# 0xC000005/PyChebyshev

Measured on AMD Instinct MI355X. Metric: point-evals/sec, 5D Black-Scholes n=11^5 barycentric + TT, 1/2/4/8 GPU, higher is better.
Workload: dtype f64; 1 GPU; 5D Black-Scholes n=11^5 full-tensor barycentric, 1,000,000 fp64 queries per GPU; evals_per_point=1, parallelism=batch-sharded x1, model replicated, one process per GPU, gather=none

## Files before the change

### pychebyshev_amd/_build.py

```python
from __future__ import annotations

import hashlib
import os
import shutil
import subprocess
import sys

HERE = os.path.dirname(os.path.abspath(__file__))
CSRC = os.path.join(HERE, "csrc")
LIB = os.path.join(HERE, "libpcx_hip.so")
PCX_H = os.path.join("..", "..", "include", "pcx.h")
HOST_H = ["pcx_common.h", "pcx_internal.h", PCX_H]
SOURCES = {
    "pcx_core.hip": HOST_H,
    "pcx_bary.hip": HOST_H + ["pcx_bary_internal.h", "bary_kernels.h", "gather_kernels.h", "sobol_kernels.h"],
    "pcx_bary_grid.hip": HOST_H + ["pcx_bary_internal.h", "bary_grid_kernels.h", "bary_weights.h"],
    "pcx_bary_kfold.hip": HOST_H + ["pcx_bary_internal.h", "bary_kfold_kernels.h"],
    "pcx_spline.hip": HOST_H + ["pcx_bary_internal.h", "gather_kernels.h", "route_kernels.h"],
    "pcx_tt.hip": HOST_H + ["tt_kernels.h", "tt_lpp_kernels.h", "tt_fd_kernels.h"],
    "pcx_tt_box.hip": HOST_H + ["tt_lpp_kernels.h", "tt_box_kernels.h"],
    "pcx_ttbuild.hip": HOST_H + ["ttcross_kernels.h", "ttsvd_kernels.h", "tt_round_kernels.h"],
    "pcx_calculus.hip": HOST_H + ["pcx_bary_internal.h", "calculus_kernels.h"],
    "pcx_comm.hip": [PCX_H],
}
OBJ_DIR = os.path.join(HERE, "_obj")
ARCH = "gfx950"
FLAGS = ["-O3", "-std=c++17", "-fPIC", "-fno-fast-math", "-ffp-contract=on", "-Wall", "-Wno-unused-function"]


def hipcc_path() -> str:
    for cand in (os.environ.get("HIPCC"), shutil.which("hipcc"), "/opt/rocm/bin/hipcc"):
        if cand and os.path.exists(cand):
            return cand
    raise RuntimeError("hipcc not found (set HIPCC or install ROCm)")


def _newer(target: str, deps) -> bool:
    if not os.path.exists(target):
        return True
    t = os.path.getmtime(target)
    return any(os.path.exists(f) and os.path.getmtime(f) > t for f in deps)


def _deps(src: str):
    return [os.path.join(CSRC, src)] + [os.path.join(CSRC, h) for h in SOURCES[src]] + [os.path.abspath(__file__)]


STAMP = LIB + ".stamp"


def _tu_digest(src: str) -> str:
    h = hashlib.sha256()
    h.update((" ".join(FLAGS) + ARCH).encode())
    for f in _deps(src)[:-1]:
        if os.path.exists(f):
            h.update(os.path.basename(f).encode())
            with open(f, "rb") as fh:
                h.update(fh.read())
    return h.hexdigest()


def _source_digest() -> str:
    return hashlib.sha256("".join(_tu_digest(src) for src in sorted(SOURCES)).encode()).hexdigest()


def _read(path: str) -> str:
    try:
        with open(path) as fh:
            return fh.read().strip()
    except OSError:
        return ""


def needs_build() -> bool:
    if not os.path.exists(LIB):
        return True
    try:
        with open(STAMP) as fh:
            return fh.read().strip() != _source_digest()
    except OSError:
        return any(_newer(LIB, _deps(src)) for src in SOURCES)


def _run(cmd, verbose):
    if verbose:
        print(" ".join(cmd), flush=True)
    res = subprocess.run(cmd, stdout=subprocess.PIPE, stderr=subprocess.STDOUT, text=True)
    if res.returncode != 0:
        raise RuntimeError("hipcc failed:\n" + res.stdout)
    if verbose and res.stdout.strip():
        print(res.stdout)


def build(force: bool = False, verbose: bool = False) -> str:
    if not force and not needs_build():
        return LIB
    hipcc = hipcc_path()
    os.makedirs(OBJ_DIR, exist_ok=True)
    digest_at_start = _source_digest()
    objs, stale = [], []
    for src in SOURCES:
        obj = os.path.join(OBJ_DIR, os.path.splitext(src)[0] + ".o")
        objs.append(obj)
        if force or not os.path.exists(obj) or _read(obj + ".stamp") != _tu_digest(src):
            stale.append((src, obj))

    def compile_one(item):
        src, obj = item
        digest = _tu_digest(src)
        _run([hipcc, f"--offload-arch={ARCH}", "-c"] + FLAGS + ["-o", obj, os.path.join(CSRC, src)], verbose)
        with open(obj + ".stamp", "w") as fh:
            fh.write(digest + "\n")

    jobs = max(1, min(len(stale), int(os.environ.get("PCX_BUILD_JOBS", "4"))))
    if jobs > 1:
        from concurrent.futures import ThreadPoolExecutor
        with ThreadPoolExecutor(jobs) as pool:
            list(pool.map(compile_one, stale))
    else:
        for item in stale:
            compile_one(item)
    for stale_obj in os.listdir(OBJ_DIR):
        if stale_obj.endswith(".o") and os.path.join(OBJ_DIR, stale_obj) not in objs:
            os.remove(os.path.join(OBJ_DIR, stale_obj))
    _run([hipcc, f"--offload-arch={ARCH}", "-shared", "-fPIC", "-o", LIB] + objs + ["-ldl"], verbose)
    with open(STAMP, "w") as fh:
        fh.write(digest_at_start + "\n")
    return LIB


if __name__ == "__main__":
    print(build(force="--force" in sys.argv, verbose=True))
```

### pychebyshev_amd/csrc/bary_kernels.h

```cpp
#pragma once

#include "pcx_common.h"

__global__ void k_mode_product(const double *__restrict__ in, double *__restrict__ out,
                               const double *__restrict__ D, long outer, int na, long inner) {
    long idx = (long)blockIdx.x * blockDim.x + threadIdx.x;
    long total = outer * na * inner;
    if (idx >= total) return;
    long q = idx % inner;
    long t = idx / inner;
    int i = (int)(t % na);
    long o = t / na;
    const double *src = in + (o * na) * inner + q;
    const double *drow = D + (long)i * na;
    double s = 0.0;
    for (int j = 0; j < na; ++j) s = __builtin_fma(src[(long)j * inner], drow[j], s);
    out[idx] = s;
}

__global__ void k_contract_axis(const double *__restrict__ in, double *__restrict__ out,
                                const double *__restrict__ vec, long outer, int na, long inner) {
    long idx = (long)blockIdx.x * blockDim.x + threadIdx.x;
    if (idx >= outer * inner) return;
    long q = idx % inner;
    long o = idx / inner;
    const double *src = in + (o * na) * inner + q;
    double s = 0.0;
    for (int j = 0; j < na; ++j) s = __builtin_fma(src[(long)j * inner], vec[j], s);
    out[idx] = s;
}

__global__ void k_pack_fragments(const double *__restrict__ T2, double *__restrict__ frag, int M,
                                 int K, int MT, int KS) {
    long idx = (long)blockIdx.x * blockDim.x + threadIdx.x;
    long total = (long)MT * KS * 64;
    if (idx >= total) return;
    int l = (int)(idx & 63);
    long ts = idx >> 6;
    int s = (int)(ts % KS);
    int t = (int)(ts / KS);
    int m = 16 * t + (l & 15);
    int k = 4 * s + (l >> 4);
    frag[idx] = (m < M && k < K) ? T2[(long)m * K + k] : 0.0;
}

__global__ void k_pack_fragments_slabs(const double *__restrict__ T3, double *__restrict__ frag, int n0, int M1,
                                       int K, int tps, int KS) {
    long idx = (long)blockIdx.x * blockDim.x + threadIdx.x;
    const long per_slab = (long)tps * KS * 64;
    if (idx >= per_slab * n0) return;
    const int i0 = (int)(idx / per_slab);
    const long r = idx - (long)i0 * per_slab;
    int l = (int)(r & 63);
    long ts = r >> 6;
    int s = (int)(ts % KS);
    int t = (int)(ts / KS);
    int m = 16 * t + (l & 15);
    int k = 4 * s + (l >> 4);
    frag[idx] = (m < M1 && k < K) ? T3[((long)i0 * M1 + m) * K + k] : 0.0;
}

__device__ __forceinline__ void bary_g0_finish(const BaryG0 &gs, const double *__restrict__ diff0, double *vecA,
                                               double *vecB, const double *b0, int stride, double *out_row) {
    typedef const double __attribute__((address_space(4))) *cptr_t;
    const cptr_t D0 = (cptr_t)(unsigned long long)diff0;
    const int n0 = gs.n0;
    for (int o = 0; o <= gs.maxorder; ++o) {
        if (o > 0) {
            for (int i = 0; i < n0; ++i) {
                double s = 0.0;
                for (int j = 0; j < n0; ++j) s = __builtin_fma(vecA[j * stride], D0[i * n0 + j], s);
                vecB[i * stride] = s;
            }
            double *t = vecA; vecA = vecB; vecB = t;
        }
        double y = 0.0;
        for (int i = 0; i < n0; ++i) y = __builtin_fma(b0[i * stride], vecA[i * stride], y);
        if (out_row)
            for (int s = 0; s < gs.nmem; ++s)
                if (gs.order[s] == o) out_row[gs.col[s]] = y;
    }
}

__device__ __forceinline__ void bary_weights_1d(double x, const double *__restrict__ nodes,
                                                const double *__restrict__ wts, int n, double *dst,
                                                int stride) {
    int exact = -1;
    for (int j = 0; j < n; ++j) {
        double diff = x - nodes[j];
        if (exact < 0 && __builtin_fabs(diff) < 1e-14) exact = j;
    }
    if (exact >= 0) {
        for (int j = 0; j < n; ++j) dst[j * stride] = (j == exact) ? 1.0 : 0.0;
    } else {
        double su = 0.0;
        for (int j = 0; j < n; ++j) {
            double u = wts[j] / (x - nodes[j]);
            dst[j * stride] = u;
            su += u;
        }
        double r = 1.0 / su;
        for (int j = 0; j < n; ++j) dst[j * stride] *= r;
    }
}

__device__ __forceinline__ double code_weight(unsigned code, const double *bw_col, int PW) {
    double w0 = bw_col[(code & 255u) * PW];
    double w1 = bw_col[((code >> 8) & 255u) * PW];
    double w2 = bw_col[((code >> 16) & 255u) * PW];
    double w3 = bw_col[(code >> 24) * PW];
    return (w0 * w1) * (w2 * w3);
}

struct pcx_u4 { unsigned v[4]; };
__device__ __forceinline__ pcx_u4 load_row_codes(const unsigned *__restrict__ codes, long t, int g) {
    const uint4 q = reinterpret_cast<const uint4 *>(codes)[4 * t + g];
    return pcx_u4{{q.x, q.y, q.z, q.w}};
}

template <int NF>
__device__ __forceinline__ double code_weight_t(unsigned code, const double *bw_col, int PW) {
    if constexpr (NF >= 4) return code_weight(code, bw_col, PW);
    else {
        double w0 = bw_col[(code & 255u) * PW];
        double w1 = bw_col[((code >> 8) & 255u) * PW];
        if constexpr (NF == 3) return (w0 * w1) * bw_col[((code >> 16) & 255u) * PW];
        else return w0 * w1;
    }
}

#define PCX_CHUNK_TILES 4

template <int KS, int NT, bool WIDE, int NF = 4, bool G0 = false>
__global__ void __launch_bounds__(256, 2)
k_bary_mfma(BaryDims dims, BaryMfmaPlan plan, const double *__restrict__ nodes,
            const double *__restrict__ wts, const double *const *__restrict__ frag_tab,
            const unsigned *__restrict__ rowcode, const unsigned *__restrict__ kcode,
            const unsigned *__restrict__ rowcode_hi, const unsigned *__restrict__ kcode_hi,
            const double *__restrict__ pts, double *__restrict__ out, long N, long ostride,
            long ooff, int chunks_per_split, double *__restrict__ partial,
            const int *__restrict__ perm, BaryG0 gs, const double *__restrict__ diff0) {
    static_assert(NT == 1 || NT == 2 || NT == 4, "PW must divide the wave");
    constexpr int PW = 16 * NT;
    constexpr int PH = 64 / PW;
    extern __shared__ double lds[];
    const int lane = threadIdx.x & 63;
    const int wave = threadIdx.x >> 6;
    const int g = lane >> 4;
    const int c = lane & 15;
    double *bw = lds + (size_t)wave * plan.rows * PW;
    const double *bwt = bw + (size_t)plan.tail_base * PW;
    const long base = ((long)blockIdx.x * 4 + wave) * PW;
    typedef const double __attribute__((address_space(1))) *gptr_t;
    const gptr_t frag = (gptr_t)frag_tab[blockIdx.z];
    const int nchunks = (plan.MT + PCX_CHUNK_TILES - 1) / PCX_CHUNK_TILES;
    const int ch0 = blockIdx.y * chunks_per_split;
    const int ch1 = (ch0 + chunks_per_split < nchunks) ? ch0 + chunks_per_split : nchunks;

    {
        const int pp = lane % PW;
        const int ph = lane / PW;
        const long pidx = base + pp;
        const bool valid = pidx < N;
        const long row = valid ? (perm ? (long)perm[pidx] : pidx) : 0;
        for (int k = ph; k < dims.d; k += PH) {
            const double *nd = nodes + dims.off[k];
            double x = valid ? pts[row * dims.d + k] : nd[0];
            const int trow = dims.off[k] + (k >= plan.split ? 1 : 0);
            bary_weights_1d(x, nd, wts + dims.off[k], dims.n[k], bw + (size_t)trow * PW + pp, PW);
        }
        if (ph == 0) {
            bw[(size_t)(plan.tail_base - 1) * PW + pp] = 1.0;
            bw[(size_t)(plan.rows - 1) * PW + pp] = 1.0;
        }
    }
    __syncthreads();

    double B[NT][KS];
#pragma unroll
    for (int s = 0; s < KS; ++s) {
        unsigned code = kcode[4 * s + g];
#pragma unroll
        for (int nt = 0; nt < NT; ++nt) B[nt][s] = code_weight(code, bwt + 16 * nt + c, PW);
        if (WIDE) {
            unsigned hi = kcode_hi[4 * s + g];
#pragma unroll
            for (int nt = 0; nt < NT; ++nt) B[nt][s] *= code_weight(hi, bwt + 16 * nt + c, PW);
        }
    }

    double total[NT], cs[NT];
#pragma unroll
    for (int nt = 0; nt < NT; ++nt) { total[nt] = 0.0; cs[nt] = 0.0; }
    const gptr_t tf = frag + lane;
    const int t_begin = ch0 * PCX_CHUNK_TILES;
    const int t_end = (ch1 * PCX_CHUNK_TILES < plan.MT) ? ch1 * PCX_CHUNK_TILES : plan.MT;
    const bool split = gridDim.y > 1;
    constexpr bool PIPELINED = (KS >= 12);
    constexpr int DEPTH = 6;
    unsigned cn[4] = {0u, 0u, 0u, 0u}, cnh[4] = {0u, 0u, 0u, 0u};
    double head[DEPTH];
#pragma unroll
    for (int i = 0; i < DEPTH; ++i) head[i] = 0.0;
    if (PIPELINED && t_begin < t_end) {
        {
            const pcx_u4 q = load_row_codes(rowcode, t_begin, g);
            pcx_u4 qh = q;
            if (WIDE) qh = load_row_codes(rowcode_hi, t_begin, g);
#pragma unroll
            for (int j = 0; j < 4; ++j) {
                cn[j] = q.v[j];
                if (WIDE) cnh[j] = qh.v[j];
            }
        }
#pragma unroll
        for (int i = 0; i < DEPTH; ++i) head[i] = tf[((size_t)t_begin * KS + i) * 64];
    }
    for (int t = t_begin; t < t_end; ++t) {
        double w[NT][4];
        pcx_d4 acc[NT];
#pragma unroll
        for (int nt = 0; nt < NT; ++nt) acc[nt] = (pcx_d4){0.0, 0.0, 0.0, 0.0};
        const gptr_t tt = tf + (size_t)t * KS * 64;
        if constexpr (PIPELINED) {
            const int t_next = (t + 1 < t_end) ? t + 1 : t;
            const gptr_t tn = tf + (size_t)t_next * KS * 64;
            double ring[DEPTH];
            unsigned cc[4], cch[4];
#pragma unroll
            for (int i = 0; i < DEPTH; ++i) ring[i] = head[i];
            {
                const pcx_u4 q = load_row_codes(rowcode, t_next, g);
                pcx_u4 qh = q;
                if (WIDE) qh = load_row_codes(rowcode_hi, t_next, g);
#pragma unroll
                for (int j = 0; j < 4; ++j) {
                    cc[j] = cn[j];
                    cn[j] = q.v[j];
                    if (WIDE) { cch[j] = cnh[j]; cnh[j] = qh.v[j]; }
                }
            }
            double wr[4][NT][4];
            double wh[4][NT][4];
#pragma unroll
            for (int s = 0; s < KS; ++s) {
                const double a = ring[s % DEPTH];
                if (s + DEPTH < KS) ring[s % DEPTH] = tt[(s + DEPTH) * 64];
                else head[s + DEPTH - KS] = tn[(s + DEPTH - KS) * 64];
#pragma unroll
                for (int j = 0; j < 4; ++j) {
                    if (s == 2 * j) {
#pragma unroll
                        for (int nt = 0; nt < NT; ++nt)
#pragma unroll
                            for (int f = 0; f < (NF < 4 ? NF : 4); ++f)
                                wr[j][nt][f] = bw[(size_t)((cc[j] >> (8 * f)) & 255u) * PW + 16 * nt + c];
                    }
                    if (s == 2 * j + 2) {
#pragma unroll
                        for (int nt = 0; nt < NT; ++nt)
                            w[nt][j] = NF >= 4 ? (wr[j][nt][0] * wr[j][nt][1]) * (wr[j][nt][2] * wr[j][nt][3])
                                     : (NF == 3 ? (wr[j][nt][0] * wr[j][nt][1]) * wr[j][nt][2]
                                                : wr[j][nt][0] * wr[j][nt][1]);
                    }
                    if (WIDE && s == 2 * j + 1) {
#pragma unroll
                        for (int nt = 0; nt < NT; ++nt)
#pragma unroll
                            for (int f = 0; f < 4; ++f)
                                wh[j][nt][f] = bw[(size_t)((cch[j] >> (8 * f)) & 255u) * PW + 16 * nt + c];
                    }
                    if (WIDE && s == 2 * j + 3) {
#pragma unroll
                        for (int nt = 0; nt < NT; ++nt)
                            w[nt][j] *= (wh[j][nt][0] * wh[j][nt][1]) * (wh[j][nt][2] * wh[j][nt][3]);
                    }
                }
                __builtin_amdgcn_sched_barrier(0);
#pragma unroll
                for (int nt = 0; nt < NT; ++nt)
                    acc[nt] = __builtin_amdgcn_mfma_f64_16x16x4f64(a, B[nt][s], acc[nt], 0, 0, 0);
                __builtin_amdgcn_sched_barrier(0);
            }
        } else {
            const pcx_u4 q = load_row_codes(rowcode, t, g);
            pcx_u4 qh = q;
            if (WIDE) qh = load_row_codes(rowcode_hi, t, g);
#pragma unroll
            for (int j = 0; j < 4; ++j) {
                unsigned code = q.v[j];
#pragma unroll
                for (int nt = 0; nt < NT; ++nt) w[nt][j] = code_weight_t<NF>(code, bw + 16 * nt + c, PW);
                if (WIDE) {
                    unsigned hi = qh.v[j];
#pragma unroll
                    for (int nt = 0; nt < NT; ++nt) w[nt][j] *= code_weight(hi, bw + 16 * nt + c, PW);
                }
            }
#pragma unroll
            for (int s = 0; s < KS; ++s) {
                double a = tt[s * 64];
#pragma unroll
                for (int nt = 0; nt < NT; ++nt)
                    acc[nt] = __builtin_amdgcn_mfma_f64_16x16x4f64(a, B[nt][s], acc[nt], 0, 0, 0);
            }
        }
#pragma unroll
        for (int nt = 0; nt < NT; ++nt)
#pragma unroll
            for (int j = 0; j < 4; ++j) cs[nt] = __builtin_fma(acc[nt][j], w[nt][j], cs[nt]);
        if constexpr (G0) {
            if ((t + 1) % gs.tps == 0) {
                const int i0 = t / gs.tps;
                double *Pl = const_cast<double *>(bwt);
#pragma unroll
                for (int nt = 0; nt < NT; ++nt) {
                    double v = cs[nt];
                    v += __shfl_xor(v, 16, 64);
                    v += __shfl_xor(v, 32, 64);
                    if (g == 0) Pl[(size_t)i0 * PW + 16 * nt + c] = v;
                    cs[nt] = 0.0;
                }
            }
            continue;
        }
        const bool chunk_end = ((t + 1) % PCX_CHUNK_TILES == 0) || (t + 1 == plan.MT);
        if (chunk_end) {
            if (split) {
                const int ch = t / PCX_CHUNK_TILES;
#pragma unroll
                for (int nt = 0; nt < NT; ++nt) {
                    long pidx = base + 16 * nt + c;
                    if (pidx < N)
                        partial[(((size_t)blockIdx.z * nchunks + ch) * 4 + g) * (size_t)N + pidx] = cs[nt];
                }
            }
#pragma unroll
            for (int nt = 0; nt < NT; ++nt) { total[nt] += cs[nt]; cs[nt] = 0.0; }
        }
    }

    if constexpr (G0) {
        if (lane < PW) {
            double *Pl = const_cast<double *>(bwt) + lane;
            const long pidx = base + lane;
            const long row = (pidx < N) ? (perm ? (long)perm[pidx] : pidx) : 0;
            bary_g0_finish(gs, diff0, Pl, Pl + (size_t)gs.n0 * PW, bw + (size_t)dims.off[0] * PW + lane, PW,
                           pidx < N ? out + row * ostride + ooff : nullptr);
        }
        return;
    }
    if (!split) {
#pragma unroll
        for (int nt = 0; nt < NT; ++nt) {
            double v = total[nt];
            v += __shfl_xor(v, 16, 64);
            v += __shfl_xor(v, 32, 64);
            long pidx = base + 16 * nt + c;
            if (g == 0 && pidx < N) {
                long row = perm ? (long)perm[pidx] : pidx;
                out[row * ostride + ooff + blockIdx.z] = v;
            }
        }
    }
}

template <int KS>
__global__ void __launch_bounds__(512, 2)
k_bary_mfma4(BaryDims dims, BaryMfmaPlan plan, const double *__restrict__ nodes,
             const double *__restrict__ wts, const double *const *__restrict__ frag_tab,
             const unsigned *__restrict__ rowcode, const unsigned *__restrict__ kcode,
             const double *__restrict__ pts, double *__restrict__ out, long N, long ostride,
             long ooff, const int *__restrict__ perm) {
    constexpr int NT = 2;
    constexpr int PW = 32;
    constexpr int SLAB = KS * 64;
    constexpr int CPT = (SLAB + 511) / 512;
    extern __shared__ double lds[];
    const int lane = threadIdx.x & 63;
    const int wave = threadIdx.x >> 6;
    const int g = lane >> 4;
    const int c = lane & 15;
    double *bw = lds + (size_t)wave * plan.rows * PW;
    const double *bwt = bw + (size_t)plan.tail_base * PW;
    double *slab = lds + (size_t)8 * plan.rows * PW;
    const long base = ((long)blockIdx.x * 8 + wave) * PW;
    typedef const double __attribute__((address_space(1))) *gptr_t;
    const gptr_t frag = (gptr_t)frag_tab[blockIdx.z];

    {
        const int pp = lane & 31;
        const int ph = lane >> 5;
        const long pidx = base + pp;
        const bool valid = pidx < N;
        const long row = valid ? (perm ? (long)perm[pidx] : pidx) : 0;
        for (int k = ph; k < dims.d; k += 2) {
            const double *nd = nodes + dims.off[k];
            double x = valid ? pts[row * dims.d + k] : nd[0];
            const int trow = dims.off[k] + (k >= plan.split ? 1 : 0);
            bary_weights_1d(x, nd, wts + dims.off[k], dims.n[k], bw + (size_t)trow * PW + pp, PW);
        }
        if (ph == 0) {
            bw[(size_t)(plan.tail_base - 1) * PW + pp] = 1.0;
            bw[(size_t)(plan.rows - 1) * PW + pp] = 1.0;
        }
    }
    double stage[CPT];
    auto img_index = [](int i) {
        const int s_ = i >> 6, l_ = i & 63;
        const int k_ = l_ >> 4, rg_ = (l_ >> 2) & 3, ii_ = l_ & 3;
        return s_ * 64 + (rg_ >> 1) * 32 + (k_ * 4 + ii_) * 2 + (rg_ & 1);
    };
#pragma unroll
    for (int r = 0; r < CPT; ++r) {
        const int i = threadIdx.x + 512 * r;
        if (i < SLAB) slab[img_index(i)] = frag[i];
    }
    if (plan.MT > 1) {
#pragma unroll
        for (int r = 0; r < CPT; ++r) {
            const int i = threadIdx.x + 512 * r;
            stage[r] = (i < SLAB) ? frag[(size_t)SLAB + i] : 0.0;
        }
    }
    __syncthreads();

    double B[NT][KS];
#pragma unroll
    for (int s = 0; s < KS; ++s) {
        unsigned code = kcode[4 * s + g];
#pragma unroll
        for (int nt = 0; nt < NT; ++nt) B[nt][s] = code_weight(code, bwt + 16 * nt + c, PW);
    }

    double total[NT], cs[NT];
#pragma unroll
    for (int nt = 0; nt < NT; ++nt) { total[nt] = 0.0; cs[nt] = 0.0; }
    const int aoff = ((lane >> 4) * 4 + (lane & 3)) * 2;
    for (int t = 0; t < plan.MT; ++t) {
        const double *cur = slab + (size_t)(t & 1) * SLAB;
        double *nxt = slab + (size_t)((t + 1) & 1) * SLAB;
        if (t + 1 < plan.MT) {
#pragma unroll
            for (int r = 0; r < CPT; ++r) {
                const int i = threadIdx.x + 512 * r;
                if (i < SLAB) nxt[img_index(i)] = stage[r];
            }
        }
        if (t + 2 < plan.MT) {
            const gptr_t src = frag + (size_t)(t + 2) * SLAB;
#pragma unroll
            for (int r = 0; r < CPT; ++r) {
                const int i = threadIdx.x + 512 * r;
                stage[r] = (i < SLAB) ? src[i] : 0.0;
            }
        }
        const pcx_u4 q4 = load_row_codes(rowcode, t, g);
        const unsigned code0 = q4.v[0], code1 = q4.v[1], code2 = q4.v[2], code3 = q4.v[3];
#pragma unroll
        for (int half = 0; half < 2; ++half) {
            constexpr int DEPTH = (KS < 6) ? KS : 6;
            double acc[2][NT];
#pragma unroll
            for (int r = 0; r < 2; ++r)
#pragma unroll
                for (int nt = 0; nt < NT; ++nt) acc[r][nt] = 0.0;
            typedef double d2_t __attribute__((ext_vector_type(2)));
            const d2_t *ar = reinterpret_cast<const d2_t *>(cur + aoff + 32 * half);
            d2_t ring[DEPTH];
#pragma unroll
            for (int s = 0; s < DEPTH; ++s) ring[s] = ar[s * 32];
#pragma unroll
            for (int s = 0; s < KS; ++s) {
                const double a0 = ring[s % DEPTH][0], a1 = ring[s % DEPTH][1];
                if (s + DEPTH < KS) ring[s % DEPTH] = ar[(s + DEPTH) * 32];
                __builtin_amdgcn_sched_barrier(0);
#pragma unroll
                for (int nt = 0; nt < NT; ++nt) {
                    acc[0][nt] = __builtin_amdgcn_mfma_f64_4x4x4f64(a0, B[nt][s], acc[0][nt], 0, 0, 0);
                    acc[1][nt] = __builtin_amdgcn_mfma_f64_4x4x4f64(a1, B[nt][s], acc[1][nt], 0, 0, 0);
                }
                __builtin_amdgcn_sched_barrier(0);
            }
            const unsigned codeA = half ? code2 : code0, codeB = half ? code3 : code1;
#pragma unroll
            for (int nt = 0; nt < NT; ++nt) {
                cs[nt] = __builtin_fma(acc[0][nt], code_weight(codeA, bw + 16 * nt + c, PW), cs[nt]);
                cs[nt] = __builtin_fma(acc[1][nt], code_weight(codeB, bw + 16 * nt + c, PW), cs[nt]);
            }
        }
        const bool chunk_end = ((t + 1) % PCX_CHUNK_TILES == 0) || (t + 1 == plan.MT);
        if (chunk_end) {
#pragma unroll
            for (int nt = 0; nt < NT; ++nt) { total[nt] += cs[nt]; cs[nt] = 0.0; }
        }
        __syncthreads();
    }

#pragma unroll
    for (int nt = 0; nt < NT; ++nt) {
        double v = total[nt];
        v += __shfl_xor(v, 16, 64);
        v += __shfl_xor(v, 32, 64);
        long pidx = base + 16 * nt + c;
        if (g == 0 && pidx < N) {
            long row = perm ? (long)perm[pidx] : pidx;
            out[row * ostride + ooff + blockIdx.z] = v;
        }
    }
}

__global__ void k_bary_reduce(const double *__restrict__ partial, double *__restrict__ out, long N,
                              int nchunks, int nspec, long ostride, long ooff,
                              const int *__restrict__ perm) {
    long idx = (long)blockIdx.x * blockDim.x + threadIdx.x;
    if (idx >= N * nspec) return;
    long p = idx % N;
    int z = (int)(idx / N);
    const double *src = partial + (size_t)z * nchunks * 4 * (size_t)N + p;
    double sg[4];
    for (int g = 0; g < 4; ++g) {
        double t = 0.0;
        for (int ch = 0; ch < nchunks; ++ch) t += src[((size_t)ch * 4 + g) * (size_t)N];
        sg[g] = t;
    }
    long row = perm ? (long)perm[p] : p;
    out[row * ostride + ooff + z] = (sg[0] + sg[1]) + (sg[2] + sg[3]);
}

__global__ void __launch_bounds__(256)
k_bary_rows(BaryDims dims, int LPP, const double *__restrict__ nodes,
            const double *__restrict__ wts, const double *__restrict__ T,
            const double *__restrict__ pts, double *__restrict__ out, long N, long ostride,
            long ooff, const int *__restrict__ perm) {
    extern __shared__ double lds[];
    const int ppw = 256 / LPP;
    const int pl = threadIdx.x / LPP;
    const int sub = threadIdx.x % LPP;
    const long pidx = (long)blockIdx.x * ppw + pl;
    const bool valid = pidx < N;
    const long row = valid ? (perm ? (long)perm[pidx] : pidx) : 0;
    double *bw = lds + (size_t)pl * dims.sum_n;
    for (int k = sub; k < dims.d; k += LPP) {
        const double *nd = nodes + dims.off[k];
        double x = valid ? pts[row * dims.d + k] : nd[0];
        bary_weights_1d(x, nd, wts + dims.off[k], dims.n[k], bw + dims.off[k], 1);
    }
    __syncthreads();
    const int d = dims.d;
    const int K = dims.n[d - 1];
    long M = 1;
    for (int k = 0; k < d - 1; ++k) M *= dims.n[k];
    const double *bl = bw + dims.off[d - 1];
    double acc = 0.0;
    for (long m = sub; m < M; m += LPP) {
        double w = 1.0;
        long rem = m;
        for (int k = d - 2; k >= 0; --k) {
            int nk = dims.n[k];
            int i = (int)(rem % nk);
            rem /= nk;
            w *= bw[dims.off[k] + i];
        }
        const double *row = T + m * K;
        double s = 0.0;
        for (int j = 0; j < K; ++j) s = __builtin_fma(row[j], bl[j], s);
        acc = __builtin_fma(s, w, acc);
    }
    for (int o = LPP >> 1; o > 0; o >>= 1) acc += __shfl_xor(acc, o, 64);
    if (sub == 0 && valid) out[row * ostride + ooff] = acc;
}


typedef const double __attribute__((address_space(4))) *pcx_cptr;
__device__ __forceinline__ pcx_cptr pcx_as_constant(const double *p) { return (pcx_cptr)(unsigned long long)p; }

template <int NLP, bool EXACT>
__device__ __forceinline__ void bary_weights_reg(double x, double scale, pcx_cptr snodes, pcx_cptr wts, int n,
                                                 double (&b)[NLP]) {
    double t[NLP];
    double run = 1.0, amin = 1.0e300;
#pragma unroll
    for (int j = 0; j < NLP; ++j) {
        b[j] = 0.0;
        t[j] = 1.0;
        if (EXACT || j < n) {
            t[j] = __builtin_fma(x, scale, -snodes[j]);
            amin = __builtin_fmin(amin, __builtin_fabs(t[j]));
            b[j] = wts[j] * run;
            run *= t[j];
        }
    }
    run = 1.0;
    double su = 0.0;
#pragma unroll
    for (int j = NLP - 1; j >= 0; --j) {
        if (EXACT || j < n) {
            b[j] *= run;
            su += b[j];
            run *= t[j];
        }
    }
    const double r = 1.0 / su;
#pragma unroll
    for (int j = 0; j < NLP; ++j) b[j] *= r;
    if (amin < 1e-14 * scale) {
        bool found = false;
#pragma unroll
        for (int j = 0; j < NLP; ++j) {
            const bool hit = !found && (EXACT || j < n) && __builtin_fabs(t[j]) < 1e-14 * scale;
            b[j] = hit ? 1.0 : 0.0;
            found = found || hit;
        }
    }
}

__device__ __forceinline__ void bary_weights_prod(double x, double scale, pcx_cptr snodes, pcx_cptr wts, int n,
                                                  double *dst, int stride) {
    double run = 1.0, amin = 1.0e300;
    for (int j = 0; j < n; ++j) {
        dst[j * stride] = wts[j] * run;
        const double t = __builtin_fma(x, scale, -snodes[j]);
        amin = __builtin_fmin(amin, __builtin_fabs(t));
        run *= t;
    }
    run = 1.0;
    double su = 0.0;
    for (int j = n - 1; j >= 0; --j) {
        const double c = dst[j * stride] * run;
        dst[j * stride] = c;
        su += c;
        run *= __builtin_fma(x, scale, -snodes[j]);
    }
    const double r = 1.0 / su;
    for (int j = 0; j < n; ++j) dst[j * stride] *= r;
    if (amin < 1e-14 * scale) {
        bool found = false;
        for (int j = 0; j < n; ++j) {
            const bool hit = !found && __builtin_fabs(__builtin_fma(x, scale, -snodes[j])) < 1e-14 * scale;
            dst[j * stride] = hit ? 1.0 : 0.0;
            found = found || hit;
        }
    }
}

template <int LEVEL, int DOUT, int NLP>
__device__ __forceinline__ double bary_small_nest(const BaryDims &dims, pcx_cptr Tb,
                                                  const double *bw_lane, const double (&bl)[NLP]) {
    if constexpr (LEVEL == DOUT) {
        double s = 0.0;
#pragma unroll
        for (int i = 0; i < NLP; ++i) s = __builtin_fma(Tb[i], bl[i], s);
        return s;
    } else {
        long stride = 1;
        for (int q = LEVEL + 1; q <= DOUT; ++q) stride *= dims.n[q];
        const double *wk = bw_lane + (size_t)dims.off[LEVEL] * 64;
        double s = 0.0;
        for (int i = 0; i < dims.n[LEVEL]; ++i)
            s = __builtin_fma(wk[(size_t)i * 64], bary_small_nest<LEVEL + 1, DOUT, NLP>(dims, Tb + i * stride, bw_lane, bl), s);
        return s;
    }
}


template <int DOUT, int NLP>
__device__ __forceinline__ void bary_small_body(const BaryDims &dims, const BarySmallScale &sc, pcx_cptr csn, pcx_cptr cnd,
                                                pcx_cptr cw, const double *T, const double *const *T_tab, int m,
                                                const double *__restrict__ pts, double *__restrict__ out, bool valid,
                                                long row, long ostride, long ooff, double *bw_lane) {
    const int d = DOUT + 1;
#pragma unroll
    for (int k = 0; k < DOUT; ++k) {
        const double x = valid ? pts[row * d + k] : cnd[dims.off[k]];
        bary_weights_prod(x, sc.s[k], csn + dims.off[k], cw + dims.off[k], dims.n[k],
                          bw_lane + (size_t)dims.off[k] * 64, 64);
    }
    double bl[NLP];
    {
        const double x = valid ? pts[row * d + DOUT] : cnd[dims.off[DOUT]];
        if (dims.n[DOUT] == NLP)
            bary_weights_reg<NLP, true>(x, sc.s[DOUT], csn + dims.off[DOUT], cw + dims.off[DOUT], NLP, bl);
        else
            bary_weights_reg<NLP, false>(x, sc.s[DOUT], csn + dims.off[DOUT], cw + dims.off[DOUT], dims.n[DOUT], bl);
    }
    if (T_tab == nullptr) {
        const double y = bary_small_nest<0, DOUT, NLP>(dims, pcx_as_constant(T), bw_lane, bl);
        if (valid) out[row * ostride + ooff] = y;
    } else {
        for (int z = 0; z < m; ++z) {
            const double y = bary_small_nest<0, DOUT, NLP>(dims, pcx_as_constant(T_tab[z]), bw_lane, bl);
            if (valid) out[row * ostride + ooff + z] = y;
        }
    }
}

template <int DOUT, int NLP>
__global__ void __launch_bounds__(64)
k_bary_small(BaryDims dims, BarySmallScale sc, const double *__restrict__ snodes, const double *__restrict__ nodes,
             const double *__restrict__ wts, const double *__restrict__ T, const double *const *__restrict__ T_tab,
             int m, const double *__restrict__ pts, double *__restrict__ out, long N, long ostride, long ooff,
             const int *__restrict__ perm) {
    extern __shared__ double lds[];
    const int lane = threadIdx.x;
    const long pidx = (long)blockIdx.x * 64 + lane;
    const bool valid = pidx < N;
    const long row = valid ? (perm ? (long)perm[pidx] : pidx) : 0;
    bary_small_body<DOUT, NLP>(dims, sc, pcx_as_constant(snodes), pcx_as_constant(nodes), pcx_as_constant(wts), T, T_tab, m,
                               pts, out, valid, row, ostride, ooff, lds + lane);
}

template <int NL>
__device__ __forceinline__ double bary_sq_block(pcx_cptr Tb, const double (&b1)[NL], const double (&b2)[NL]) {
    constexpr int R4 = (NL % 4 == 0) ? 4 : (NL % 3 == 0) ? 3 : (NL % 5 == 0) ? 5 : (NL % 4 == 1 && NL > 5) ? 3 : 4;
    double t0 = 0.0, t1 = 0.0;
#pragma unroll
    for (int i = 0; i < NL; i += R4) {
        double s[R4];
#pragma unroll
        for (int r = 0; r < R4; ++r)
            if (i + r < NL) s[r] = Tb[(i + r) * NL] * b2[0];
#pragma unroll
        for (int k = 1; k < NL; ++k)
#pragma unroll
            for (int r = 0; r < R4; ++r)
                if (i + r < NL) s[r] = __builtin_fma(Tb[(i + r) * NL + k], b2[k], s[r]);
#pragma unroll
        for (int r = 0; r < R4; ++r)
            if (i + r < NL) {
                if (r & 1) t1 = __builtin_fma(b1[i + r], s[r], t1);
                else t0 = __builtin_fma(b1[i + r], s[r], t0);
            }
    }
    return t0 + t1;
}

template <int NL, int LEAD>
__device__ __forceinline__ double bary_sq_tensor(const BaryDims &dims, pcx_cptr T, const double *bw_lane,
                                                 const double (&b1)[NL], const double (&b2)[NL]) {
    if constexpr (LEAD == 0) return bary_sq_block<NL>(T, b1, b2);
    else if constexpr (LEAD == 1) {
        double y = 0.0;
        for (int i0 = 0; i0 < dims.n[0]; ++i0, T += NL * NL)
            y = __builtin_fma(bw_lane[(size_t)i0 * 64], bary_sq_block<NL>(T, b1, b2), y);
        return y;
    } else {
        double y = 0.0;
        const double *w1 = bw_lane + (size_t)dims.off[1] * 64;
        for (int i0 = 0; i0 < dims.n[0]; ++i0) {
            double a = 0.0;
            for (int i1 = 0; i1 < dims.n[1]; ++i1, T += NL * NL)
                a = __builtin_fma(w1[(size_t)i1 * 64], bary_sq_block<NL>(T, b1, b2), a);
            y = __builtin_fma(bw_lane[(size_t)i0 * 64], a, y);
        }
        return y;
    }
}

template <int NL, int LEAD>
__device__ __forceinline__ void bary_sq_body(const BaryDims &dims, const BarySmallScale &sc, pcx_cptr csn, pcx_cptr cnd, pcx_cptr cw,
                                             const double *T, const double *const *T_tab, int m, const double *__restrict__ pts,
                                             double *__restrict__ out, bool valid, long row, long ostride, long ooff,
                                             double *bw_lane) {
    constexpr int D = LEAD + 2;
#pragma unroll
    for (int k = 0; k < LEAD; ++k) {
        const double x = valid ? pts[row * D + k] : cnd[dims.off[k]];
        bary_weights_prod(x, sc.s[k], csn + dims.off[k], cw + dims.off[k], dims.n[k], bw_lane + (size_t)dims.off[k] * 64, 64);
    }
    double b1[NL], b2[NL];
    {
        const double x1 = valid ? pts[row * D + LEAD] : cnd[dims.off[LEAD]];
        const double x2 = valid ? pts[row * D + LEAD + 1] : cnd[dims.off[LEAD + 1]];
        bary_weights_reg<NL, true>(x1, sc.s[LEAD], csn + dims.off[LEAD], cw + dims.off[LEAD], NL, b1);
        bary_weights_reg<NL, true>(x2, sc.s[LEAD + 1], csn + dims.off[LEAD + 1], cw + dims.off[LEAD + 1], NL, b2);
    }
    for (int z = 0; z < m; ++z) {
        const double y = bary_sq_tensor<NL, LEAD>(dims, pcx_as_constant(T_tab ? T_tab[z] : T), bw_lane, b1, b2);
        if (valid) out[row * ostride + ooff + z] = y;
    }
}

template <int NL, int LEAD>
__global__ void __launch_bounds__(64)
k_bary_sq(BaryDims dims, BarySmallScale sc, const double *__restrict__ snodes, const double *__restrict__ nodes,
          const double *__restrict__ wts, const double *__restrict__ T, const double *const *__restrict__ T_tab, int m,
          const double *__restrict__ pts, double *__restrict__ out, long N, long ostride, long ooff,
          const int *__restrict__ perm) {
    extern __shared__ double lds[];
    const int lane = threadIdx.x;
    const long pidx = (long)blockIdx.x * 64 + lane;
    const bool valid = pidx < N;
    const long row = valid ? (perm ? (long)perm[pidx] : pidx) : 0;
    bary_sq_body<NL, LEAD>(dims, sc, pcx_as_constant(snodes), pcx_as_constant(nodes), pcx_as_constant(wts), T, T_tab, m, pts, out,
                           valid, row, ostride, ooff, lds + lane);
}


template <int DOUT, int NLP>
__global__ void __launch_bounds__(64)
k_bary_small_pieces(BaryDims dims, const SplinePieceModel *__restrict__ models, const int *__restrict__ blk_piece,
                    const int *__restrict__ blk_first, const int *__restrict__ piece_end, int m,
                    const double *__restrict__ pts, double *__restrict__ out, long ostride, long ooff,
                    const int *__restrict__ perm) {
    extern __shared__ double lds[];
    const int lane = threadIdx.x;
    const int piece = blk_piece[blockIdx.x];
    const long pidx = (long)blk_first[blockIdx.x] + lane;
    const bool valid = pidx < (long)piece_end[piece];
    const long row = valid ? (long)perm[pidx] : 0;
    typedef const SplinePieceModel __attribute__((address_space(4))) *model_cptr;
    const model_cptr mp = (model_cptr)(unsigned long long)(models + piece);
    BarySmallScale sc;
#pragma unroll
    for (int k = 0; k < 4; ++k) sc.s[k] = mp->sc.s[k];
    bary_small_body<DOUT, NLP>(dims, sc, pcx_as_constant(mp->snodes), pcx_as_constant(mp->nodes), pcx_as_constant(mp->wts),
                               mp->T, mp->T_tab, m, pts, out, valid, row, ostride, ooff, lds + lane);
}

template <int NL, int LEAD>
__global__ void __launch_bounds__(64)
k_bary_sq_pieces(BaryDims dims, const SplinePieceModel *__restrict__ models, const int *__restrict__ blk_piece,
                 const int *__restrict__ blk_first, const int *__restrict__ piece_end, int m,
                 const double *__restrict__ pts, double *__restrict__ out, long ostride, long ooff,
                 const int *__restrict__ perm) {
    extern __shared__ double lds[];
    const int lane = threadIdx.x;
    const int piece = blk_piece[blockIdx.x];
    const long pidx = (long)blk_first[blockIdx.x] + lane;
    const bool valid = pidx < (long)piece_end[piece];
    const long row = valid ? (long)perm[pidx] : 0;
    typedef const SplinePieceModel __attribute__((address_space(4))) *model_cptr;
    const model_cptr mp = (model_cptr)(unsigned long long)(models + piece);
    BarySmallScale sc;
#pragma unroll
    for (int k = 0; k < 4; ++k) sc.s[k] = mp->sc.s[k];
    bary_sq_body<NL, LEAD>(dims, sc, pcx_as_constant(mp->snodes), pcx_as_constant(mp->nodes), pcx_as_constant(mp->wts), mp->T,
                           mp->T_tab, m, pts, out, valid, row, ostride, ooff, lds + lane);
}
```

### pychebyshev_amd/csrc/pcx_bary.hip

```cpp

#include "pcx_bary_internal.h"
#include "bary_kernels.h"
#include "gather_kernels.h"
#include "sobol_kernels.h"

static const int g_g0_span_default = [] { const char *e = getenv("PCX_BARY_G0_SPAN"); return e ? std::min(8, std::max(0, atoi(e))) : 1; }();

static const double g_group_tol_default = [] { const char *e = getenv("PCX_BARY_GROUP_TOL"); double v = e ? atof(e) : 0.0; return v > 0.0 ? v : 3e-13; }();

static const long kSmallTensorElems = 4096;
static const int kCacheSpecs = 96;

static const int kKsList[] = {1, 2, 3, 4, 5, 6, 7, 8, 9, 10, 11, 12, 13, 14, 15, 16, 17, 18, 19, 20, 21, 22,
                              23, 24, 25, 26, 27, 28, 29, 30, 31, 32, 36, 40, 44, 48, 52, 56, 60, 64};

static int pick_ks(int K) {
    int need = (K + 3) / 4;
    for (int ks : kKsList)
        if (ks >= need) return ks;
    return -1;
}

static bool plan_mfma(const BaryDims &dm, BaryMfmaPlan &best) {
    bool found = false;
    long best_cost = 0;
    for (int split = std::max(0, dm.d - 2 * PCX_CODE_FIELDS); split < dm.d; ++split) {
        if (split > 2 * PCX_CODE_FIELDS) continue;
        long M = 1, K = 1, head_rows = 0, tail_rows = 0;
        for (int k = 0; k < split; ++k) { M *= dm.n[k]; head_rows += dm.n[k]; }
        for (int k = split; k < dm.d; ++k) { K *= dm.n[k]; tail_rows += dm.n[k]; }
        if (K > 256 || M > (1 << 24)) continue;
        if (head_rows > PCX_MAX_PART_ROWS || tail_rows > PCX_MAX_PART_ROWS) continue;
        int ks = pick_ks((int)K);
        if (ks < 0) continue;
        long mt = (M + 15) / 16;
        long cost = mt * (ks + 5) * (ks > 32 ? 23 : 20);
        if (!found || cost < best_cost || (cost == best_cost && K > best.K)) {
            found = true;
            best_cost = cost;
            best.split = split; best.M = (int)M; best.K = (int)K; best.MT = (int)mt; best.KS = ks;
            best.tail_base = (int)head_rows + 1;
            best.rows = dm.sum_n + 2;
        }
    }
    return found;
}

static size_t mfma4_lds_bytes(const BaryDims &dm, int ks) {
    return ((size_t)8 * (dm.sum_n + 2) * 32 + (size_t)2 * ks * 64) * sizeof(double);
}

static size_t mfma_lds_bytes(const BaryDims &dm, int nt) {
    return (size_t)4 * (dm.sum_n + 2) * 16 * nt * sizeof(double);
}

extern "C" int pcx_bary_destroy(pcx_bary *h) {
    PCX_API_BEGIN
    if (!h) return PCX_OK;
    (void)hipSetDevice(h->device);
    if (h->stream) (void)hipStreamSynchronize(h->stream);
    for (auto &kv : h->cache) kv.second.free_all();
    (void)hipFree(h->d_tab);
    h->s_partial.release();
    (void)hipFree(h->d_nodes); (void)hipFree(h->d_wts); (void)hipFree(h->d_diff);
    (void)hipFree(h->d_cheb);
    h->s_cheb[0].release(); h->s_cheb[1].release(); h->s_sobol.release();
    (void)hipFree(h->d_snodes);
    (void)hipFree(h->d_gsnodes);
    (void)hipFree(h->d_rowcode); (void)hipFree(h->d_kcode);
    (void)hipFree(h->d_rowcode_hi); (void)hipFree(h->d_kcode_hi);
    (void)hipFree(h->d_rowcode_g0);
    for (pcx_bary *&r : h->rot) { if (r) pcx_bary_destroy(r); r = nullptr; }
    h->stage.release();
    h->s_rot.release(); h->s_rot2.release();
    if (h->stream) (void)hipStreamDestroy(h->stream);
    delete h;
    return PCX_OK;
    PCX_API_END
}

static int bary_pack(pcx_bary *h, DerivedTensor &dt) {
    if (!h->mfma_ok) return PCX_OK;
    const BaryMfmaPlan &p = h->plan;
    size_t cnt = h->kfold_ok ? bary_kfold_frag_count(h->kf) : (size_t)(h->grid_ok ? h->gp.MT : p.MT) * p.KS * 64;
    DevBuf frag, slot;
    int rc = frag.alloc(cnt * sizeof(double));
    if (rc) return rc;
    if (h->kfold_ok) {
        if ((rc = bary_pack_kfold(h, dt.plain, frag.as<double>()))) return rc;
    } else if (h->grid_ok) {
        if ((rc = bary_pack_grid(h, dt.plain, frag.as<double>()))) return rc;
    } else {
        int blocks = (int)((cnt + 255) / 256);
        hipLaunchKernelGGL(k_pack_fragments, dim3(blocks), dim3(256), 0, h->stream, dt.plain, frag.as<double>(),
                           p.M, p.K, p.MT, p.KS);
        HIP_TRY(hipGetLastError());
    }
    if ((rc = slot.alloc(sizeof(double *)))) return rc;
    double *fp = frag.as<double>();
    HIP_TRY(hipMemcpy(slot.p, &fp, sizeof(double *), hipMemcpyHostToDevice));
    dt.frag = frag.release<double>();
    dt.slot = slot.release<double *>();
    return PCX_OK;
}

extern "C" int pcx_bary_create(int device, int d, const int32_t *n_nodes, const double *nodes_cat,
                               const double *weights_cat, const double *diffmat_cat,
                               const double *tensor, pcx_bary **out) {
    PCX_API_BEGIN
    if (!out) return fail(PCX_ERR_INVALID, "out is NULL");
    *out = nullptr;
    if (d < 1 || d > PCX_MAX_DIMS) return fail(PCX_ERR_INVALID, "d=%d outside [1, %d]", d, PCX_MAX_DIMS);
    if (!n_nodes || !nodes_cat || !weights_cat || !diffmat_cat || !tensor)
        return fail(PCX_ERR_INVALID, "NULL model array");
    int rc = use_device(device);
    if (rc) return rc;
    pcx_bary *h = new (std::nothrow) pcx_bary();
    if (!h) return fail(PCX_ERR_NOMEM, "out of host memory");
    h->device = device;
    h->dims.d = d;
    h->g0_span = g_g0_span_default;
    h->group_tol = g_group_tol_default;
    long total = 1, sum_n = 0, sum_n2 = 0;
    for (int k = 0; k < d; ++k) {
        if (n_nodes[k] < 1 || n_nodes[k] > 4096) { delete h; return fail(PCX_ERR_INVALID, "n_nodes[%d]=%d outside [1, 4096]", k, n_nodes[k]); }
        h->dims.n[k] = n_nodes[k];
        h->dims.off[k] = (int)sum_n;
        h->doff.push_back((int)sum_n2);
        sum_n += n_nodes[k];
        sum_n2 += (long)n_nodes[k] * n_nodes[k];
        total *= n_nodes[k];
        if (total > (1L << 33)) { delete h; return fail(PCX_ERR_UNSUPPORTED, "tensor larger than 2^33 elements"); }
    }
    for (int k = d; k < PCX_MAX_DIMS; ++k) { h->dims.n[k] = 1; h->dims.off[k] = 0; }
    h->dims.sum_n = (int)sum_n;
    h->total = total;

#define CREATE_TRY(expr)                                                                   \
    do {                                                                                   \
        hipError_t e_ = (expr);                                                            \
        if (e_ != hipSuccess) {                                                            \
            int c_ = fail(PCX_ERR_HIP, "%s failed: %s", #expr, hipGetErrorString(e_));     \
            pcx_bary_destroy(h);                                                           \
            return c_;                                                                     \
        }                                                                                  \
    } while (0)

    CREATE_TRY(hipStreamCreateWithFlags(&h->stream, hipStreamNonBlocking));
    CREATE_TRY(hipMalloc((void **)&h->d_nodes, sum_n * sizeof(double)));
    CREATE_TRY(hipMalloc((void **)&h->d_wts, sum_n * sizeof(double)));
    CREATE_TRY(hipMalloc((void **)&h->d_diff, sum_n2 * sizeof(double)));
    CREATE_TRY(hipMemcpy(h->d_nodes, nodes_cat, sum_n * sizeof(double), hipMemcpyHostToDevice));
    CREATE_TRY(hipMemcpy(h->d_wts, weights_cat, sum_n * sizeof(double), hipMemcpyHostToDevice));
    CREATE_TRY(hipMemcpy(h->d_diff, diffmat_cat, sum_n2 * sizeof(double), hipMemcpyHostToDevice));

    long Mrows = total / h->dims.n[d - 1];
    int lpp = 1;
    while (lpp < 64 && lpp < Mrows) lpp <<= 1;
    while (lpp < 64 && (size_t)(256 / lpp) * sum_n * sizeof(double) > 48 * 1024) lpp <<= 1;
    h->lpp = lpp;

    h->mfma_ok = plan_mfma(h->dims, h->plan);
    if (h->mfma_ok) {
        const bool narrow = h->plan.split <= PCX_CODE_FIELDS && d - h->plan.split <= PCX_CODE_FIELDS;
        h->nt = (h->plan.KS <= 32 || (narrow && h->plan.KS <= 40)) ? 2 : 1;
        if (mfma_lds_bytes(h->dims, h->nt) > 150 * 1024) h->nt = 1;
        if (mfma_lds_bytes(h->dims, h->nt) > 150 * 1024) h->mfma_ok = false;
    }
    if (!h->mfma_ok && (size_t)(256 / h->lpp) * sum_n * sizeof(double) > 160 * 1024) {
        int c_ = fail(PCX_ERR_UNSUPPORTED, "sum of node counts %ld too large for any kernel (MFMA plan: each of the "
                      "head / tail parts <= %d rows and a tail product <= 256; row kernel: sum <= 5120)", sum_n, PCX_MAX_PART_ROWS);
        pcx_bary_destroy(h);
        return c_;
    }
    h->mfma4_ok = h->mfma_ok && mfma4_lds_bytes(h->dims, h->plan.KS) <= 160 * 1024 &&
                  h->plan.KS <= 32 && h->plan.split <= PCX_CODE_FIELDS && d - h->plan.split <= PCX_CODE_FIELDS;
    {
        static const int kNlp[] = {2, 3, 4, 5, 6, 7, 8, 9, 10, 11, 12, 13, 14, 15, 16, 24, 32, 48, 64};
        const int nl = h->dims.n[d - 1];
        const long outer_rows = sum_n - nl;
        if (d <= 4 && nl <= 64 && outer_rows * 64 * (long)sizeof(double) <= 64 * 1024 && total <= (1L << 22)) {
            for (int v : kNlp)
                if (v >= nl) { h->small_nlp = v; break; }
            h->small_preferred = total <= kSmallTensorElems && (nl <= 48 || (d == 2 && n_nodes[0] <= 48));
            if (d >= 2 && n_nodes[d - 2] == nl && ((nl >= 4 && nl <= 24) || nl == 26 || nl == 28 || nl == 30 || nl == 32) &&
                (outer_rows - nl) * 64 * (long)sizeof(double) <= 48 * 1024) {
                h->sq_nl = nl;
                static const bool sq_auto = [] { const char *e = getenv("PCX_BARY_SQ"); return !(e && e[0] == '0'); }();
                h->sq_preferred = sq_auto && (d <= 3 || total <= kSmallTensorElems) && nl != 23 &&
                                  !(d >= 3 && nl >= 24) && !(d == 3 && nl == 20 && n_nodes[0] == 20);
            }
            std::vector<double> sn((size_t)sum_n);
            for (int k = 0; k < d; ++k) {
                const double *nd = nodes_cat + h->dims.off[k];
                const double span = nd[n_nodes[k] - 1] - nd[0];
                int e = 0;
                if (span > 0.0 && std::isfinite(span)) (void)std::frexp(2.0 / span, &e);
                const double sck = std::ldexp(1.0, e - 1);
                h->small_scale.s[k] = sck;
                for (int j = 0; j < n_nodes[k]; ++j) sn[h->dims.off[k] + j] = nd[j] * sck;
            }
            CREATE_TRY(hipMalloc((void **)&h->d_snodes, sum_n * sizeof(double)));
            CREATE_TRY(hipMemcpy(h->d_snodes, sn.data(), sum_n * sizeof(double), hipMemcpyHostToDevice));
        }
    }
    if (h->mfma_ok) {
        const BaryMfmaPlan &p = h->plan;
        const unsigned ones_h = (unsigned)(p.tail_base - 1), ones_t = (unsigned)(p.rows - 1 - p.tail_base);
        std::vector<unsigned> rowcode((size_t)p.MT * 16), kcode((size_t)p.KS * 4);
        std::vector<unsigned> rowcode_hi(rowcode.size()), kcode_hi(kcode.size());
        h->wide = p.split > PCX_CODE_FIELDS || d - p.split > PCX_CODE_FIELDS;
        for (long m = 0; m < (long)p.MT * 16; ++m) {
            unsigned f[2 * PCX_CODE_FIELDS] = {ones_h, ones_h, ones_h, ones_h, ones_h, ones_h, ones_h, ones_h};
            if (m < p.M) {
                long rem = m;
                for (int k = p.split - 1; k >= 0; --k) {
                    int i = (int)(rem % h->dims.n[k]);
                    rem /= h->dims.n[k];
                    f[k] = (unsigned)(h->dims.off[k] + i);
                }
            }
            rowcode[m] = f[0] | (f[1] << 8) | (f[2] << 16) | (f[3] << 24);
            rowcode_hi[m] = f[4] | (f[5] << 8) | (f[6] << 16) | (f[7] << 24);
        }
        for (long kk = 0; kk < (long)p.KS * 4; ++kk) {
            unsigned f[2 * PCX_CODE_FIELDS] = {ones_t, ones_t, ones_t, ones_t, ones_t, ones_t, ones_t, ones_t};
            if (kk < p.K) {
                long rem = kk;
                for (int k = d - 1; k >= p.split; --k) {
                    int i = (int)(rem % h->dims.n[k]);
                    rem /= h->dims.n[k];
                    f[k - p.split] = (unsigned)(h->dims.off[k] - h->dims.off[p.split] + i);
                }
            }
            kcode[kk] = f[0] | (f[1] << 8) | (f[2] << 16) | (f[3] << 24);
            kcode_hi[kk] = f[4] | (f[5] << 8) | (f[6] << 16) | (f[7] << 24);
        }
        auto lane_order = [&](std::vector<unsigned> &v) {
            std::vector<unsigned> o(v.size());
            for (long t = 0; t < (long)p.MT; ++t)
                for (int g = 0; g < 4; ++g)
                    for (int j = 0; j < 4; ++j) o[(size_t)(4 * t + g) * 4 + j] = v[(size_t)16 * t + g + 4 * j];
            v.swap(o);
        };
        lane_order(rowcode);
        lane_order(rowcode_hi);
        if (h->wide) {
            CREATE_TRY(hipMalloc((void **)&h->d_rowcode_hi, rowcode_hi.size() * sizeof(unsigned)));
            CREATE_TRY(hipMalloc((void **)&h->d_kcode_hi, kcode_hi.size() * sizeof(unsigned)));
            CREATE_TRY(hipMemcpy(h->d_rowcode_hi, rowcode_hi.data(), rowcode_hi.size() * sizeof(unsigned), hipMemcpyHostToDevice));
            CREATE_TRY(hipMemcpy(h->d_kcode_hi, kcode_hi.data(), kcode_hi.size() * sizeof(unsigned), hipMemcpyHostToDevice));
        }
        CREATE_TRY(hipMalloc((void **)&h->d_rowcode, rowcode.size() * sizeof(unsigned)));
        CREATE_TRY(hipMalloc((void **)&h->d_kcode, kcode.size() * sizeof(unsigned)));
        CREATE_TRY(hipMemcpy(h->d_rowcode, rowcode.data(), rowcode.size() * sizeof(unsigned), hipMemcpyHostToDevice));
        CREATE_TRY(hipMemcpy(h->d_kcode, kcode.data(), kcode.size() * sizeof(unsigned), hipMemcpyHostToDevice));
        long M1 = 1;
        for (int k = 1; k < p.split; ++k) M1 *= h->dims.n[k];
        if (!h->wide && p.split >= 2 && p.split <= PCX_CODE_FIELDS && h->nt == 2 && p.KS <= 32 && M1 >= 16 &&
            2 * h->dims.n[0] <= p.rows - p.tail_base && h->dims.n[0] >= 2 && h->dims.n[0] <= 16) {
            const int tps = (int)((M1 + 15) / 16);
            const long mtg = (long)tps * h->dims.n[0];
            if (mtg * 100 <= (long)p.MT * 115) {
                std::vector<unsigned> rc((size_t)mtg * 16);
                for (long t = 0; t < mtg; ++t)
                    for (int r = 0; r < 16; ++r) {
                        const long m1 = (t % tps) * 16 + r;
                        unsigned f[PCX_CODE_FIELDS] = {ones_h, ones_h, ones_h, ones_h};
                        if (m1 < M1) {
                            long rem = m1;
                            for (int k = p.split - 1; k >= 1; --k) {
                                int i = (int)(rem % h->dims.n[k]);
                                rem /= h->dims.n[k];
                                f[k - 1] = (unsigned)(h->dims.off[k] + i);
                            }
                        }
                        rc[(size_t)16 * t + r] = f[0] | (f[1] << 8) | (f[2] << 16) | (f[3] << 24);
                    }
                std::vector<unsigned> o(rc.size());
                for (long t = 0; t < mtg; ++t)
                    for (int g = 0; g < 4; ++g)
                        for (int j = 0; j < 4; ++j) o[(size_t)(4 * t + g) * 4 + j] = rc[(size_t)16 * t + g + 4 * j];
                CREATE_TRY(hipMalloc((void **)&h->d_rowcode_g0, o.size() * sizeof(unsigned)));
                CREATE_TRY(hipMemcpy(h->d_rowcode_g0, o.data(), o.size() * sizeof(unsigned), hipMemcpyHostToDevice));
                h->g0_ok = true;
                h->g0_tps = tps;
                h->g0_nf = std::max(2, p.split - 1);
            }
        }
    }

    if (h->mfma_ok && !(h->plan.split > PCX_CODE_FIELDS || d - h->plan.split > PCX_CODE_FIELDS)) {
        long kfold_est = 0;
        {
            const long keff = bary_plan_kfold(h->dims, h->kf);
            kfold_est = bary_kfold_estimate(h->kf, keff);
            long geff = 0;
            BaryGridPlan gtry;
            gtry.MT = 0;
            if (keff > 0 && !h->g0_ok) {
                (void)bary_plan_grid(h->dims, h->plan, gtry);
                if (gtry.MT > 0)
                    geff = (long)((double)h->plan.M * h->plan.K * 10000.0 / ((double)gtry.MT * 16.0 * h->plan.KS * 4.0));
            }
            h->kfold_ok = bary_kfold_take(h->kf, keff, geff, h->plan.KS);
        }
        if (h->kfold_ok) {
            const int nt_rc = h->nt;
            h->nt = 2;
            if (bary_kfold_lds_bytes(h->kf, 2) > (size_t)72 * 1024) h->nt = 1;
            if (bary_kfold_lds_bytes(h->kf, h->nt) > (size_t)150 * 1024) { h->kfold_ok = false; h->nt = nt_rc; }
        }
        if (h->kfold_ok && total >= kSmallTensorElems && kfold_est >= 500) h->sq_preferred = h->small_preferred = false;
        if (h->kfold_ok && h->g0_ok) {
            h->g0_ok = false;
            (void)hipFree(h->d_rowcode_g0);
            h->d_rowcode_g0 = nullptr;
        }
        if (!h->kfold_ok && !h->g0_ok) h->grid_ok = bary_plan_grid(h->dims, h->plan, h->gp);
        if (h->grid_ok) {
            h->nt = h->plan.KS > 32 ? 1 : 2;
            const size_t cap = (size_t)(h->gp.wpb == 4 ? 150 : 64) * 1024;
            if (bary_grid_lds_bytes(h, h->nt) > cap) h->nt = 1;
            if (bary_grid_lds_bytes(h, h->nt) > cap) h->grid_ok = false;
        }
    }
    if (h->grid_ok || h->kfold_ok) {
        std::vector<double> sn((size_t)sum_n + PCX_MAX_DIMS, 0.0);
        h->grid_prod = true;
        for (int k = 0; k < d; ++k) {
            const double *nd = nodes_cat + h->dims.off[k];
            const double span = nd[n_nodes[k] - 1] - nd[0];
            int e = 0;
            if (span > 0.0 && std::isfinite(span)) (void)std::frexp(2.0 / span, &e);
            const double sck = std::ldexp(1.0, e - 1);
            sn[(size_t)sum_n + k] = sck;
            for (int j = 0; j < n_nodes[k]; ++j) sn[h->dims.off[k] + j] = nd[j] * sck;
            if (n_nodes[k] > 64) h->grid_prod = false;
        }
        { const char *e = getenv("PCX_BARY_GRID_PROD"); if (e && e[0] == '0') h->grid_prod = false; }
        CREATE_TRY(hipMalloc((void **)&h->d_gsnodes, sn.size() * sizeof(double)));
        CREATE_TRY(hipMemcpy(h->d_gsnodes, sn.data(), sn.size() * sizeof(double), hipMemcpyHostToDevice));
    }
    if (h->grid_ok || h->kfold_ok) h->mfma4_ok = false;

    DerivedTensor dt;
    {
        DevBuf plain;
        rc = alloc_plain(plain, total);
        if (rc) { pcx_bary_destroy(h); return rc; }
        dt.plain = plain.release<double>();
    }
    { hipError_t e_ = hipMemcpy(dt.plain, tensor, total * sizeof(double), hipMemcpyHostToDevice);
      if (e_ != hipSuccess) { (void)hipFree(dt.plain); int c_ = fail(PCX_ERR_HIP, "tensor upload: %s", hipGetErrorString(e_)); pcx_bary_destroy(h); return c_; } }
    rc = bary_pack(h, dt);
    if (rc) { (void)hipFree(dt.plain); pcx_bary_destroy(h); return rc; }
    h->cache[std::vector<int>(d, 0)] = dt;
    CREATE_TRY(hipMalloc((void **)&h->d_tab, kMaxSpecs * sizeof(double *)));
    CREATE_TRY(hipStreamSynchronize(h->stream));
#undef CREATE_TRY
    *out = h;
    return PCX_OK;
    PCX_API_END
}

static void host_grid_metadata(double lo, double hi, int n, double *x, double *w, double *D) {
    const double pi = 3.14159265358979323846;
    for (int k = 0; k < n; ++k)
        x[k] = 0.5 * (lo + hi) + 0.5 * (hi - lo) * std::sin(0.5 * pi / n * (double)(-n + 1 + 2 * k));
    std::sort(x, x + n);
    for (int i = 0; i < n; ++i) {
        double wi = 1.0;
        for (int j = 0; j < n; ++j)
            if (j != i) wi /= (x[i] - x[j]);
        w[i] = wi;
    }
    for (int i = 0; i < n; ++i) {
        double rowsum = 0.0;
        for (int j = 0; j < n; ++j) {
            double v = (i == j) ? 0.0 : w[j] / ((x[i] - x[j]) * w[i]);
            D[(size_t)i * n + j] = v;
            rowsum += v;
        }
        D[(size_t)i * n + i] = -rowsum;
    }
}

extern "C" int pcx_bary_create_from_pcb(int device, const char *path, pcx_bary **out) {
    PCX_API_BEGIN
    if (!out) return fail(PCX_ERR_INVALID, "out is NULL");
    *out = nullptr;
    if (!path) return fail(PCX_ERR_INVALID, "path is NULL");
    FILE *f = fopen(path, "rb");
    if (!f) return fail(PCX_ERR_INVALID, "cannot open %s", path);
    auto bail = [&](const char *why) { fclose(f); return fail(PCX_ERR_INVALID, "%s: %s", path, why); };
    unsigned char head[12];
    if (fread(head, 1, 12, f) != 12) return bail("shorter than the 12-byte .pcb header");
    if (memcmp(head, "PCB\0", 4) != 0) return bail("not a PyChebyshev binary file (bad magic)");
    if (head[4] != 1) return bail("unsupported .pcb major version");
    if ((head[6] | (head[7] << 8)) != 1) return bail("class tag is not ChebyshevApproximation");
    if (head[8] | head[9] | head[10] | head[11]) return bail("reserved header bytes nonzero");
    uint32_t d = 0;
    if (fread(&d, 4, 1, f) != 1) return bail("unexpected EOF reading num_dimensions");
    if (d < 1 || d > PCX_MAX_DIMS) return bail("num_dimensions outside [1, 16]");
    std::vector<double> lo(d), hi(d);
    std::vector<uint32_t> nn(d);
    if (fread(lo.data(), 8, d, f) != d || fread(hi.data(), 8, d, f) != d || fread(nn.data(), 4, d, f) != d)
        return bail("unexpected EOF reading domain / n_nodes");
    size_t total = 1, sum_n = 0, sum_n2 = 0;
    std::vector<int32_t> n(d);
    for (uint32_t k = 0; k < d; ++k) {
        if (!(lo[k] < hi[k])) return bail("domain lo must be < hi");
        if (nn[k] < 1 || nn[k] > 4096) return bail("n_nodes outside [1, 4096]");
        n[k] = (int32_t)nn[k];
        total *= nn[k];
        sum_n += nn[k];
        sum_n2 += (size_t)nn[k] * nn[k];
        if (total > ((size_t)1 << 33)) return bail("tensor larger than 2^33 elements");
    }
    std::vector<double> tensor(total);
    if (fread(tensor.data(), 8, total, f) != total) return bail("unexpected EOF reading tensor_values");
    fclose(f);
    for (size_t i = 0; i < total; ++i)
        if (!std::isfinite(tensor[i])) return fail(PCX_ERR_INVALID, "%s: tensor_values contains NaN or Inf", path);
    std::vector<double> nodes(sum_n), wts(sum_n), diff(sum_n2);
    size_t o1 = 0, o2 = 0;
    for (uint32_t k = 0; k < d; ++k) {
        host_grid_metadata(lo[k], hi[k], n[k], nodes.data() + o1, wts.data() + o1, diff.data() + o2);
        o1 += n[k];
        o2 += (size_t)n[k] * n[k];
    }
    int rc = pcx_bary_create(device, (int)d, n.data(), nodes.data(), wts.data(), diff.data(), tensor.data(), out);
    if (rc == PCX_OK) { (*out)->dom_lo = lo; (*out)->dom_hi = hi; }
    return rc;
    PCX_API_END
}

extern "C" int pcx_bary_save_pcb(pcx_bary *h, const char *path, const double *lo, const double *hi) {
    PCX_API_BEGIN
    if (!h || !path) return fail(PCX_ERR_INVALID, "NULL argument");
    const int d = h->dims.d;
    if ((lo == nullptr) != (hi == nullptr)) return fail(PCX_ERR_INVALID, "pass both domain bounds or neither");
    if (!lo) {
        if ((int)h->dom_lo.size() != d)
            return fail(PCX_ERR_INVALID, "the handle does not know its domain (not loaded from a .pcb file): pass lo / hi");
        lo = h->dom_lo.data();
        hi = h->dom_hi.data();
    }
    for (int k = 0; k < d; ++k)
        if (!(lo[k] < hi[k])) return fail(PCX_ERR_INVALID, "domain[%d]: lo must be < hi", k);
    std::vector<double> tensor((size_t)h->total);
    {
        HIP_TRY(hipSetDevice(h->device));
        std::lock_guard<std::mutex> lk(h->mu);
        const DerivedTensor &base = h->cache[std::vector<int>(d, 0)];
        HIP_TRY(hipMemcpy(tensor.data(), base.plain, (size_t)h->total * sizeof(double), hipMemcpyDeviceToHost));
    }
    FILE *f = fopen(path, "wb");
    if (!f) return fail(PCX_ERR_INVALID, "cannot open %s for writing", path);
    const unsigned char head[12] = {'P', 'C', 'B', 0, 1, 0, 1, 0, 0, 0, 0, 0};
    const uint32_t du = (uint32_t)d;
    std::vector<uint32_t> nn(d);
    for (int k = 0; k < d; ++k) nn[k] = (uint32_t)h->dims.n[k];
    bool ok = fwrite(head, 1, 12, f) == 12 && fwrite(&du, 4, 1, f) == 1 && fwrite(lo, 8, d, f) == (size_t)d &&
              fwrite(hi, 8, d, f) == (size_t)d && fwrite(nn.data(), 4, d, f) == (size_t)d &&
              fwrite(tensor.data(), 8, tensor.size(), f) == tensor.size();
    ok = (fclose(f) == 0) && ok;
    if (!ok) return fail(PCX_ERR_INVALID, "short write to %s", path);
    return PCX_OK;
    PCX_API_END
}

extern "C" int pcx_bary_shape(pcx_bary *h, int32_t *d_out, int32_t *n_nodes_out) {
    PCX_API_BEGIN
    if (!h) return fail(PCX_ERR_INVALID, "handle is NULL");
    if (d_out) *d_out = h->dims.d;
    if (n_nodes_out)
        for (int k = 0; k < PCX_MAX_DIMS; ++k) n_nodes_out[k] = k < h->dims.d ? h->dims.n[k] : 0;
    return PCX_OK;
    PCX_API_END
}

PCX_HIDDEN int bary_get_tensor(pcx_bary *h, const int32_t *deriv, DerivedTensor **out) {
    const int d = h->dims.d;
    std::vector<int> key(d, 0);
    if (deriv)
        for (int k = 0; k < d; ++k) {
            if (deriv[k] < 0 || deriv[k] > 8) return fail(PCX_ERR_INVALID, "derivative order %d at dim %d outside [0, 8]", deriv[k], k);
            key[k] = deriv[k];
        }
    auto it = h->cache.find(key);
    if (it != h->cache.end()) {
        it->second.last_use = ++h->clock;
        *out = &it->second;
        return PCX_OK;
    }
    if (h->cache.size() > (size_t)kCacheSpecs) {
        auto victim = h->cache.end();
        for (auto c = h->cache.begin(); c != h->cache.end(); ++c) {
            bool is_base = true;
            for (int v : c->first) is_base = is_base && v == 0;
            if (is_base || c->second.last_use > h->call_mark) continue;
            if (victim == h->cache.end() || c->second.last_use < victim->second.last_use) victim = c;
        }
        if (victim == h->cache.end())
            return fail(PCX_ERR_UNSUPPORTED, "more than %d distinct derivative specs in one call", kCacheSpecs);
        HIP_TRY(hipDeviceSynchronize());
        if (!h->tab_host.empty()) h->tab_host.clear();
        victim->second.free_all();
        h->cache.erase(victim);
    }

    DerivedTensor &base = h->cache[std::vector<int>(d, 0)];
    DevBuf cur, tmp;
    int rc = alloc_plain(cur, h->total);
    if (rc) return rc;
    if ((rc = alloc_plain(tmp, h->total))) return rc;
    HIP_TRY(hipMemcpyAsync(cur.p, base.plain, h->total * sizeof(double), hipMemcpyDeviceToDevice, h->stream));
    for (int k = d - 1; k >= 0; --k) {
        long outer = 1, inner = 1;
        for (int q = 0; q < k; ++q) outer *= h->dims.n[q];
        for (int q = k + 1; q < d; ++q) inner *= h->dims.n[q];
        for (int r = 0; r < key[k]; ++r) {
            int blocks = (int)((h->total + 255) / 256);
            hipLaunchKernelGGL(k_mode_product, dim3(blocks), dim3(256), 0, h->stream, cur.as<double>(), tmp.as<double>(),
                               h->d_diff + h->doff[k], outer, h->dims.n[k], inner);
            std::swap(cur.p, tmp.p);
        }
    }
    HIP_TRY(hipGetLastError());
    HIP_TRY(hipStreamSynchronize(h->stream));
    DerivedTensor dt;
    dt.plain = cur.as<double>();
    if ((rc = bary_pack(h, dt))) return rc;
    (void)cur.release<double>();
    dt.last_use = ++h->clock;
    auto ins = h->cache.emplace(key, dt);
    *out = &ins.first->second;
    return PCX_OK;
}

template <int KS, int NT, bool WIDE, int NF = 4>
static int launch_mfma_t(pcx_bary *h, const double *const *frag_tab, int m, const double *d_pts, long N,
                         double *d_out, long ostride, long ooff, hipStream_t st, Scratch *split_scratch,
                         const int *perm) {
    const bool allow_split = split_scratch != nullptr;
    size_t lds = mfma_lds_bytes(h->dims, NT);
    auto kern = k_bary_mfma<KS, NT, WIDE, NF>;
    if (lds > 64 * 1024)
        HIP_TRY(hipFuncSetAttribute((const void *)kern, hipFuncAttributeMaxDynamicSharedMemorySize, (int)lds));
    long per_wg = 4L * 16 * NT;
    long blocks = (N + per_wg - 1) / per_wg;
    if (blocks > 0x7fffffffL) return fail(PCX_ERR_UNSUPPORTED, "batch too large for one launch");
    int nchunks = (h->plan.MT + PCX_CHUNK_TILES - 1) / PCX_CHUNK_TILES;
    int nsplit = 1, cps = nchunks;
    const long want = 512;
    if (allow_split && blocks * m < want && nchunks > 1) {
        nsplit = (int)std::min<long>(nchunks, (want + blocks * m - 1) / (blocks * m));
        cps = (nchunks + nsplit - 1) / nsplit;
        nsplit = (nchunks + cps - 1) / cps;
    }
    double *partial = nullptr;
    if (nsplit > 1) {
        int rc = split_scratch->reserve((size_t)m * nchunks * 4 * (size_t)N * sizeof(double));
        if (rc) return rc;
        partial = (double *)split_scratch->ptr;
    }
    hipLaunchKernelGGL(kern, dim3((unsigned)blocks, (unsigned)nsplit, (unsigned)m), dim3(256), lds, st,
                       h->dims, h->plan, h->d_nodes, h->d_wts, frag_tab, h->d_rowcode, h->d_kcode,
                       h->d_rowcode_hi, h->d_kcode_hi, d_pts, d_out, N, ostride, ooff, cps, partial, perm, BaryG0{}, nullptr);
    HIP_TRY(hipGetLastError());
    if (nsplit > 1) {
        long cnt = N * m;
        hipLaunchKernelGGL(k_bary_reduce, dim3((unsigned)((cnt + 255) / 256)), dim3(256), 0, st, partial, d_out,
                           N, nchunks, m, ostride, ooff, perm);
        HIP_TRY(hipGetLastError());
    }
    return PCX_OK;
}

template <int KS>
static int launch_mfma4_t(pcx_bary *h, const double *const *frag_tab, int m, const double *d_pts, long N,
                          double *d_out, long ostride, long ooff, hipStream_t st, const int *perm) {
    size_t lds = mfma4_lds_bytes(h->dims, KS);
    auto kern = k_bary_mfma4<KS>;
    if (lds > 64 * 1024)
        HIP_TRY(hipFuncSetAttribute((const void *)kern, hipFuncAttributeMaxDynamicSharedMemorySize, (int)lds));
    long blocks = (N + 255) / 256;
    if (blocks > 0x7fffffffL) return fail(PCX_ERR_UNSUPPORTED, "batch too large for one launch");
    hipLaunchKernelGGL(kern, dim3((unsigned)blocks, 1, (unsigned)m), dim3(512), lds, st, h->dims, h->plan,
                       h->d_nodes, h->d_wts, frag_tab, h->d_rowcode, h->d_kcode, d_pts, d_out, N, ostride, ooff, perm);
    HIP_TRY(hipGetLastError());
    return PCX_OK;
}

static int launch_mfma4(pcx_bary *h, const double *const *frag_tab, int m, const double *d_pts, long N,
                        double *d_out, long ostride, long ooff, hipStream_t st, const int *perm) {
    switch (h->plan.KS) {
#define CASE_KS(v) case v: return launch_mfma4_t<v>(h, frag_tab, m, d_pts, N, d_out, ostride, ooff, st, perm);
        CASE_KS(1) CASE_KS(2) CASE_KS(3) CASE_KS(4) CASE_KS(5) CASE_KS(6) CASE_KS(7) CASE_KS(8)
        CASE_KS(9) CASE_KS(10) CASE_KS(11) CASE_KS(12) CASE_KS(13) CASE_KS(14) CASE_KS(15) CASE_KS(16)
        CASE_KS(17) CASE_KS(18) CASE_KS(19) CASE_KS(20) CASE_KS(21) CASE_KS(22) CASE_KS(23) CASE_KS(24)
        CASE_KS(25) CASE_KS(26) CASE_KS(27) CASE_KS(28) CASE_KS(29) CASE_KS(30) CASE_KS(31) CASE_KS(32)
#undef CASE_KS
    }
    return fail(PCX_ERR_UNSUPPORTED, "no MFMA instantiation for KS=%d", h->plan.KS);
}

template <int NT, bool WIDE, int NF>
static int launch_mfma_nf(pcx_bary *h, const double *const *frag_tab, int m, const double *d_pts, long N,
                          double *d_out, long ostride, long ooff, hipStream_t st, Scratch *split_scratch,
                          const int *perm) {
    switch (h->plan.KS) {
#define CASE_KS(v) case v: return launch_mfma_t<v, NT, WIDE, NF>(h, frag_tab, m, d_pts, N, d_out, ostride, ooff, st, split_scratch, perm);
        CASE_KS(1) CASE_KS(2) CASE_KS(3) CASE_KS(4) CASE_KS(5) CASE_KS(6) CASE_KS(7) CASE_KS(8)
        CASE_KS(9) CASE_KS(10) CASE_KS(11) CASE_KS(12) CASE_KS(13) CASE_KS(14) CASE_KS(15) CASE_KS(16)
        CASE_KS(17) CASE_KS(18) CASE_KS(19) CASE_KS(20) CASE_KS(21) CASE_KS(22) CASE_KS(23) CASE_KS(24)
        CASE_KS(25) CASE_KS(26) CASE_KS(27) CASE_KS(28) CASE_KS(29) CASE_KS(30) CASE_KS(31) CASE_KS(32)
#undef CASE_KS
    }
    if constexpr (NT == 1) {
        switch (h->plan.KS) {
#define CASE_KS(v) case v: return launch_mfma_t<v, 1, WIDE, NF>(h, frag_tab, m, d_pts, N, d_out, ostride, ooff, st, split_scratch, perm);
            CASE_KS(36) CASE_KS(40) CASE_KS(44) CASE_KS(48) CASE_KS(52) CASE_KS(56) CASE_KS(60) CASE_KS(64)
#undef CASE_KS
        }
    }
    if constexpr (NT == 2 && !WIDE) {
        switch (h->plan.KS) {
#define CASE_KS(v) case v: return launch_mfma_t<v, 2, WIDE, NF>(h, frag_tab, m, d_pts, N, d_out, ostride, ooff, st, split_scratch, perm);
            CASE_KS(36) CASE_KS(40)
#undef CASE_KS
        }
    }
    return fail(PCX_ERR_UNSUPPORTED, "no MFMA instantiation for KS=%d, NT=%d", h->plan.KS, NT);
}

template <int NT, bool WIDE>
static int launch_mfma_nt(pcx_bary *h, const double *const *frag_tab, int m, const double *d_pts, long N,
                          double *d_out, long ostride, long ooff, hipStream_t st, Scratch *split_scratch,
                          const int *perm) {
    if constexpr (!WIDE) {
        if (h->plan.split <= 2)
            return launch_mfma_nf<NT, false, 2>(h, frag_tab, m, d_pts, N, d_out, ostride, ooff, st, split_scratch, perm);
        if (h->plan.split == 3)
            return launch_mfma_nf<NT, false, 3>(h, frag_tab, m, d_pts, N, d_out, ostride, ooff, st, split_scratch, perm);
    }
    return launch_mfma_nf<NT, WIDE, 4>(h, frag_tab, m, d_pts, N, d_out, ostride, ooff, st, split_scratch, perm);
}

static int launch_rows(pcx_bary *h, const DerivedTensor &dt, const double *d_pts, long N,
                       double *d_out, long ostride, long ooff, hipStream_t st, const int *perm) {
    int ppw = 256 / h->lpp;
    size_t lds = (size_t)ppw * h->dims.sum_n * sizeof(double);
    if (lds > 160 * 1024) return fail(PCX_ERR_UNSUPPORTED, "sum of node counts %d too large for the rows kernel", h->dims.sum_n);
    if (lds > 64 * 1024)
        HIP_TRY(hipFuncSetAttribute((const void *)k_bary_rows, hipFuncAttributeMaxDynamicSharedMemorySize, (int)lds));
    long blocks = (N + ppw - 1) / ppw;
    if (blocks > 0x7fffffffL) return fail(PCX_ERR_UNSUPPORTED, "batch too large for one launch");
    hipLaunchKernelGGL(k_bary_rows, dim3((unsigned)blocks), dim3(256), lds, st, h->dims, h->lpp,
                       h->d_nodes, h->d_wts, dt.plain, d_pts, d_out, N, ostride, ooff, perm);
    HIP_TRY(hipGetLastError());
    return PCX_OK;
}

template <int DOUT, int NLP>
static int launch_small_t(pcx_bary *h, const DerivedTensor &dt, const double *const *T_tab, int m, const double *d_pts,
                          long N, double *d_out, long ostride, long ooff, hipStream_t st, const int *perm) {
    auto kern = k_bary_small<DOUT, NLP>;
    size_t lds = (size_t)(h->dims.sum_n - h->dims.n[DOUT]) * 64 * sizeof(double);
    if (lds > 64 * 1024)
        HIP_TRY(hipFuncSetAttribute((const void *)kern, hipFuncAttributeMaxDynamicSharedMemorySize, (int)lds));
    long blocks = (N + 63) / 64;
    if (blocks > 0x7fffffffL) return fail(PCX_ERR_UNSUPPORTED, "batch too large for one launch");
    hipLaunchKernelGGL(kern, dim3((unsigned)blocks), dim3(64), lds, st, h->dims, h->small_scale, h->d_snodes, h->d_nodes,
                       h->d_wts, dt.plain, T_tab, m, d_pts, d_out, N, ostride, ooff, perm);
    HIP_TRY(hipGetLastError());
    return PCX_OK;
}

template <int DOUT>
static int launch_small_d(pcx_bary *h, const DerivedTensor &dt, const double *const *T_tab, int m, const double *d_pts,
                          long N, double *d_out, long ostride, long ooff, hipStream_t st, const int *perm) {
    switch (h->small_nlp) {
#define CASE_NLP(v) case v: return launch_small_t<DOUT, v>(h, dt, T_tab, m, d_pts, N, d_out, ostride, ooff, st, perm);
    CASE_NLP(2) CASE_NLP(3) CASE_NLP(4) CASE_NLP(5) CASE_NLP(6) CASE_NLP(7) CASE_NLP(8) CASE_NLP(9) CASE_NLP(10) CASE_NLP(11)
    CASE_NLP(12) CASE_NLP(13) CASE_NLP(14) CASE_NLP(15) CASE_NLP(16) CASE_NLP(24) CASE_NLP(32) CASE_NLP(48) CASE_NLP(64)
#undef CASE_NLP
    }
    return fail(PCX_ERR_UNSUPPORTED, "lane-per-point kernel does not cover this shape");
}

static int launch_small(pcx_bary *h, const DerivedTensor &dt, const double *const *T_tab, int m, const double *d_pts,
                        long N, double *d_out, long ostride, long ooff, hipStream_t st, const int *perm) {
    switch (h->dims.d) {
    case 1: return launch_small_d<0>(h, dt, T_tab, m, d_pts, N, d_out, ostride, ooff, st, perm);
    case 2: return launch_small_d<1>(h, dt, T_tab, m, d_pts, N, d_out, ostride, ooff, st, perm);
    case 3: return launch_small_d<2>(h, dt, T_tab, m, d_pts, N, d_out, ostride, ooff, st, perm);
    case 4: return launch_small_d<3>(h, dt, T_tab, m, d_pts, N, d_out, ostride, ooff, st, perm);
    }
    return fail(PCX_ERR_UNSUPPORTED, "lane-per-point kernel does not cover this shape");
}


template <int NL>
static int launch_sq_t(pcx_bary *h, const DerivedTensor &dt, const double *const *T_tab, int m, const double *d_pts,
                       long N, double *d_out, long ostride, long ooff, hipStream_t st, const int *perm) {
    const int d = h->dims.d;
    size_t lds = 0;
    for (int k = 0; k < d - 2; ++k) lds += (size_t)h->dims.n[k] * 64 * sizeof(double);
    long blocks = (N + 63) / 64;
    if (blocks > 0x7fffffffL) return fail(PCX_ERR_UNSUPPORTED, "batch too large for one launch");
#define PCX_SQ_GO(LEAD)                                                                                               \
    hipLaunchKernelGGL((k_bary_sq<NL, LEAD>), dim3((unsigned)blocks), dim3(64), lds, st, h->dims, h->small_scale,    \
                       h->d_snodes, h->d_nodes, h->d_wts, dt.plain, T_tab, m, d_pts, d_out, N, ostride, ooff, perm)
    if (d == 2) PCX_SQ_GO(0);
    else if (d == 3) PCX_SQ_GO(1);
    else PCX_SQ_GO(2);
#undef PCX_SQ_GO
    HIP_TRY(hipGetLastError());
    return PCX_OK;
}

static int launch_sq(pcx_bary *h, const DerivedTensor &dt, const double *const *T_tab, int m, const double *d_pts,
                     long N, double *d_out, long ostride, long ooff, hipStream_t st, const int *perm) {
    switch (h->sq_nl) {
#define CASE_NL(v) case v: return launch_sq_t<v>(h, dt, T_tab, m, d_pts, N, d_out, ostride, ooff, st, perm);
    CASE_NL(4) CASE_NL(5) CASE_NL(6) CASE_NL(7) CASE_NL(8) CASE_NL(9) CASE_NL(10) CASE_NL(11) CASE_NL(12) CASE_NL(13)
    CASE_NL(14) CASE_NL(15) CASE_NL(16) CASE_NL(17) CASE_NL(18) CASE_NL(19) CASE_NL(20) CASE_NL(21) CASE_NL(22)
    CASE_NL(23) CASE_NL(24) CASE_NL(26) CASE_NL(28) CASE_NL(30) CASE_NL(32)
#undef CASE_NL
    }
    return fail(PCX_ERR_UNSUPPORTED, "square-trailing lane-per-point kernel does not cover this shape");
}

static int bary_pack_g0(pcx_bary *h, DerivedTensor &dt) {
    if (dt.frag_g0) return PCX_OK;
    const BaryMfmaPlan &p = h->plan;
    const int n0 = h->dims.n[0];
    const size_t cnt = (size_t)n0 * h->g0_tps * p.KS * 64;
    DevBuf frag, slot;
    int rc = frag.alloc(cnt * sizeof(double));
    if (rc) return rc;
    hipLaunchKernelGGL(k_pack_fragments_slabs, dim3((unsigned)((cnt + 255) / 256)), dim3(256), 0, h->stream, dt.plain,
                       frag.as<double>(), n0, p.M / n0, p.K, h->g0_tps, p.KS);
    HIP_TRY(hipGetLastError());
    if ((rc = slot.alloc(sizeof(double *)))) return rc;
    double *fp = frag.as<double>();
    HIP_TRY(hipMemcpy(slot.p, &fp, sizeof(double *), hipMemcpyHostToDevice));
    HIP_TRY(hipStreamSynchronize(h->stream));
    dt.frag_g0 = frag.release<double>();
    dt.slot_g0 = slot.release<double *>();
    return PCX_OK;
}

template <int KS, int NF>
static int launch_g0_t(pcx_bary *h, const DerivedTensor &base, const BaryG0 &gs, const double *d_pts, long N, double *d_out,
                       long ostride, long ooff, hipStream_t st) {
    auto kern = k_bary_mfma<KS, 2, false, NF, true>;
    const size_t lds = mfma_lds_bytes(h->dims, 2);
    if (lds > 64 * 1024)
        HIP_TRY(hipFuncSetAttribute((const void *)kern, hipFuncAttributeMaxDynamicSharedMemorySize, (int)lds));
    const long blocks = (N + 127) / 128;
    if (blocks > 0x7fffffffL) return fail(PCX_ERR_UNSUPPORTED, "batch too large for one launch");
    BaryMfmaPlan plan = h->plan;
    plan.MT = gs.tps * gs.n0;
    const int nchunks = (plan.MT + PCX_CHUNK_TILES - 1) / PCX_CHUNK_TILES;
    hipLaunchKernelGGL(kern, dim3((unsigned)blocks, 1, 1), dim3(256), lds, st, h->dims, plan, h->d_nodes, h->d_wts,
                       (const double *const *)base.slot_g0, h->d_rowcode_g0, h->d_kcode, nullptr, nullptr, d_pts, d_out, N,
                       ostride, ooff, nchunks, nullptr, nullptr, gs, h->d_diff + h->doff[0]);
    HIP_TRY(hipGetLastError());
    return PCX_OK;
}

template <int NF>
static int launch_g0_nf(pcx_bary *h, const DerivedTensor &base, const BaryG0 &gs, const double *d_pts, long N, double *d_out,
                        long ostride, long ooff, hipStream_t st) {
    switch (h->plan.KS) {
#define CASE_KS(v) case v: return launch_g0_t<v, NF>(h, base, gs, d_pts, N, d_out, ostride, ooff, st);
        CASE_KS(1) CASE_KS(2) CASE_KS(3) CASE_KS(4) CASE_KS(5) CASE_KS(6) CASE_KS(7) CASE_KS(8)
        CASE_KS(9) CASE_KS(10) CASE_KS(11) CASE_KS(12) CASE_KS(13) CASE_KS(14) CASE_KS(15) CASE_KS(16)
        CASE_KS(17) CASE_KS(18) CASE_KS(19) CASE_KS(20) CASE_KS(21) CASE_KS(22) CASE_KS(23) CASE_KS(24)
        CASE_KS(25) CASE_KS(26) CASE_KS(27) CASE_KS(28) CASE_KS(29) CASE_KS(30) CASE_KS(31) CASE_KS(32)
#undef CASE_KS
    }
    return fail(PCX_ERR_UNSUPPORTED, "no dim-0 group instantiation for KS=%d", h->plan.KS);
}

static const long kG0MinPoints = 65536;

PCX_HIDDEN int bary_effective_variant(const pcx_bary *h) {
    if (h->variant != 0) return h->variant;
    if (h->sq_nl && h->sq_preferred) return 5;
    return (h->small_nlp && (h->small_preferred || !h->mfma_ok)) ? 4 : (h->mfma_ok ? 2 : 1);
}

PCX_HIDDEN int bary_launch(pcx_bary *h, DerivedTensor *const *dts, int m, const double *const *frag_tab,
                       const double *d_pts, long N, double *d_out, long ostride, long ooff,
                       hipStream_t st, Scratch *split_scratch, const int *perm) {
    if (N == 0) return PCX_OK;
    const int variant = bary_effective_variant(h);
    if (variant == 4) {
        if (!h->small_nlp) return fail(PCX_ERR_UNSUPPORTED, "lane-per-point kernel does not cover this shape");
        return launch_small(h, *dts[0], m > 1 ? frag_tab : nullptr, m, d_pts, N, d_out, ostride, ooff, st, perm);
    }
    if (variant == 5) {
        if (!h->sq_nl) return fail(PCX_ERR_UNSUPPORTED, "square-trailing lane-per-point kernel does not cover this shape");
        return launch_sq(h, *dts[0], m > 1 ? frag_tab : nullptr, m, d_pts, N, d_out, ostride, ooff, st, perm);
    }
    if (variant == 3) {
        if (!h->mfma4_ok) return fail(PCX_ERR_UNSUPPORTED, "4x4x4 MFMA kernel does not cover this shape");
        return launch_mfma4(h, frag_tab, m, d_pts, N, d_out, ostride, ooff, st, perm);
    }
    if (variant == 2) {
        if (!h->mfma_ok) return fail(PCX_ERR_UNSUPPORTED, "MFMA kernel does not cover this shape");
        if (h->kfold_ok) return bary_launch_kfold(h, frag_tab, m, d_pts, N, d_out, ostride, ooff, st, perm);
        if (h->grid_ok) return bary_launch_grid(h, frag_tab, m, d_pts, N, d_out, ostride, ooff, st, split_scratch, perm);
        int nt = (N >= 65536) ? h->nt : 1;
        if (h->wide)
            return nt == 2 ? launch_mfma_nt<2, true>(h, frag_tab, m, d_pts, N, d_out, ostride, ooff, st, split_scratch, perm)
                           : launch_mfma_nt<1, true>(h, frag_tab, m, d_pts, N, d_out, ostride, ooff, st, split_scratch, perm);
        return nt == 2 ? launch_mfma_nt<2, false>(h, frag_tab, m, d_pts, N, d_out, ostride, ooff, st, split_scratch, perm)
                       : launch_mfma_nt<1, false>(h, frag_tab, m, d_pts, N, d_out, ostride, ooff, st, split_scratch, perm);
    }
    for (int s = 0; s < m; ++s) {
        int rc = launch_rows(h, *dts[s], d_pts, N, d_out, ostride, ooff + s, st, perm);
        if (rc) return rc;
    }
    return PCX_OK;
}

static const long kRotMaxElems = 1L << 24;
static pcx_bary *bary_rot(pcx_bary *h, int q) {
    if (h->rot_state[q]) return h->rot[q];
    h->rot_state[q] = 2;
    const int d = h->dims.d;
    if (q < 1 || q >= d || h->total > kRotMaxElems || h->dims.n[q] < 2 || h->dims.n[q] > 16) return nullptr;
    const long sum_n = h->dims.sum_n;
    long sum_n2 = 0;
    for (int k = 0; k < d; ++k) sum_n2 += (long)h->dims.n[k] * h->dims.n[k];
    std::vector<double> nodes((size_t)sum_n), wts((size_t)sum_n), diff((size_t)sum_n2), T((size_t)h->total), TR((size_t)h->total);
    const DerivedTensor &val = h->cache[std::vector<int>(d, 0)];
    if (hipMemcpy(nodes.data(), h->d_nodes, sum_n * sizeof(double), hipMemcpyDeviceToHost) != hipSuccess ||
        hipMemcpy(wts.data(), h->d_wts, sum_n * sizeof(double), hipMemcpyDeviceToHost) != hipSuccess ||
        hipMemcpy(diff.data(), h->d_diff, sum_n2 * sizeof(double), hipMemcpyDeviceToHost) != hipSuccess ||
        hipMemcpy(T.data(), val.plain, h->total * sizeof(double), hipMemcpyDeviceToHost) != hipSuccess) {
        (void)hipGetLastError();
        return nullptr;
    }
    int pd[PCX_MAX_DIMS];
    pd[0] = q;
    for (int k = 0, c = 1; k < d; ++k)
        if (k != q) pd[c++] = k;
    std::vector<int32_t> nn(d);
    std::vector<double> rn, rw, rd;
    long stride[PCX_MAX_DIMS];
    { long acc = 1; for (int k = d - 1; k >= 0; --k) { stride[k] = acc; acc *= h->dims.n[k]; } }
    for (int c = 0; c < d; ++c) {
        const int k = pd[c], n = h->dims.n[k];
        nn[c] = n;
        rn.insert(rn.end(), nodes.begin() + h->dims.off[k], nodes.begin() + h->dims.off[k] + n);
        rw.insert(rw.end(), wts.begin() + h->dims.off[k], wts.begin() + h->dims.off[k] + n);
        rd.insert(rd.end(), diff.begin() + h->doff[k], diff.begin() + h->doff[k] + (long)n * n);
    }
    {
        int idx[PCX_MAX_DIMS] = {};
        long src = 0;
        for (long e = 0; e < h->total; ++e) {
            TR[(size_t)e] = T[(size_t)src];
            for (int c = d - 1; c >= 0; --c) {
                src += stride[pd[c]];
                if (++idx[c] < nn[c]) break;
                src -= stride[pd[c]] * nn[c];
                idx[c] = 0;
            }
        }
    }
    pcx_bary *r = nullptr;
    if (pcx_bary_create(h->device, d, nn.data(), rn.data(), rw.data(), rd.data(), TR.data(), &r) != PCX_OK || !r) return nullptr;
    if (!r->g0_ok) { pcx_bary_destroy(r); return nullptr; }
    h->rot[q] = r;
    h->rot_state[q] = 1;
    return r;
}

static int bary_launch_group(pcx_bary *h, int q, const int32_t *lower, const int *rel, const int *col, int nmem,
                             const double *pp, long N, double *d_out, long ostride, long ooff, hipStream_t st) {
    const int d = h->dims.d;
    pcx_bary *g = q == 0 ? h : h->rot[q];
    std::vector<int32_t> bspec(d);
    if (q == 0) bspec.assign(lower, lower + d);
    else { bspec[0] = lower[q]; for (int k = 0, c = 1; k < d; ++k) if (k != q) bspec[c++] = lower[k]; }
    if (g != h) g->call_mark = g->clock;
    DerivedTensor *base = nullptr;
    int rc = bary_get_tensor(g, bspec.data(), &base);
    if (rc) return rc;
    if ((rc = bary_pack_g0(g, *base))) return rc;
    BaryG0 gs{};
    gs.nmem = nmem;
    gs.tps = g->g0_tps;
    gs.n0 = g->dims.n[0];
    for (int i = 0; i < nmem; ++i) {
        gs.order[i] = rel[i];
        gs.col[i] = col[i];
        gs.maxorder = std::max(gs.maxorder, rel[i]);
    }
    return (g->g0_nf == 2) ? launch_g0_nf<2>(g, *base, gs, pp, N, d_out, ostride, ooff, st)
                           : launch_g0_nf<3>(g, *base, gs, pp, N, d_out, ostride, ooff, st);
}

static const int kProbePoints = 2048;
static double bary_pair_deviation(pcx_bary *h, const std::vector<int> &lower, int q) {
    std::vector<int> key = lower;
    key.push_back(q);
    auto it = h->pair_dev.find(key);
    if (it != h->pair_dev.end()) return it->second;
    struct Forget {
        pcx_bary *h; const std::vector<int> &key; bool keep = false;
        ~Forget() {
            if (keep) return;
            h->pair_dev.erase(key);
            (void)hipGetLastError();
            if (getenv("PCX_BARY_PROBE_LOG")) fprintf(stderr, "[pcx] pair probe could not run: not cached, retried by the next call\n");
        }
    } forget{h, key};
    double &dev = h->pair_dev[key];
    dev = INFINITY;
    const int d = h->dims.d;
    std::vector<double> nodes((size_t)h->dims.sum_n);
    if (hipMemcpy(nodes.data(), h->d_nodes, nodes.size() * sizeof(double), hipMemcpyDeviceToHost) != hipSuccess) return dev;
    std::vector<double> lo(d), hi(d);
    for (int k = 0; k < d; ++k) {
        const int n = h->dims.n[k];
        const double a = nodes[h->dims.off[k]], b = nodes[h->dims.off[k] + n - 1];
        const double half = n > 1 ? 0.5 * (b - a) / std::cos(3.14159265358979323846 / (2.0 * n)) : 0.0;
        lo[k] = 0.5 * (a + b) - half;
        hi[k] = 0.5 * (a + b) + half;
    }
    const long N = kProbePoints;
    std::vector<double> P((size_t)N * d);
    uint64_t state = 0x9E3779B97F4A7C15ull;
    auto rnd = [&]() { state = state * 6364136223846793005ull + 1442695040888963407ull; return (uint32_t)(state >> 33); };
    for (long p = 0; p < N; ++p) {
        const int mode = (int)(p % 4);
        for (int k = 0; k < d; ++k) {
            const uint32_t r = rnd();
            const double uni = lo[k] + (hi[k] - lo[k]) * ((double)(r >> 8) / 8388608.0);
            const int pick = mode == 0 ? 2 : (mode == 1 ? (int)(r & 1) : (int)(r % 3));
            P[(size_t)p * d + k] = pick == 0 ? lo[k] : (pick == 1 ? hi[k] : uni);
        }
    }
    DevBuf dp, dr, dout;
    if (dp.alloc(P.size() * sizeof(double)) || dr.alloc(P.size() * sizeof(double)) || dout.alloc((size_t)N * 2 * sizeof(double))) return dev;
    if (hipMemcpy(dp.p, P.data(), P.size() * sizeof(double), hipMemcpyHostToDevice) != hipSuccess) return dev;
    const double *gp = dp.as<double>();
    if (q > 0) {
        SliderCols cols{};
        cols.nc = d;
        cols.col[0] = q;
        for (int k = 0, c = 1; k < d; ++k)
            if (k != q) cols.col[c++] = k;
        hipLaunchKernelGGL(k_gather_columns, dim3((unsigned)((N * d + 255) / 256)), dim3(256), 0, h->stream, dp.as<double>(), N, d,
                           cols, dr.as<double>());
        gp = dr.as<double>();
    }
    std::vector<int32_t> lspec(lower.begin(), lower.end()), uspec(lower.begin(), lower.end());
    ++uspec[q];
    const int rel = 1, col = 0;
    if (bary_launch_group(h, q, lspec.data(), &rel, &col, 1, gp, N, dout.as<double>(), 2, 0, h->stream)) return dev;
    DerivedTensor *own = nullptr;
    if (bary_get_tensor(h, uspec.data(), &own)) return dev;
    DerivedTensor *one[1] = {own};
    if (bary_launch(h, one, 1, own->slot, dp.as<double>(), N, dout.as<double>(), 2, 1, h->stream, &h->s_partial)) return dev;
    std::vector<double> R((size_t)N * 2);
    if (hipStreamSynchronize(h->stream) != hipSuccess ||
        hipMemcpy(R.data(), dout.p, R.size() * sizeof(double), hipMemcpyDeviceToHost) != hipSuccess) {
        (void)hipGetLastError();
        return dev;
    }
    double scale = 0.0, diff = 0.0;
    for (long p = 0; p < N; ++p) {
        scale = std::max(scale, std::fabs(R[2 * p + 1]));
        diff = std::max(diff, std::fabs(R[2 * p] - R[2 * p + 1]));
    }
    if (std::isfinite(diff) && std::isfinite(scale)) dev = scale > 0.0 ? diff / scale : (diff == 0.0 ? 0.0 : INFINITY);
    forget.keep = true;
    static const bool log = getenv("PCX_BARY_PROBE_LOG") != nullptr;
    if (log) {
        fprintf(stderr, "[pcx] pair probe (");
        for (int k = 0; k < d; ++k) fprintf(stderr, "%d%s", lower[k], k + 1 < d ? "," : "");
        fprintf(stderr, ") + e_%d out of one GEMM: %.3g of the scale from its own GEMM (tolerance %.3g)\n", q, dev, h->group_tol);
    }
    return dev;
}

struct BaryGroup { int q; int base; std::vector<int> members; };

static void bary_plan_groups(pcx_bary *h, const int32_t *derivs, int m, long N, bool own_stream, std::vector<BaryGroup> &subs,
                             std::vector<char> &grouped) {
    const int d = h->dims.d;
    grouped.assign(m, 0);
    const int span = h->g0_span;
    if (!(span > 0 && derivs && m > 1 && N >= kG0MinPoints && bary_effective_variant(h) == 2)) return;
    auto spec = [&](int s) { return std::vector<int>(derivs + (size_t)s * d, derivs + (size_t)(s + 1) * d); };
    if (span >= 2 && h->g0_ok) {
        std::map<std::vector<int>, std::vector<int>> by_key;
        for (int s = 0; s < m; ++s)
            by_key[std::vector<int>(derivs + (size_t)s * d + 1, derivs + (size_t)(s + 1) * d)].push_back(s);
        for (auto &kv : by_key) {
            std::vector<int> &mem = kv.second;
            if (mem.size() < 2) continue;
            std::sort(mem.begin(), mem.end(), [&](int a, int b) {
                const int oa = derivs[(size_t)a * d], ob = derivs[(size_t)b * d];
                return oa != ob ? oa < ob : a < b;
            });
            for (size_t i = 0; i < mem.size();) {
                const int base = derivs[(size_t)mem[i] * d];
                size_t e = i;
                while (e < mem.size() && derivs[(size_t)mem[e] * d] <= base + span && e - i < PCX_G0_MAX) ++e;
                if (e - i >= 2) {
                    subs.push_back(BaryGroup{0, base, std::vector<int>(mem.begin() + i, mem.begin() + e)});
                    for (size_t q = i; q < e; ++q) grouped[mem[q]] = 1;
                }
                i = e;
            }
        }
    }
    std::map<std::vector<int>, int> first;
    std::vector<int> by_order;
    for (int s = 0; s < m; ++s)
        if (!grouped[s] && first.emplace(spec(s), s).second) by_order.push_back(s);
    auto total_order = [&](int s) { int t = 0; for (int k = 0; k < d; ++k) t += derivs[(size_t)s * d + k]; return t; };
    std::stable_sort(by_order.begin(), by_order.end(), [&](int a, int b) { return total_order(a) > total_order(b); });
    for (int b : by_order) {
        if (grouped[b]) continue;
        std::vector<int> lower = spec(b);
        for (int q = 0; q < d; ++q) {
            if (lower[q] < 1) continue;
            --lower[q];
            auto it = first.find(lower);
            ++lower[q];
            if (it == first.end() || grouped[it->second]) continue;
            if (q == 0 ? !h->g0_ok : !(own_stream && bary_rot(h, q))) continue;
            --lower[q];
            const double dev = bary_pair_deviation(h, lower, q);
            ++lower[q];
            if (!(dev <= h->group_tol)) continue;
            subs.push_back(BaryGroup{q, lower[q] - 1, {it->second, b}});
            grouped[it->second] = grouped[b] = 1;
            break;
        }
    }
}

static int bary_launch_specs(pcx_bary *h, const int32_t *derivs, DerivedTensor *const *dts, int m,
                             const double *const *frag_tab, const double *d_pts, long N, double *d_out, long ostride,
                             long ooff, hipStream_t st, Scratch *split_scratch, long N_call = -1) {
    const int d = h->dims.d;
    std::vector<BaryGroup> subs;
    std::vector<char> grouped;
    const bool own_stream = st == h->stream || (h->stage.second && st == h->stage.second);
    bary_plan_groups(h, derivs, m, N_call > 0 ? N_call : N, own_stream, subs, grouped);
    for (int s = 0; s < m;) {
        if (grouped[s]) { ++s; continue; }
        int e = s;
        while (e < m && !grouped[e]) ++e;
        int rc = bary_launch(h, dts + s, e - s, (e - s == 1) ? (const double *const *)dts[s]->slot : frag_tab + s, d_pts, N,
                             d_out, ostride, ooff + s, st, split_scratch);
        if (rc) return rc;
        s = e;
    }
    const double *rpts[PCX_MAX_DIMS] = {};
    {
        int nq = 0;
        for (const BaryGroup &sub : subs)
            if (sub.q > 0 && !rpts[sub.q]) { rpts[sub.q] = d_pts; ++nq; }
        if (nq) {
            Scratch &sc = (h->stage.second && st == h->stage.second) ? h->s_rot2 : h->s_rot;
            int rc = sc.reserve((size_t)nq * N * d * sizeof(double));
            if (rc) return rc;
            double *dst = (double *)sc.ptr;
            for (int q = 1; q < d; ++q) {
                if (!rpts[q]) continue;
                SliderCols cols{};
                cols.nc = d;
                cols.col[0] = q;
                for (int k = 0, c = 1; k < d; ++k)
                    if (k != q) cols.col[c++] = k;
                const long elems = N * d;
                hipLaunchKernelGGL(k_gather_columns, dim3((unsigned)((elems + 255) / 256)), dim3(256), 0, st, d_pts, N, d, cols, dst);
                HIP_TRY(hipGetLastError());
                rpts[q] = dst;
                dst += (size_t)N * d;
            }
        }
    }
    for (const BaryGroup &sub : subs) {
        std::vector<int32_t> lower(derivs + (size_t)sub.members[0] * d, derivs + (size_t)(sub.members[0] + 1) * d);
        lower[sub.q] = sub.base;
        int rel[PCX_G0_MAX], col[PCX_G0_MAX];
        const int nmem = (int)sub.members.size();
        for (int i = 0; i < nmem; ++i) {
            rel[i] = derivs[(size_t)sub.members[i] * d + sub.q] - sub.base;
            col[i] = sub.members[i];
        }
        int rc = bary_launch_group(h, sub.q, lower.data(), rel, col, nmem, sub.q == 0 ? d_pts : rpts[sub.q], N, d_out, ostride,
                                   ooff, st);
        if (rc) return rc;
    }
    return PCX_OK;
}

extern "C" int pcx_bary_count_gemms(pcx_bary *h, const int32_t *derivs, int m, int64_t N, int32_t *gemms_out) {
    PCX_API_BEGIN
    if (!h || !derivs || !gemms_out || m < 1) return fail(PCX_ERR_INVALID, "bad argument");
    HIP_TRY(hipSetDevice(h->device));
    std::lock_guard<std::mutex> lk(h->mu);
    std::vector<BaryGroup> subs;
    std::vector<char> grouped;
    bary_plan_groups(h, derivs, m, (long)N, true, subs, grouped);
    int count = (int)subs.size();
    for (int s = 0; s < m; ++s) count += !grouped[s];
    *gemms_out = count;
    return PCX_OK;
    PCX_API_END
}

extern "C" int pcx_bary_eval_batch_dev(pcx_bary *h, const double *d_pts, int64_t N,
                                       const int32_t *deriv, double *d_out, void *stream) {
    PCX_API_BEGIN
    if (!h) return fail(PCX_ERR_INVALID, "handle is NULL");
    if (N < 0) return fail(PCX_ERR_INVALID, "N=%lld < 0", (long long)N);
    if (N > 0 && (!d_pts || !d_out)) return fail(PCX_ERR_INVALID, "NULL device buffer");
    HIP_TRY(hipSetDevice(h->device));
    std::lock_guard<std::mutex> lk(h->mu);
    h->call_mark = h->clock;
    DerivedTensor *dt = nullptr;
    int rc = bary_get_tensor(h, deriv, &dt);
    if (rc) return rc;
    hipStream_t st = stream ? (hipStream_t)stream : h->stream;
    return bary_launch(h, &dt, 1, dt->slot, d_pts, (long)N, d_out, 1, 0, st,
                       st == h->stream ? &h->s_partial : nullptr);
    PCX_API_END
}

PCX_HIDDEN int bary_spec_tensors(pcx_bary *h, const int32_t *derivs, int m, std::vector<DerivedTensor *> &dts,
                                 const double *const **frag_tab) {
    const int d = h->dims.d;
    dts.resize(m);
    for (int s = 0; s < m; ++s) {
        int rc = bary_get_tensor(h, derivs ? derivs + (size_t)s * d : nullptr, &dts[s]);
        if (rc) return rc;
    }
    *frag_tab = dts[0]->slot;
    const int eff = bary_effective_variant(h);
    if (m > 1 && (eff == 4 || eff == 5 || h->mfma_ok)) {
        std::vector<double *> tab(m);
        for (int s = 0; s < m; ++s) tab[s] = (eff == 4 || eff == 5) ? dts[s]->plain : dts[s]->frag;
        if (tab != h->tab_host) {
            HIP_TRY(hipDeviceSynchronize());
            HIP_TRY(hipMemcpy(h->d_tab, tab.data(), m * sizeof(double *), hipMemcpyHostToDevice));
            h->tab_host = tab;
        }
        *frag_tab = h->d_tab;
    }
    return PCX_OK;
}

extern "C" int pcx_bary_eval_multi_batch_dev(pcx_bary *h, const double *d_pts, int64_t N, const int32_t *derivs,
                                             int m, double *d_out, void *stream) {
    PCX_API_BEGIN
    if (!h) return fail(PCX_ERR_INVALID, "handle is NULL");
    if (N < 0 || m < 1) return fail(PCX_ERR_INVALID, "bad N or m");
    if (!derivs) return fail(PCX_ERR_INVALID, "derivs is NULL");
    if (N == 0) return PCX_OK;
    if (!d_pts || !d_out) return fail(PCX_ERR_INVALID, "NULL device buffer");
    HIP_TRY(hipSetDevice(h->device));
    std::lock_guard<std::mutex> lk(h->mu);
    h->call_mark = h->clock;
    const int d = h->dims.d;
    hipStream_t st = stream ? (hipStream_t)stream : h->stream;
    for (int s0 = 0; s0 < m; s0 += kMaxSpecs) {
        const int mc = std::min(kMaxSpecs, m - s0);
        std::vector<DerivedTensor *> dts;
        const double *const *frag_tab = nullptr;
        int rc = bary_spec_tensors(h, derivs + (size_t)s0 * d, mc, dts, &frag_tab);
        if (rc) return rc;
        rc = bary_launch_specs(h, derivs + (size_t)s0 * d, dts.data(), mc, frag_tab, d_pts, (long)N, d_out, m, s0, st,
                               st == h->stream ? &h->s_partial : nullptr);
        if (rc) return rc;
    }
    return PCX_OK;
    PCX_API_END
}

static int bary_eval_host(pcx_bary *h, const double *pts, int64_t N, const int32_t *derivs, int m,
                          double *out, int64_t N_call = -1) {
    if (N_call < N) N_call = N;
    if (!h) return fail(PCX_ERR_INVALID, "handle is NULL");
    if (N < 0 || m < 1) return fail(PCX_ERR_INVALID, "bad N or m");
    if (N > 0 && (!pts || !out)) return fail(PCX_ERR_INVALID, "NULL buffer");
    if (m > kMaxSpecs)
        return eval_spec_groups(N, derivs, h->dims.d, m, out, [&](const int32_t *group, int mc, double *part) {
            return bary_eval_host(h, pts, N, group, mc, part, N_call);
        });
    HIP_TRY(hipSetDevice(h->device));
    std::lock_guard<std::mutex> lk(h->mu);
    h->call_mark = h->clock;
    const int d = h->dims.d;
    std::vector<DerivedTensor *> dts;
    const double *const *frag_tab = nullptr;
    int rc = bary_spec_tensors(h, derivs, m, dts, &frag_tab);
    if (rc) return rc;
    const int64_t piece = std::min<int64_t>((int64_t)1 << 21, std::max<int64_t>(kPipeChunkPoints, (((int64_t)10 << 20) / (d * 8)) & ~(int64_t)65535));
    const StagePlan plan = N >= 2 * piece ? StagePlan{1 << 16, piece, true, true} : StagePlan{kChunkPoints, kChunkPoints, false, true};
    return stage_host_batch(h->stage, h->device, h->stream, pts, N, d, m, out, plan,
                            [&](int slot, hipStream_t st, const double *dp, long cnt, double *dout) {
                                return bary_launch_specs(h, derivs, dts.data(), m, frag_tab, dp, cnt, dout, m, 0, st,
                                                         slot ? nullptr : &h->s_partial, (long)N_call);
                            });
}

extern "C" int pcx_bary_eval_batch(pcx_bary *h, const double *pts, int64_t N, const int32_t *deriv,
                                   double *out) {
    PCX_API_BEGIN
    return bary_eval_host(h, pts, N, deriv, 1, out);
    PCX_API_END
}

extern "C" int pcx_bary_eval_multi_batch(pcx_bary *h, const double *pts, int64_t N,
                                         const int32_t *derivs, int m, double *out) {
    PCX_API_BEGIN
    if (!derivs) return fail(PCX_ERR_INVALID, "derivs is NULL");
    return bary_eval_host(h, pts, N, derivs, m, out);
    PCX_API_END
}

template <int DOUT, int NLP>
static void launch_small_pieces_t(const pcx_bary *p0, const SplinePieceModel *models, const int *blk_piece,
                                  const int *blk_first, const int *piece_end, int m, long blocks, const double *dp,
                                  double *dout, const int *perm, hipStream_t st) {
    auto kern = k_bary_small_pieces<DOUT, NLP>;
    const size_t lds = (size_t)(p0->dims.sum_n - p0->dims.n[DOUT]) * 64 * sizeof(double);
    if (lds > 64 * 1024)
        (void)hipFuncSetAttribute((const void *)kern, hipFuncAttributeMaxDynamicSharedMemorySize, (int)lds);
    hipLaunchKernelGGL(kern, dim3((unsigned)blocks), dim3(64), lds, st, p0->dims, models, blk_piece, blk_first, piece_end, m,
                       dp, dout, (long)m, 0L, perm);
}

template <int DOUT>
static int launch_small_pieces_d(const pcx_bary *p0, const SplinePieceModel *models, const int *blk_piece,
                                 const int *blk_first, const int *piece_end, int m, long blocks, const double *dp,
                                 double *dout, const int *perm, hipStream_t st) {
    switch (p0->small_nlp) {
#define CASE_NLP(v) case v: launch_small_pieces_t<DOUT, v>(p0, models, blk_piece, blk_first, piece_end, m, blocks, dp, dout, perm, st); return PCX_OK;
    CASE_NLP(2) CASE_NLP(3) CASE_NLP(4) CASE_NLP(5) CASE_NLP(6) CASE_NLP(7) CASE_NLP(8) CASE_NLP(9) CASE_NLP(10) CASE_NLP(11)
    CASE_NLP(12) CASE_NLP(13) CASE_NLP(14) CASE_NLP(15) CASE_NLP(16) CASE_NLP(24) CASE_NLP(32) CASE_NLP(48) CASE_NLP(64)
#undef CASE_NLP
    }
    return fail(PCX_ERR_UNSUPPORTED, "lane-per-point kernel does not cover this shape");
}

template <int NL>
static int launch_sq_pieces_t(const pcx_bary *p0, const SplinePieceModel *models, const int *blk_piece, const int *blk_first,
                              const int *piece_end, int m, long blocks, const double *dp, double *dout, const int *perm,
                              hipStream_t st) {
    const int d = p0->dims.d;
    size_t lds = 0;
    for (int k = 0; k < d - 2; ++k) lds += (size_t)p0->dims.n[k] * 64 * sizeof(double);
#define PCX_SQP_GO(LEAD)                                                                                              \
    hipLaunchKernelGGL((k_bary_sq_pieces<NL, LEAD>), dim3((unsigned)blocks), dim3(64), lds, st, p0->dims, models, blk_piece, \
                       blk_first, piece_end, m, dp, dout, (long)m, 0L, perm)
    if (d == 2) PCX_SQP_GO(0);
    else if (d == 3) PCX_SQP_GO(1);
    else PCX_SQP_GO(2);
#undef PCX_SQP_GO
    return PCX_OK;
}

PCX_HIDDEN int bary_launch_sq_pieces(const pcx_bary *p0, const SplinePieceModel *models, const int *blk_piece, const int *blk_first,
                            const int *piece_end, int m, long blocks, const double *dp, double *dout, const int *perm,
                            hipStream_t st) {
    switch (p0->sq_nl) {
#define CASE_NL(v) case v: return launch_sq_pieces_t<v>(p0, models, blk_piece, blk_first, piece_end, m, blocks, dp, dout, perm, st);
    CASE_NL(4) CASE_NL(5) CASE_NL(6) CASE_NL(7) CASE_NL(8) CASE_NL(9) CASE_NL(10) CASE_NL(11) CASE_NL(12) CASE_NL(13)
    CASE_NL(14) CASE_NL(15) CASE_NL(16) CASE_NL(17) CASE_NL(18) CASE_NL(19) CASE_NL(20) CASE_NL(21) CASE_NL(22)
    CASE_NL(23) CASE_NL(24) CASE_NL(26) CASE_NL(28) CASE_NL(30) CASE_NL(32)
#undef CASE_NL
    }
    return fail(PCX_ERR_UNSUPPORTED, "square-trailing lane-per-point kernel does not cover this piece shape");
}
PCX_HIDDEN int bary_launch_small_pieces(int dout, const pcx_bary *p0, const SplinePieceModel *models, const int *blk_piece,
                                        const int *blk_first, const int *piece_end, int m, long blocks, const double *dp,
                                        double *dout_buf, const int *perm, hipStream_t st) {
    switch (dout) {
    case 0: return launch_small_pieces_d<0>(p0, models, blk_piece, blk_first, piece_end, m, blocks, dp, dout_buf, perm, st);
    case 1: return launch_small_pieces_d<1>(p0, models, blk_piece, blk_first, piece_end, m, blocks, dp, dout_buf, perm, st);
    case 2: return launch_small_pieces_d<2>(p0, models, blk_piece, blk_first, piece_end, m, blocks, dp, dout_buf, perm, st);
    case 3: return launch_small_pieces_d<3>(p0, models, blk_piece, blk_first, piece_end, m, blocks, dp, dout_buf, perm, st);
    }
    return fail(PCX_ERR_UNSUPPORTED, "lane-per-point kernel covers d <= 4");
}

extern "C" int pcx_bary_group_eval_multi_batch(pcx_bary *const *handles, int n_handles, const double *pts, int64_t N,
                                               const int32_t *derivs, int m, double *out, int pin) {
    PCX_API_BEGIN
    if (!handles || n_handles < 1) return fail(PCX_ERR_INVALID, "no handles");
    for (int g = 0; g < n_handles; ++g) {
        if (!handles[g]) return fail(PCX_ERR_INVALID, "handle %d is NULL", g);
        if (handles[g]->dims.d != handles[0]->dims.d || handles[g]->total != handles[0]->total)
            return fail(PCX_ERR_INVALID, "handle %d holds a different model", g);
    }
    if (N < 0 || m < 1) return fail(PCX_ERR_INVALID, "bad N or m");
    if (N > 0 && (!pts || !out)) return fail(PCX_ERR_INVALID, "NULL buffer");
    const int d = handles[0]->dims.d;
    return fan_out_host(n_handles, handles[0]->device, pin, N, pts, (size_t)N * d * sizeof(double), out,
                        (size_t)N * m * sizeof(double), [&](int g, int64_t lo, int64_t cnt) {
                            return bary_eval_host(handles[g], pts + (size_t)lo * d, cnt, derivs, m, out + (size_t)lo * m, N);
                        });
    PCX_API_END
}

extern "C" int pcx_bary_derivative_tensor(pcx_bary *h, const int32_t *deriv, double *tensor_out) {
    PCX_API_BEGIN
    if (!h || !tensor_out) return fail(PCX_ERR_INVALID, "NULL argument");
    HIP_TRY(hipSetDevice(h->device));
    std::lock_guard<std::mutex> lk(h->mu);
    h->call_mark = h->clock;
    DerivedTensor *dt = nullptr;
    int rc = bary_get_tensor(h, deriv, &dt);
    if (rc) return rc;
    HIP_TRY(hipStreamSynchronize(h->stream));
    HIP_TRY(hipMemcpy(tensor_out, dt->plain, h->total * sizeof(double), hipMemcpyDeviceToHost));
    return PCX_OK;
    PCX_API_END
}

static int bary_cheb_matrices(pcx_bary *h) {
    if (h->d_cheb) return PCX_OK;
    const int d = h->dims.d;
    std::vector<double> M((size_t)h->doff[d - 1] + (size_t)h->dims.n[d - 1] * h->dims.n[d - 1]);
    for (int k = 0; k < d; ++k) {
        const long n = h->dims.n[k];
        double *Mk = M.data() + h->doff[k];
        for (long m = 0; m < n; ++m)
            for (long i = 0; i < n; ++i) {
                const long p = (m * (2 * (n - 1 - i) + 1)) % (4 * n);
                Mk[m * n + i] = (2.0 / (double)n) * std::cos(M_PI * (double)p / (2.0 * (double)n)) * (m == 0 ? 0.5 : 1.0);
            }
    }
    DevBuf b;
    int rc = b.alloc(M.size() * sizeof(double));
    if (rc) return rc;
    HIP_TRY(hipMemcpy(b.p, M.data(), M.size() * sizeof(double), hipMemcpyHostToDevice));
    h->d_cheb = b.release<double>();
    return PCX_OK;
}

static int bary_cheb_coeffs(pcx_bary *h, const double **coeffs) {
    int rc = bary_cheb_matrices(h);
    if (rc) return rc;
    DerivedTensor *base = nullptr;
    if ((rc = bary_get_tensor(h, nullptr, &base))) return rc;
    for (Scratch &sc : h->s_cheb)
        if ((rc = sc.reserve((size_t)h->total * sizeof(double)))) return rc;
    const int d = h->dims.d;
    const double *src = base->plain;
    double *dst = (double *)h->s_cheb[0].ptr, *other = (double *)h->s_cheb[1].ptr;
    const int blocks = (int)((h->total + 255) / 256);
    for (int k = 0; k < d; ++k) {
        long outer = 1, inner = 1;
        for (int q = 0; q < k; ++q) outer *= h->dims.n[q];
        for (int q = k + 1; q < d; ++q) inner *= h->dims.n[q];
        hipLaunchKernelGGL(k_mode_product, dim3(blocks), dim3(256), 0, h->stream, src, dst, h->d_cheb + h->doff[k], outer,
                           h->dims.n[k], inner);
        src = dst;
        std::swap(dst, other);
    }
    HIP_TRY(hipGetLastError());
    *coeffs = src;
    return PCX_OK;
}

extern "C" int pcx_bary_chebyshev_coefficients(pcx_bary *h, double *coeffs_out) {
    PCX_API_BEGIN
    if (!h || !coeffs_out) return fail(PCX_ERR_INVALID, "NULL argument");
    HIP_TRY(hipSetDevice(h->device));
    std::lock_guard<std::mutex> lk(h->mu);
    h->call_mark = h->clock;
    const double *coeffs = nullptr;
    int rc = bary_cheb_coeffs(h, &coeffs);
    if (rc) return rc;
    HIP_TRY(hipMemcpyAsync(coeffs_out, coeffs, (size_t)h->total * sizeof(double), hipMemcpyDeviceToHost, h->stream));
    HIP_TRY(hipStreamSynchronize(h->stream));
    return PCX_OK;
    PCX_API_END
}

extern "C" int pcx_bary_sobol(pcx_bary *h, double *variance_out, double *first_out, double *total_out) {
    PCX_API_BEGIN
    if (!h || !variance_out || !first_out || !total_out) return fail(PCX_ERR_INVALID, "NULL argument");
    HIP_TRY(hipSetDevice(h->device));
    std::lock_guard<std::mutex> lk(h->mu);
    h->call_mark = h->clock;
    const int d = h->dims.d;
    SobolDims sd{};
    sd.L = h->dims.n[d - 1];
    sd.rows = h->total / sd.L;
    int W = 1;
    while (W < 64 && W < sd.L) W <<= 1;
    for (sd.lw = 0; (1 << sd.lw) < W; ++sd.lw) {}
    for (int k = 0; k < PCX_MAX_DIMS; ++k) sd.n[k] = k < d ? (unsigned)h->dims.n[k] : 1u;
    sd.pid = 1.0;
    for (int k = 0; k < d; ++k) sd.pid *= M_PI;
    const long per_block = (long)(PCX_SOBOL_THREADS / 64) * (64 / W) * PCX_SOBOL_UNROLL;
    const int blocks = (int)std::min<long>(PCX_SOBOL_MAX_BLOCKS, (sd.rows + per_block - 1) / per_block);
    const int S = PCX_SOBOL_SLOTS(d);
    int rc = h->s_sobol.reserve(((size_t)blocks + 1) * S * sizeof(double));
    if (rc) return rc;
    double *slab = (double *)h->s_sobol.ptr, *res = slab + (size_t)blocks * S;
    const double *coeffs = nullptr;
    if ((rc = bary_cheb_coeffs(h, &coeffs))) return rc;
    const bool narrow = sd.rows <= 0xffffffffL;
    switch (d) {
#define CASE_D(v)                                                                                                        \
    case v:                                                                                                              \
        if (narrow) hipLaunchKernelGGL((k_sobol_energy<v, unsigned>), dim3(blocks), dim3(PCX_SOBOL_THREADS), 0, h->stream, \
                                       coeffs, slab, sd);                                                   \
        else hipLaunchKernelGGL((k_sobol_energy<v, unsigned long long>), dim3(blocks), dim3(PCX_SOBOL_THREADS), 0,       \
                                h->stream, coeffs, slab, sd);                                               \
        break;
        CASE_D(1) CASE_D(2) CASE_D(3) CASE_D(4) CASE_D(5) CASE_D(6) CASE_D(7) CASE_D(8)
        CASE_D(9) CASE_D(10) CASE_D(11) CASE_D(12) CASE_D(13) CASE_D(14) CASE_D(15) CASE_D(16)
#undef CASE_D
        default: return fail(PCX_ERR_INVALID, "d=%d outside [1, %d]", d, PCX_MAX_DIMS);
    }
    hipLaunchKernelGGL(k_sobol_finish, dim3(1), dim3(PCX_SOBOL_FINISH_THREADS), 0, h->stream,
                       (const double *)slab, blocks, S, res);
    HIP_TRY(hipGetLastError());
    double r[PCX_SOBOL_SLOTS(PCX_MAX_DIMS)];
    HIP_TRY(hipMemcpyAsync(r, res, (size_t)S * sizeof(double), hipMemcpyDeviceToHost, h->stream));
    HIP_TRY(hipStreamSynchronize(h->stream));
    if (r[S - 1] != 0.0)
        return fail(PCX_ERR_INVALID, "coefficients contain NaN or Inf; sobol_indices() requires finite spectral coefficients");
    const double var = r[0];
    for (int k = 0; k < d; ++k) {
        if (d == 1) {
            first_out[k] = total_out[k] = var > 0.0 ? 1.0 : 0.0;
        } else if (var == 0.0) {
            first_out[k] = total_out[k] = 0.0;
        } else {
            first_out[k] = r[1 + k] / var;
            total_out[k] = r[1 + d + k] / var;
        }
    }
    *variance_out = var;
    return PCX_OK;
    PCX_API_END
}

extern "C" int pcx_tensor_contract_axis(int device, int d, const int32_t *n_nodes, const double *tensor,
                                        int axis, const double *vec, double *out) {
    PCX_API_BEGIN
    if (d < 1 || d > PCX_MAX_DIMS || !n_nodes || !tensor || !vec || !out) return fail(PCX_ERR_INVALID, "bad argument");
    if (axis < 0 || axis >= d) return fail(PCX_ERR_INVALID, "axis %d outside [0, %d)", axis, d);
    long outer = 1, inner = 1;
    for (int k = 0; k < d; ++k) {
        if (n_nodes[k] < 1) return fail(PCX_ERR_INVALID, "n_nodes[%d] < 1", k);
        if (k < axis) outer *= n_nodes[k];
        if (k > axis) inner *= n_nodes[k];
    }
    const int na = n_nodes[axis];
    int rc = use_device(device);
    if (rc) return rc;
    DevBuf din, dvec, dout;
    HIP_TRY(hipMalloc(&din.p, (size_t)outer * na * inner * sizeof(double)));
    HIP_TRY(hipMalloc(&dvec.p, (size_t)na * sizeof(double)));
    HIP_TRY(hipMalloc(&dout.p, (size_t)outer * inner * sizeof(double)));
    HIP_TRY(hipMemcpy(din.p, tensor, (size_t)outer * na * inner * sizeof(double), hipMemcpyHostToDevice));
    HIP_TRY(hipMemcpy(dvec.p, vec, (size_t)na * sizeof(double), hipMemcpyHostToDevice));
    long cnt = outer * inner;
    hipLaunchKernelGGL(k_contract_axis, dim3((unsigned)((cnt + 255) / 256)), dim3(256), 0, 0, (const double *)din.p,
                       (double *)dout.p, (const double *)dvec.p, outer, na, inner);
    HIP_TRY(hipGetLastError());
    HIP_TRY(hipMemcpy(out, dout.p, (size_t)cnt * sizeof(double), hipMemcpyDeviceToHost));
    return PCX_OK;
    PCX_API_END
}

extern "C" int pcx_bary_set_kernel(pcx_bary *h, int variant) {
    PCX_API_BEGIN
    if (!h) return fail(PCX_ERR_INVALID, "handle is NULL");
    if (variant < 0 || variant > 5) return fail(PCX_ERR_INVALID, "variant %d outside [0, 5]", variant);
    if (variant == 4 && !h->small_nlp) return fail(PCX_ERR_UNSUPPORTED, "lane-per-point kernel does not cover this shape");
    if (variant == 5 && !h->sq_nl) return fail(PCX_ERR_UNSUPPORTED, "square-trailing lane-per-point kernel does not cover this shape");
    if (variant == 2 && !h->mfma_ok) return fail(PCX_ERR_UNSUPPORTED, "MFMA kernel does not cover this shape");
    if (variant == 3 && !h->mfma4_ok) return fail(PCX_ERR_UNSUPPORTED, "4x4x4 MFMA kernel does not cover this shape");
    std::lock_guard<std::mutex> lk(h->mu);
    h->variant = variant;
    return PCX_OK;
    PCX_API_END
}

extern "C" int pcx_bary_set_group_span(pcx_bary *h, int span) {
    PCX_API_BEGIN
    if (!h) return fail(PCX_ERR_INVALID, "handle is NULL");
    if (span < 0 || span > 8) return fail(PCX_ERR_INVALID, "span %d outside [0, 8]", span);
    std::lock_guard<std::mutex> lk(h->mu);
    h->g0_span = span;
    return PCX_OK;
    PCX_API_END
}

extern "C" int pcx_bary_set_group_tolerance(pcx_bary *h, double tol) {
    PCX_API_BEGIN
    if (!h) return fail(PCX_ERR_INVALID, "handle is NULL");
    if (!(tol >= 0.0)) return fail(PCX_ERR_INVALID, "tolerance must be >= 0");
    std::lock_guard<std::mutex> lk(h->mu);
    h->group_tol = tol;
    return PCX_OK;
    PCX_API_END
}

extern "C" int pcx_bary_kernel_info(pcx_bary *h, int32_t *info) {
    PCX_API_BEGIN
    if (!h || !info) return fail(PCX_ERR_INVALID, "NULL argument");
    { const int keep = h->variant; h->variant = 0; info[0] = bary_effective_variant(h); h->variant = keep; }
    info[1] = h->mfma_ok ? (h->kfold_ok ? h->kf.MT : (h->grid_ok ? h->gp.MT : h->plan.MT)) : 0;
    info[2] = h->mfma_ok ? (h->kfold_ok ? h->kf.nbody * h->kf.P : h->plan.KS) : 0;
    info[3] = h->mfma_ok ? (int32_t)(h->kfold_ok ? bary_kfold_lds_bytes(h->kf, h->nt)
                                                  : (h->grid_ok ? bary_grid_lds_bytes(h, h->nt) : mfma_lds_bytes(h->dims, h->nt)))
                         : (256 / h->lpp) * h->dims.sum_n * 8;
    info[4] = h->mfma_ok ? 64 * h->nt : 256 / h->lpp;
    info[5] = h->mfma_ok ? h->plan.split : h->dims.d - 1;
    return PCX_OK;
    PCX_API_END
}

extern "C" int pcx_bary_grid_info(pcx_bary *h, int32_t *info) {
    PCX_API_BEGIN
    if (!h || !info) return fail(PCX_ERR_INVALID, "NULL argument");
    info[0] = h->grid_ok ? 1 : (h->kfold_ok ? 2 : 0);
    info[1] = h->grid_ok ? h->gp.RA : 0;
    info[2] = h->grid_ok ? h->gp.MT : (h->kfold_ok ? h->kf.MT : 0);
    info[3] = h->grid_ok ? h->gp.nchunks : (h->kfold_ok ? h->kf.KS2 : 0);
    return PCX_OK;
    PCX_API_END
}

extern "C" int pcx_bary_stream(pcx_bary *h, void **stream) {
    PCX_API_BEGIN
    if (!h || !stream) return fail(PCX_ERR_INVALID, "NULL argument");
    *stream = (void *)h->stream;
    return PCX_OK;
    PCX_API_END
}
```

### pychebyshev_amd/csrc/pcx_bary_internal.h

```cpp
#pragma once

#include "pcx_internal.h"

static int alloc_plain(DevBuf &b, long total) {
    int rc = b.alloc(((size_t)total + PCX_PLAIN_PAD) * sizeof(double));
    if (rc) return rc;
    HIP_TRY(hipMemset((char *)b.p + (size_t)total * sizeof(double), 0, PCX_PLAIN_PAD * sizeof(double)));
    return PCX_OK;
}

struct DerivedTensor {
    double *plain = nullptr;
    double *frag = nullptr;
    double **slot = nullptr;
    double *frag_g0 = nullptr;
    double **slot_g0 = nullptr;
    uint64_t last_use = 0;
    void free_all() {
        if (plain) (void)hipFree(plain);
        if (frag) (void)hipFree(frag);
        if (slot) (void)hipFree(slot);
        if (frag_g0) (void)hipFree(frag_g0);
        if (slot_g0) (void)hipFree(slot_g0);
        plain = frag = frag_g0 = nullptr;
        slot = slot_g0 = nullptr;
    }
};

struct pcx_bary {
    int device = 0;
    hipStream_t stream = nullptr;
    BaryDims dims;
    long total = 0;
    std::vector<int> doff;
    double *d_nodes = nullptr, *d_wts = nullptr, *d_diff = nullptr;
    double *d_cheb = nullptr;
    Scratch s_cheb[2];
    Scratch s_sobol;
    bool mfma_ok = false;
    BaryMfmaPlan plan;
    int nt = 2;
    unsigned *d_rowcode = nullptr, *d_kcode = nullptr;
    unsigned *d_rowcode_hi = nullptr, *d_kcode_hi = nullptr;
    bool wide = false;
    bool grid_ok = false;
    BaryGridPlan gp;
    double *d_gsnodes = nullptr;
    bool kfold_ok = false;
    BaryKfoldPlan kf;
    bool grid_prod = false;
    bool g0_ok = false;
    int g0_tps = 0;
    int g0_nf = 2;
    unsigned *d_rowcode_g0 = nullptr;
    int g0_span = 1;
    pcx_bary *rot[PCX_MAX_DIMS] = {};
    char rot_state[PCX_MAX_DIMS] = {};
    Scratch s_rot, s_rot2;
    std::map<std::vector<int>, double> pair_dev;
    double group_tol = 3e-13;
    int lpp = 64;
    bool mfma4_ok = false;
    int small_nlp = 0;
    std::vector<double> dom_lo, dom_hi;
    BarySmallScale small_scale;
    double *d_snodes = nullptr;
    bool small_preferred = false;
    int sq_nl = 0;
    bool sq_preferred = false;
    int variant = 0;
    std::mutex mu;
    std::map<std::vector<int>, DerivedTensor> cache;
    uint64_t clock = 0;
    uint64_t call_mark = 0;
    HostStage stage;
    double **d_tab = nullptr;
    std::vector<double *> tab_host;
    Scratch s_partial;
};

static const int kMaxSpecs = 64;

template <typename Fn>
static int eval_spec_groups(int64_t N, const int32_t *derivs, int d, int m, double *out, Fn &&eval) {
    if (!derivs) return fail(PCX_ERR_INVALID, "derivs is NULL");
    std::vector<double> part;
    for (int s0 = 0; s0 < m; s0 += kMaxSpecs) {
        const int mc = std::min(kMaxSpecs, m - s0);
        part.resize((size_t)N * mc);
        int rc = eval(derivs + (size_t)s0 * d, mc, part.data());
        if (rc) return rc;
        for (int64_t i = 0; i < N; ++i)
            memcpy(out + (size_t)i * m + s0, part.data() + (size_t)i * mc, (size_t)mc * sizeof(double));
    }
    return PCX_OK;
}

PCX_HIDDEN bool bary_plan_grid(const BaryDims &dm, const BaryMfmaPlan &plan, BaryGridPlan &gp);
PCX_HIDDEN int bary_pack_grid(pcx_bary *h, const double *plain, double *frag);
PCX_HIDDEN size_t bary_grid_lds_bytes(const pcx_bary *h, int nt);
PCX_HIDDEN long bary_plan_kfold(const BaryDims &dm, BaryKfoldPlan &kp);
PCX_HIDDEN long bary_kfold_estimate(const BaryKfoldPlan &kp, long eff);
PCX_HIDDEN bool bary_kfold_take(const BaryKfoldPlan &kp, long eff, long grid_eff, int grid_ks);
PCX_HIDDEN size_t bary_kfold_frag_count(const BaryKfoldPlan &kp);
PCX_HIDDEN size_t bary_kfold_lds_bytes(const BaryKfoldPlan &kp, int nt);
PCX_HIDDEN int bary_pack_kfold(pcx_bary *h, const double *plain, double *frag);
PCX_HIDDEN int bary_launch_kfold(pcx_bary *h, const double *const *frag_tab, int m, const double *d_pts, long N, double *d_out,
                                 long ostride, long ooff, hipStream_t st, const int *perm);
PCX_HIDDEN int bary_launch_grid(pcx_bary *h, const double *const *frag_tab, int m, const double *d_pts, long N, double *d_out,
                                long ostride, long ooff, hipStream_t st, Scratch *split_scratch, const int *perm);

PCX_HIDDEN int bary_get_tensor(pcx_bary *h, const int32_t *deriv, DerivedTensor **out);
PCX_HIDDEN int bary_spec_tensors(pcx_bary *h, const int32_t *derivs, int m, std::vector<DerivedTensor *> &dts,
                                 const double *const **frag_tab);
PCX_HIDDEN int bary_effective_variant(const pcx_bary *h);
PCX_HIDDEN int bary_launch(pcx_bary *h, DerivedTensor *const *dts, int m, const double *const *frag_tab,
                           const double *d_pts, long N, double *d_out, long ostride, long ooff, hipStream_t st,
                           Scratch *split_scratch, const int *perm = nullptr);
PCX_HIDDEN int bary_launch_small_pieces(int dout, const pcx_bary *p0, const SplinePieceModel *models, const int *blk_piece,
                                        const int *blk_first, const int *piece_end, int m, long blocks, const double *dp,
                                        double *dout_buf, const int *perm, hipStream_t st);
PCX_HIDDEN int bary_launch_sq_pieces(const pcx_bary *p0, const SplinePieceModel *models, const int *blk_piece, const int *blk_first,
                                     const int *piece_end, int m, long blocks, const double *dp, double *dout, const int *perm,
                                     hipStream_t st);
```

### pychebyshev_amd/csrc/pcx_common.h

```cpp
#pragma once

#include <hip/hip_runtime.h>
#include <stdint.h>

#include "../../include/pcx.h"

#define PCX_WAVE 64

typedef double pcx_d4 __attribute__((ext_vector_type(4)));

#define PCX_MAX_PART_ROWS 255
#define PCX_CODE_FIELDS 4

struct BaryDims {
    int d;
    int sum_n;
    int n[PCX_MAX_DIMS];
    int off[PCX_MAX_DIMS];
};

struct BaryMfmaPlan {
    int split;
    int M;
    int K;
    int MT;
    int KS;
    int tail_base;
    int rows;
};

struct BaryGridPlan {
    int RA;
    int gbs;
    int nA, nB;
    int TA, TB;
    int rowA, rowB;
    int nouter;
    int no1;
    int rowo0, rowo1;
    int nchunks;
    int hrows;
    int trows;
    int af;
    int wpb;
    int MT;
};

#define PCX_KFOLD_PAD 16
struct BaryKfoldPlan {
    int dim[3];
    long stride[3];
    int n0, n1, n2;
    int MT;
    int KS2;
    int trows;
    int str;
    int P;
    int nbody;
};

#define PCX_G0_MAX 9
struct BaryG0 {
    int nmem;
    int maxorder;
    int tps;
    int n0;
    int order[PCX_G0_MAX];
    int col[PCX_G0_MAX];
};

#define PCX_PLAIN_PAD 64

struct BarySmallScale {
    double s[4];
};

struct SplinePieceModel {
    const double *snodes, *nodes, *wts;
    const double *T;
    const double *const *T_tab;
    BarySmallScale sc;
};

struct TTDims {
    int d;
    int n[PCX_MAX_DIMS];
    int col[PCX_MAX_DIMS];
    double lo[PCX_MAX_DIMS];
    double hi[PCX_MAX_DIMS];
    double scale[PCX_MAX_DIMS];
    long frag_off[PCX_MAX_DIMS];
};
```

Before: 202.1 million point-evals/s.

## Seed MFMA accumulators with leftover K columns instead of zero-padding the last k-step

When K is not a multiple of 4, the R leftover columns (K mod 4) are packed into a separate seed array and folded into the accumulators with scalar FMAs before each tile's MFMA chain. Previously they were zero-padded into an extra MFMA k-step. This removes the padded k-step and its fragment loads, and in the pipelined path the seed load is prefetched alongside the next tile. The cost is extra register state, new R-templated kernel instantiations split across separate translation units, and a more complex pack layout.

Measured after the change: 206.3 million point-evals/s, median of 6. +2.1%, better.

```diff
diff --git a/pychebyshev_amd/_build.py b/pychebyshev_amd/_build.py
--- a/pychebyshev_amd/_build.py
+++ b/pychebyshev_amd/_build.py
@@ -13,7 +13,9 @@
 HOST_H = ["pcx_common.h", "pcx_internal.h", PCX_H]
 SOURCES = {
     "pcx_core.hip": HOST_H,
-    "pcx_bary.hip": HOST_H + ["pcx_bary_internal.h", "bary_kernels.h", "gather_kernels.h", "sobol_kernels.h"],
+    "pcx_bary.hip": HOST_H + ["pcx_bary_internal.h", "bary_kernels.h", "bary_mfma_launch.h", "gather_kernels.h", "sobol_kernels.h"],
+    "pcx_bary_seed1.hip": HOST_H + ["pcx_bary_internal.h", "bary_kernels.h", "bary_mfma_launch.h"],
+    "pcx_bary_seed2.hip": HOST_H + ["pcx_bary_internal.h", "bary_kernels.h", "bary_mfma_launch.h"],
     "pcx_bary_grid.hip": HOST_H + ["pcx_bary_internal.h", "bary_grid_kernels.h", "bary_weights.h"],
     "pcx_bary_kfold.hip": HOST_H + ["pcx_bary_internal.h", "bary_kfold_kernels.h"],
     "pcx_spline.hip": HOST_H + ["pcx_bary_internal.h", "gather_kernels.h", "route_kernels.h"],
diff --git a/pychebyshev_amd/csrc/bary_kernels.h b/pychebyshev_amd/csrc/bary_kernels.h
--- a/pychebyshev_amd/csrc/bary_kernels.h
+++ b/pychebyshev_amd/csrc/bary_kernels.h
@@ -2,7 +2,7 @@
 
 #include "pcx_common.h"
 
-__global__ void k_mode_product(const double *__restrict__ in, double *__restrict__ out,
+static __global__ void k_mode_product(const double *__restrict__ in, double *__restrict__ out,
                                const double *__restrict__ D, long outer, int na, long inner) {
     long idx = (long)blockIdx.x * blockDim.x + threadIdx.x;
     long total = outer * na * inner;
@@ -18,7 +18,7 @@
     out[idx] = s;
 }
 
-__global__ void k_contract_axis(const double *__restrict__ in, double *__restrict__ out,
+static __global__ void k_contract_axis(const double *__restrict__ in, double *__restrict__ out,
                                 const double *__restrict__ vec, long outer, int na, long inner) {
     long idx = (long)blockIdx.x * blockDim.x + threadIdx.x;
     if (idx >= outer * inner) return;
@@ -30,8 +30,8 @@
     out[idx] = s;
 }
 
-__global__ void k_pack_fragments(const double *__restrict__ T2, double *__restrict__ frag, int M,
-                                 int K, int MT, int KS) {
+static __global__ void k_pack_fragments(const double *__restrict__ T2, double *__restrict__ frag, int M,
+                                 int K, int MT, int KS, int R) {
     long idx = (long)blockIdx.x * blockDim.x + threadIdx.x;
     long total = (long)MT * KS * 64;
     if (idx >= total) return;
@@ -40,12 +40,25 @@
     int s = (int)(ts % KS);
     int t = (int)(ts / KS);
     int m = 16 * t + (l & 15);
-    int k = 4 * s + (l >> 4);
+    int k = R + 4 * s + (l >> 4);
     frag[idx] = (m < M && k < K) ? T2[(long)m * K + k] : 0.0;
 }
 
-__global__ void k_pack_fragments_slabs(const double *__restrict__ T3, double *__restrict__ frag, int n0, int M1,
-                                       int K, int tps, int KS) {
+static __global__ void k_pack_seed(const double *__restrict__ T2, double *__restrict__ seed, int M, int K, int MT, int R, int tps) {
+    long idx = (long)blockIdx.x * blockDim.x + threadIdx.x;
+    if (idx >= (long)MT * 16 * R) return;
+    const int j = (int)(idx & 3);
+    const int r = (int)((idx >> 2) % R);
+    const long tg = (idx >> 2) / R;
+    const int g = (int)(tg & 3);
+    const long t = tg >> 2;
+    const long slab = tps > 0 ? t / tps : 0;
+    const int m = 16 * (int)(tps > 0 ? t % tps : t) + g + 4 * j;
+    seed[idx] = m < M ? T2[(slab * M + m) * K + r] : 0.0;
+}
+
+static __global__ void k_pack_fragments_slabs(const double *__restrict__ T3, double *__restrict__ frag, int n0, int M1,
+                                       int K, int tps, int KS, int R) {
     long idx = (long)blockIdx.x * blockDim.x + threadIdx.x;
     const long per_slab = (long)tps * KS * 64;
     if (idx >= per_slab * n0) return;
@@ -56,7 +69,7 @@
     int s = (int)(ts % KS);
     int t = (int)(ts / KS);
     int m = 16 * t + (l & 15);
-    int k = 4 * s + (l >> 4);
+    int k = R + 4 * s + (l >> 4);
     frag[idx] = (m < M1 && k < K) ? T3[((long)i0 * M1 + m) * K + k] : 0.0;
 }
 
@@ -118,6 +131,17 @@
     return pcx_u4{{q.x, q.y, q.z, q.w}};
 }
 
+typedef const pcx_d4 __attribute__((address_space(1))) *pcx_seed_ptr;
+template <int R>
+struct pcx_seed { pcx_d4 v[R > 0 ? R : 1]; };
+template <int R>
+__device__ __forceinline__ pcx_seed<R> load_seed(pcx_seed_ptr seed, long t, int g) {
+    pcx_seed<R> q;
+#pragma unroll
+    for (int r = 0; r < R; ++r) q.v[r] = seed[(4 * t + g) * R + r];
+    return q;
+}
+
 template <int NF>
 __device__ __forceinline__ double code_weight_t(unsigned code, const double *bw_col, int PW) {
     if constexpr (NF >= 4) return code_weight(code, bw_col, PW);
@@ -131,7 +155,7 @@
 
 #define PCX_CHUNK_TILES 4
 
-template <int KS, int NT, bool WIDE, int NF = 4, bool G0 = false>
+template <int KS, int NT, bool WIDE, int NF = 4, bool G0 = false, int R = 0>
 __global__ void __launch_bounds__(256, 2)
 k_bary_mfma(BaryDims dims, BaryMfmaPlan plan, const double *__restrict__ nodes,
             const double *__restrict__ wts, const double *const *__restrict__ frag_tab,
@@ -153,6 +177,7 @@
     const long base = ((long)blockIdx.x * 4 + wave) * PW;
     typedef const double __attribute__((address_space(1))) *gptr_t;
     const gptr_t frag = (gptr_t)frag_tab[blockIdx.z];
+    const pcx_seed_ptr seed = (pcx_seed_ptr)(frag + (size_t)plan.MT * KS * 64);
     const int nchunks = (plan.MT + PCX_CHUNK_TILES - 1) / PCX_CHUNK_TILES;
     const int ch0 = blockIdx.y * chunks_per_split;
     const int ch1 = (ch0 + chunks_per_split < nchunks) ? ch0 + chunks_per_split : nchunks;
@@ -188,6 +213,18 @@
             for (int nt = 0; nt < NT; ++nt) B[nt][s] *= code_weight(hi, bwt + 16 * nt + c, PW);
         }
     }
+    double ws[NT][R > 0 ? R : 1];
+#pragma unroll
+    for (int r = 0; r < R; ++r) {
+        unsigned code = kcode[4 * KS + r];
+#pragma unroll
+        for (int nt = 0; nt < NT; ++nt) ws[nt][r] = code_weight(code, bwt + 16 * nt + c, PW);
+        if (WIDE) {
+            unsigned hi = kcode_hi[4 * KS + r];
+#pragma unroll
+            for (int nt = 0; nt < NT; ++nt) ws[nt][r] *= code_weight(hi, bwt + 16 * nt + c, PW);
+        }
+    }
 
     double total[NT], cs[NT];
 #pragma unroll
@@ -200,9 +237,22 @@
     constexpr int DEPTH = 6;
     unsigned cn[4] = {0u, 0u, 0u, 0u}, cnh[4] = {0u, 0u, 0u, 0u};
     double head[DEPTH];
+    pcx_d4 acc[NT];
+    auto seed_acc = [&](const pcx_seed<R> &sd) {
+#pragma unroll
+        for (int nt = 0; nt < NT; ++nt) acc[nt] = (pcx_d4){0.0, 0.0, 0.0, 0.0};
+#pragma unroll
+        for (int r = 0; r < R; ++r)
+#pragma unroll
+            for (int nt = 0; nt < NT; ++nt)
+#pragma unroll
+                for (int j = 0; j < 4; ++j) acc[nt][j] = __builtin_fma(sd.v[r][j], ws[nt][r], acc[nt][j]);
+    };
+    constexpr bool CARRY = PIPELINED && R > 0;
 #pragma unroll
     for (int i = 0; i < DEPTH; ++i) head[i] = 0.0;
     if (PIPELINED && t_begin < t_end) {
+        if constexpr (R > 0) seed_acc(load_seed<R>(seed, t_begin, g));
         {
             const pcx_u4 q = load_row_codes(rowcode, t_begin, g);
             pcx_u4 qh = q;
@@ -218,9 +268,11 @@
     }
     for (int t = t_begin; t < t_end; ++t) {
         double w[NT][4];
-        pcx_d4 acc[NT];
-#pragma unroll
-        for (int nt = 0; nt < NT; ++nt) acc[nt] = (pcx_d4){0.0, 0.0, 0.0, 0.0};
+        pcx_seed<R> sdn;
+        if constexpr (!CARRY) {
+            if constexpr (R > 0) sdn = load_seed<R>(seed, t, g);
+            seed_acc(sdn);
+        }
         const gptr_t tt = tf + (size_t)t * KS * 64;
         if constexpr (PIPELINED) {
             const int t_next = (t + 1 < t_end) ? t + 1 : t;
@@ -247,6 +299,9 @@
                 const double a = ring[s % DEPTH];
                 if (s + DEPTH < KS) ring[s % DEPTH] = tt[(s + DEPTH) * 64];
                 else head[s + DEPTH - KS] = tn[(s + DEPTH - KS) * 64];
+                if constexpr (R > 0) {
+                    if (s == KS - DEPTH) sdn = load_seed<R>(seed, t_next, g);
+                }
 #pragma unroll
                 for (int j = 0; j < 4; ++j) {
                     if (s == 2 * j) {
@@ -309,6 +364,7 @@
         for (int nt = 0; nt < NT; ++nt)
 #pragma unroll
             for (int j = 0; j < 4; ++j) cs[nt] = __builtin_fma(acc[nt][j], w[nt][j], cs[nt]);
+        if constexpr (CARRY) seed_acc(sdn);
         if constexpr (G0) {
             if ((t + 1) % gs.tps == 0) {
                 const int i0 = t / gs.tps;
@@ -365,7 +421,7 @@
     }
 }
 
-template <int KS>
+template <int KS, int R = 0>
 __global__ void __launch_bounds__(512, 2)
 k_bary_mfma4(BaryDims dims, BaryMfmaPlan plan, const double *__restrict__ nodes,
              const double *__restrict__ wts, const double *const *__restrict__ frag_tab,
@@ -387,6 +443,7 @@
     const long base = ((long)blockIdx.x * 8 + wave) * PW;
     typedef const double __attribute__((address_space(1))) *gptr_t;
     const gptr_t frag = (gptr_t)frag_tab[blockIdx.z];
+    const pcx_seed_ptr seed = (pcx_seed_ptr)(frag + (size_t)plan.MT * SLAB);
 
     {
         const int pp = lane & 31;
@@ -432,6 +489,13 @@
 #pragma unroll
         for (int nt = 0; nt < NT; ++nt) B[nt][s] = code_weight(code, bwt + 16 * nt + c, PW);
     }
+    double ws[NT][R > 0 ? R : 1];
+#pragma unroll
+    for (int r = 0; r < R; ++r) {
+        unsigned code = kcode[4 * KS + r];
+#pragma unroll
+        for (int nt = 0; nt < NT; ++nt) ws[nt][r] = code_weight(code, bwt + 16 * nt + c, PW);
+    }
 
     double total[NT], cs[NT];
 #pragma unroll
@@ -457,6 +521,8 @@
         }
         const pcx_u4 q4 = load_row_codes(rowcode, t, g);
         const unsigned code0 = q4.v[0], code1 = q4.v[1], code2 = q4.v[2], code3 = q4.v[3];
+        pcx_seed<R> sd;
+        if constexpr (R > 0) sd = load_seed<R>(seed, t, g);
 #pragma unroll
         for (int half = 0; half < 2; ++half) {
             constexpr int DEPTH = (KS < 6) ? KS : 6;
@@ -464,7 +530,11 @@
 #pragma unroll
             for (int r = 0; r < 2; ++r)
 #pragma unroll
-                for (int nt = 0; nt < NT; ++nt) acc[r][nt] = 0.0;
+                for (int nt = 0; nt < NT; ++nt) {
+                    acc[r][nt] = 0.0;
+#pragma unroll
+                    for (int rr = 0; rr < R; ++rr) acc[r][nt] = __builtin_fma(sd.v[rr][2 * half + r], ws[nt][rr], acc[r][nt]);
+                }
             typedef double d2_t __attribute__((ext_vector_type(2)));
             const d2_t *ar = reinterpret_cast<const d2_t *>(cur + aoff + 32 * half);
             d2_t ring[DEPTH];
@@ -510,7 +580,7 @@
     }
 }
 
-__global__ void k_bary_reduce(const double *__restrict__ partial, double *__restrict__ out, long N,
+static __global__ void k_bary_reduce(const double *__restrict__ partial, double *__restrict__ out, long N,
                               int nchunks, int nspec, long ostride, long ooff,
                               const int *__restrict__ perm) {
     long idx = (long)blockIdx.x * blockDim.x + threadIdx.x;
@@ -528,7 +598,7 @@
     out[row * ostride + ooff + z] = (sg[0] + sg[1]) + (sg[2] + sg[3]);
 }
 
-__global__ void __launch_bounds__(256)
+static __global__ void __launch_bounds__(256)
 k_bary_rows(BaryDims dims, int LPP, const double *__restrict__ nodes,
             const double *__restrict__ wts, const double *__restrict__ T,
             const double *__restrict__ pts, double *__restrict__ out, long N, long ostride,
diff --git a/pychebyshev_amd/csrc/bary_mfma_launch.h b/pychebyshev_amd/csrc/bary_mfma_launch.h
--- /dev/null
+++ b/pychebyshev_amd/csrc/bary_mfma_launch.h
@@ -0,0 +1,189 @@
+#pragma once
+
+#include "pcx_bary_internal.h"
+#include "bary_kernels.h"
+
+static size_t mfma4_lds_bytes(const BaryDims &dm, int ks) {
+    return ((size_t)8 * (dm.sum_n + 2) * 32 + (size_t)2 * ks * 64) * sizeof(double);
+}
+
+static size_t mfma_lds_bytes(const BaryDims &dm, int nt) {
+    return (size_t)4 * (dm.sum_n + 2) * 16 * nt * sizeof(double);
+}
+
+template <int KS, int NT, bool WIDE, int NF, int R>
+static int launch_mfma_t(pcx_bary *h, const double *const *frag_tab, int m, const double *d_pts, long N,
+                         double *d_out, long ostride, long ooff, hipStream_t st, Scratch *split_scratch,
+                         const int *perm) {
+    const bool allow_split = split_scratch != nullptr;
+    size_t lds = mfma_lds_bytes(h->dims, NT);
+    auto kern = k_bary_mfma<KS, NT, WIDE, NF, false, R>;
+    if (lds > 64 * 1024)
+        HIP_TRY(hipFuncSetAttribute((const void *)kern, hipFuncAttributeMaxDynamicSharedMemorySize, (int)lds));
+    long per_wg = 4L * 16 * NT;
+    long blocks = (N + per_wg - 1) / per_wg;
+    if (blocks > 0x7fffffffL) return fail(PCX_ERR_UNSUPPORTED, "batch too large for one launch");
+    int nchunks = (h->plan.MT + PCX_CHUNK_TILES - 1) / PCX_CHUNK_TILES;
+    int nsplit = 1, cps = nchunks;
+    const long want = 512;
+    if (allow_split && blocks * m < want && nchunks > 1) {
+        nsplit = (int)std::min<long>(nchunks, (want + blocks * m - 1) / (blocks * m));
+        cps = (nchunks + nsplit - 1) / nsplit;
+        nsplit = (nchunks + cps - 1) / cps;
+    }
+    double *partial = nullptr;
+    if (nsplit > 1) {
+        int rc = split_scratch->reserve((size_t)m * nchunks * 4 * (size_t)N * sizeof(double));
+        if (rc) return rc;
+        partial = (double *)split_scratch->ptr;
+    }
+    hipLaunchKernelGGL(kern, dim3((unsigned)blocks, (unsigned)nsplit, (unsigned)m), dim3(256), lds, st,
+                       h->dims, h->plan, h->d_nodes, h->d_wts, frag_tab, h->d_rowcode, h->d_kcode,
+                       h->d_rowcode_hi, h->d_kcode_hi, d_pts, d_out, N, ostride, ooff, cps, partial, perm, BaryG0{}, nullptr);
+    HIP_TRY(hipGetLastError());
+    if (nsplit > 1) {
+        long cnt = N * m;
+        hipLaunchKernelGGL(k_bary_reduce, dim3((unsigned)((cnt + 255) / 256)), dim3(256), 0, st, partial, d_out,
+                           N, nchunks, m, ostride, ooff, perm);
+        HIP_TRY(hipGetLastError());
+    }
+    return PCX_OK;
+}
+
+template <int KS, int R>
+static int launch_mfma4_t(pcx_bary *h, const double *const *frag_tab, int m, const double *d_pts, long N,
+                          double *d_out, long ostride, long ooff, hipStream_t st, const int *perm) {
+    size_t lds = mfma4_lds_bytes(h->dims, KS);
+    auto kern = k_bary_mfma4<KS, R>;
+    if (lds > 64 * 1024)
+        HIP_TRY(hipFuncSetAttribute((const void *)kern, hipFuncAttributeMaxDynamicSharedMemorySize, (int)lds));
+    long blocks = (N + 255) / 256;
+    if (blocks > 0x7fffffffL) return fail(PCX_ERR_UNSUPPORTED, "batch too large for one launch");
+    hipLaunchKernelGGL(kern, dim3((unsigned)blocks, 1, (unsigned)m), dim3(512), lds, st, h->dims, h->plan,
+                       h->d_nodes, h->d_wts, frag_tab, h->d_rowcode, h->d_kcode, d_pts, d_out, N, ostride, ooff, perm);
+    HIP_TRY(hipGetLastError());
+    return PCX_OK;
+}
+
+#define PCX_CASES_KS_1_32                                                                  \
+    CASE_KS(1) CASE_KS(2) CASE_KS(3) CASE_KS(4) CASE_KS(5) CASE_KS(6) CASE_KS(7) CASE_KS(8) \
+    CASE_KS(9) CASE_KS(10) CASE_KS(11) CASE_KS(12) CASE_KS(13) CASE_KS(14) CASE_KS(15) CASE_KS(16) \
+    CASE_KS(17) CASE_KS(18) CASE_KS(19) CASE_KS(20) CASE_KS(21) CASE_KS(22) CASE_KS(23) CASE_KS(24) \
+    CASE_KS(25) CASE_KS(26) CASE_KS(27) CASE_KS(28) CASE_KS(29) CASE_KS(30) CASE_KS(31) CASE_KS(32)
+
+template <int R>
+static int launch_mfma4(pcx_bary *h, const double *const *frag_tab, int m, const double *d_pts, long N,
+                        double *d_out, long ostride, long ooff, hipStream_t st, const int *perm) {
+    switch (h->plan.KS) {
+#define CASE_KS(v) case v: return launch_mfma4_t<v, R>(h, frag_tab, m, d_pts, N, d_out, ostride, ooff, st, perm);
+        PCX_CASES_KS_1_32
+#undef CASE_KS
+    }
+    return fail(PCX_ERR_UNSUPPORTED, "no MFMA instantiation for KS=%d", h->plan.KS);
+}
+
+template <int NT, bool WIDE, int NF, int R>
+static int launch_mfma_nf(pcx_bary *h, const double *const *frag_tab, int m, const double *d_pts, long N,
+                          double *d_out, long ostride, long ooff, hipStream_t st, Scratch *split_scratch,
+                          const int *perm) {
+    switch (h->plan.KS) {
+#define CASE_KS(v) case v: return launch_mfma_t<v, NT, WIDE, NF, R>(h, frag_tab, m, d_pts, N, d_out, ostride, ooff, st, split_scratch, perm);
+        PCX_CASES_KS_1_32
+#undef CASE_KS
+    }
+    if constexpr (NT == 1) {
+        switch (h->plan.KS) {
+#define CASE_KS(v) case v: return launch_mfma_t<v, 1, WIDE, NF, R>(h, frag_tab, m, d_pts, N, d_out, ostride, ooff, st, split_scratch, perm);
+            CASE_KS(36) CASE_KS(40) CASE_KS(44) CASE_KS(48) CASE_KS(52) CASE_KS(56) CASE_KS(60) CASE_KS(64)
+#undef CASE_KS
+        }
+        if constexpr (R > 0) {
+            if (h->plan.KS == 42)
+                return launch_mfma_t<42, 1, WIDE, NF, R>(h, frag_tab, m, d_pts, N, d_out, ostride, ooff, st, split_scratch, perm);
+        }
+    }
+    if constexpr (NT == 2 && !WIDE) {
+        switch (h->plan.KS) {
+#define CASE_KS(v) case v: return launch_mfma_t<v, 2, WIDE, NF, R>(h, frag_tab, m, d_pts, N, d_out, ostride, ooff, st, split_scratch, perm);
+            CASE_KS(36) CASE_KS(40)
+#undef CASE_KS
+        }
+    }
+    return fail(PCX_ERR_UNSUPPORTED, "no MFMA instantiation for KS=%d, NT=%d", h->plan.KS, NT);
+}
+
+template <int NT, bool WIDE, int R>
+static int launch_mfma_nt(pcx_bary *h, const double *const *frag_tab, int m, const double *d_pts, long N,
+                          double *d_out, long ostride, long ooff, hipStream_t st, Scratch *split_scratch,
+                          const int *perm) {
+    if constexpr (!WIDE) {
+        if (h->plan.split <= 2)
+            return launch_mfma_nf<NT, false, 2, R>(h, frag_tab, m, d_pts, N, d_out, ostride, ooff, st, split_scratch, perm);
+        if (h->plan.split == 3)
+            return launch_mfma_nf<NT, false, 3, R>(h, frag_tab, m, d_pts, N, d_out, ostride, ooff, st, split_scratch, perm);
+    }
+    return launch_mfma_nf<NT, WIDE, 4, R>(h, frag_tab, m, d_pts, N, d_out, ostride, ooff, st, split_scratch, perm);
+}
+
+template <int R>
+static int launch_rowcode(pcx_bary *h, const double *const *frag_tab, int m, const double *d_pts, long N, double *d_out,
+                          long ostride, long ooff, hipStream_t st, Scratch *split_scratch, const int *perm) {
+    int nt = (N >= 65536) ? h->nt : 1;
+    if (h->wide)
+        return nt == 2 ? launch_mfma_nt<2, true, R>(h, frag_tab, m, d_pts, N, d_out, ostride, ooff, st, split_scratch, perm)
+                       : launch_mfma_nt<1, true, R>(h, frag_tab, m, d_pts, N, d_out, ostride, ooff, st, split_scratch, perm);
+    return nt == 2 ? launch_mfma_nt<2, false, R>(h, frag_tab, m, d_pts, N, d_out, ostride, ooff, st, split_scratch, perm)
+                   : launch_mfma_nt<1, false, R>(h, frag_tab, m, d_pts, N, d_out, ostride, ooff, st, split_scratch, perm);
+}
+
+template <int KS, int NF, int R>
+static int launch_g0_t(pcx_bary *h, const DerivedTensor &base, const BaryG0 &gs, const double *d_pts, long N, double *d_out,
+                       long ostride, long ooff, hipStream_t st) {
+    auto kern = k_bary_mfma<KS, 2, false, NF, true, R>;
+    const size_t lds = mfma_lds_bytes(h->dims, 2);
+    if (lds > 64 * 1024)
+        HIP_TRY(hipFuncSetAttribute((const void *)kern, hipFuncAttributeMaxDynamicSharedMemorySize, (int)lds));
+    const long blocks = (N + 127) / 128;
+    if (blocks > 0x7fffffffL) return fail(PCX_ERR_UNSUPPORTED, "batch too large for one launch");
+    BaryMfmaPlan plan = h->plan;
+    plan.MT = gs.tps * gs.n0;
+    const int nchunks = (plan.MT + PCX_CHUNK_TILES - 1) / PCX_CHUNK_TILES;
+    hipLaunchKernelGGL(kern, dim3((unsigned)blocks, 1, 1), dim3(256), lds, st, h->dims, plan, h->d_nodes, h->d_wts,
+                       (const double *const *)base.slot_g0, h->d_rowcode_g0, h->d_kcode, nullptr, nullptr, d_pts, d_out, N,
+                       ostride, ooff, nchunks, nullptr, nullptr, gs, h->d_diff + h->doff[0]);
+    HIP_TRY(hipGetLastError());
+    return PCX_OK;
+}
+
+template <int NF, int R>
+static int launch_g0_nf(pcx_bary *h, const DerivedTensor &base, const BaryG0 &gs, const double *d_pts, long N, double *d_out,
+                        long ostride, long ooff, hipStream_t st) {
+    switch (h->plan.KS) {
+#define CASE_KS(v) case v: return launch_g0_t<v, NF, R>(h, base, gs, d_pts, N, d_out, ostride, ooff, st);
+        PCX_CASES_KS_1_32
+#undef CASE_KS
+    }
+    return fail(PCX_ERR_UNSUPPORTED, "no dim-0 group instantiation for KS=%d", h->plan.KS);
+}
+
+template <int R>
+static int launch_g0(pcx_bary *h, const DerivedTensor &base, const BaryG0 &gs, const double *d_pts, long N, double *d_out,
+                     long ostride, long ooff, hipStream_t st) {
+    return (h->g0_nf == 2) ? launch_g0_nf<2, R>(h, base, gs, d_pts, N, d_out, ostride, ooff, st)
+                           : launch_g0_nf<3, R>(h, base, gs, d_pts, N, d_out, ostride, ooff, st);
+}
+
+#define PCX_DEFINE_SEED_LAUNCHERS(R)                                                                                             \
+    PCX_HIDDEN int bary_launch_rowcode_seed##R(pcx_bary *h, const double *const *frag_tab, int m, const double *d_pts, long N,   \
+                                               double *d_out, long ostride, long ooff, hipStream_t st, Scratch *split_scratch,   \
+                                               const int *perm) {                                                                \
+        return launch_rowcode<R>(h, frag_tab, m, d_pts, N, d_out, ostride, ooff, st, split_scratch, perm);                       \
+    }                                                                                                                            \
+    PCX_HIDDEN int bary_launch_mfma4_seed##R(pcx_bary *h, const double *const *frag_tab, int m, const double *d_pts, long N,     \
+                                             double *d_out, long ostride, long ooff, hipStream_t st, const int *perm) {          \
+        return launch_mfma4<R>(h, frag_tab, m, d_pts, N, d_out, ostride, ooff, st, perm);                                        \
+    }                                                                                                                            \
+    PCX_HIDDEN int bary_launch_g0_seed##R(pcx_bary *h, const DerivedTensor &base, const BaryG0 &gs, const double *d_pts, long N, \
+                                          double *d_out, long ostride, long ooff, hipStream_t st) {                              \
+        return launch_g0<R>(h, base, gs, d_pts, N, d_out, ostride, ooff, st);                                                    \
+    }
diff --git a/pychebyshev_amd/csrc/pcx_bary.hip b/pychebyshev_amd/csrc/pcx_bary.hip
--- a/pychebyshev_amd/csrc/pcx_bary.hip
+++ b/pychebyshev_amd/csrc/pcx_bary.hip
@@ -1,6 +1,7 @@
 
 #include "pcx_bary_internal.h"
 #include "bary_kernels.h"
+#include "bary_mfma_launch.h"
 #include "gather_kernels.h"
 #include "sobol_kernels.h"
 
@@ -12,16 +13,21 @@
 static const int kCacheSpecs = 96;
 
 static const int kKsList[] = {1, 2, 3, 4, 5, 6, 7, 8, 9, 10, 11, 12, 13, 14, 15, 16, 17, 18, 19, 20, 21, 22,
-                              23, 24, 25, 26, 27, 28, 29, 30, 31, 32, 36, 40, 44, 48, 52, 56, 60, 64};
-
-static int pick_ks(int K) {
-    int need = (K + 3) / 4;
+                              23, 24, 25, 26, 27, 28, 29, 30, 31, 32, 36, 40, 42, 44, 48, 52, 56, 60, 64};
+
+static int pick_ks(int K, int R = 0) {
+    int need = (K - R + 3) / 4;
     for (int ks : kKsList)
-        if (ks >= need) return ks;
+        if (ks >= need && (ks != 42 || R > 0)) return ks;
     return -1;
 }
 
-static bool plan_mfma(const BaryDims &dm, BaryMfmaPlan &best) {
+static int seed_columns(long K, bool seed) {
+    const int r = (int)(K % 4);
+    return (seed && K > 4 && (r == 1 || r == 2)) ? r : 0;
+}
+
+static bool plan_mfma(const BaryDims &dm, BaryMfmaPlan &best, bool seed) {
     bool found = false;
     long best_cost = 0;
     for (int split = std::max(0, dm.d - 2 * PCX_CODE_FIELDS); split < dm.d; ++split) {
@@ -31,27 +37,20 @@
         for (int k = split; k < dm.d; ++k) { K *= dm.n[k]; tail_rows += dm.n[k]; }
         if (K > 256 || M > (1 << 24)) continue;
         if (head_rows > PCX_MAX_PART_ROWS || tail_rows > PCX_MAX_PART_ROWS) continue;
-        int ks = pick_ks((int)K);
+        const int R = seed_columns(K, seed);
+        int ks = pick_ks((int)K, R);
         if (ks < 0) continue;
         long mt = (M + 15) / 16;
-        long cost = mt * (ks + 5) * (ks > 32 ? 23 : 20);
+        long cost = mt * (2 * ks + 10 + (R > 0 ? 1 : 0)) * (ks > 32 ? 23 : 20);
         if (!found || cost < best_cost || (cost == best_cost && K > best.K)) {
             found = true;
             best_cost = cost;
-            best.split = split; best.M = (int)M; best.K = (int)K; best.MT = (int)mt; best.KS = ks;
+            best.split = split; best.M = (int)M; best.K = (int)K; best.MT = (int)mt; best.KS = ks; best.R = R;
             best.tail_base = (int)head_rows + 1;
             best.rows = dm.sum_n + 2;
         }
     }
     return found;
-}
-
-static size_t mfma4_lds_bytes(const BaryDims &dm, int ks) {
-    return ((size_t)8 * (dm.sum_n + 2) * 32 + (size_t)2 * ks * 64) * sizeof(double);
-}
-
-static size_t mfma_lds_bytes(const BaryDims &dm, int nt) {
-    return (size_t)4 * (dm.sum_n + 2) * 16 * nt * sizeof(double);
 }
 
 extern "C" int pcx_bary_destroy(pcx_bary *h) {
@@ -83,8 +82,9 @@
     if (!h->mfma_ok) return PCX_OK;
     const BaryMfmaPlan &p = h->plan;
     size_t cnt = h->kfold_ok ? bary_kfold_frag_count(h->kf) : (size_t)(h->grid_ok ? h->gp.MT : p.MT) * p.KS * 64;
+    const size_t nseed = (size_t)p.MT * 16 * p.R;
     DevBuf frag, slot;
-    int rc = frag.alloc(cnt * sizeof(double));
+    int rc = frag.alloc((cnt + nseed) * sizeof(double));
     if (rc) return rc;
     if (h->kfold_ok) {
         if ((rc = bary_pack_kfold(h, dt.plain, frag.as<double>()))) return rc;
@@ -93,8 +93,13 @@
     } else {
         int blocks = (int)((cnt + 255) / 256);
         hipLaunchKernelGGL(k_pack_fragments, dim3(blocks), dim3(256), 0, h->stream, dt.plain, frag.as<double>(),
-                           p.M, p.K, p.MT, p.KS);
+                           p.M, p.K, p.MT, p.KS, p.R);
         HIP_TRY(hipGetLastError());
+        if (nseed) {
+            hipLaunchKernelGGL(k_pack_seed, dim3((unsigned)((nseed + 255) / 256)), dim3(256), 0, h->stream, dt.plain,
+                               frag.as<double>() + cnt, p.M, p.K, p.MT, p.R, 0);
+            HIP_TRY(hipGetLastError());
+        }
     }
     if ((rc = slot.alloc(sizeof(double *)))) return rc;
     double *fp = frag.as<double>();
@@ -160,7 +165,8 @@
     while (lpp < 64 && (size_t)(256 / lpp) * sum_n * sizeof(double) > 48 * 1024) lpp <<= 1;
     h->lpp = lpp;
 
-    h->mfma_ok = plan_mfma(h->dims, h->plan);
+    { const char *e = getenv("PCX_BARY_SEED"); h->seed = !(e && e[0] == '0'); }
+    h->mfma_ok = plan_mfma(h->dims, h->plan, h->seed);
     if (h->mfma_ok) {
         const bool narrow = h->plan.split <= PCX_CODE_FIELDS && d - h->plan.split <= PCX_CODE_FIELDS;
         h->nt = (h->plan.KS <= 32 || (narrow && h->plan.KS <= 40)) ? 2 : 1;
@@ -206,9 +212,8 @@
     }
     if (h->mfma_ok) {
         const BaryMfmaPlan &p = h->plan;
-        const unsigned ones_h = (unsigned)(p.tail_base - 1), ones_t = (unsigned)(p.rows - 1 - p.tail_base);
-        std::vector<unsigned> rowcode((size_t)p.MT * 16), kcode((size_t)p.KS * 4);
-        std::vector<unsigned> rowcode_hi(rowcode.size()), kcode_hi(kcode.size());
+        const unsigned ones_h = (unsigned)(p.tail_base - 1);
+        std::vector<unsigned> rowcode((size_t)p.MT * 16), rowcode_hi((size_t)p.MT * 16);
         h->wide = p.split > PCX_CODE_FIELDS || d - p.split > PCX_CODE_FIELDS;
         for (long m = 0; m < (long)p.MT * 16; ++m) {
             unsigned f[2 * PCX_CODE_FIELDS] = {ones_h, ones_h, ones_h, ones_h, ones_h, ones_h, ones_h, ones_h};
@@ -223,19 +228,6 @@
             rowcode[m] = f[0] | (f[1] << 8) | (f[2] << 16) | (f[3] << 24);
             rowcode_hi[m] = f[4] | (f[5] << 8) | (f[6] << 16) | (f[7] << 24);
         }
-        for (long kk = 0; kk < (long)p.KS * 4; ++kk) {
-            unsigned f[2 * PCX_CODE_FIELDS] = {ones_t, ones_t, ones_t, ones_t, ones_t, ones_t, ones_t, ones_t};
-            if (kk < p.K) {
-                long rem = kk;
-                for (int k = d - 1; k >= p.split; --k) {
-                    int i = (int)(rem % h->dims.n[k]);
-                    rem /= h->dims.n[k];
-                    f[k - p.split] = (unsigned)(h->dims.off[k] - h->dims.off[p.split] + i);
-                }
-            }
-            kcode[kk] = f[0] | (f[1] << 8) | (f[2] << 16) | (f[3] << 24);
-            kcode_hi[kk] = f[4] | (f[5] << 8) | (f[6] << 16) | (f[7] << 24);
-        }
         auto lane_order = [&](std::vector<unsigned> &v) {
             std::vector<unsigned> o(v.size());
             for (long t = 0; t < (long)p.MT; ++t)
@@ -247,14 +239,10 @@
         lane_order(rowcode_hi);
         if (h->wide) {
             CREATE_TRY(hipMalloc((void **)&h->d_rowcode_hi, rowcode_hi.size() * sizeof(unsigned)));
-            CREATE_TRY(hipMalloc((void **)&h->d_kcode_hi, kcode_hi.size() * sizeof(unsigned)));
             CREATE_TRY(hipMemcpy(h->d_rowcode_hi, rowcode_hi.data(), rowcode_hi.size() * sizeof(unsigned), hipMemcpyHostToDevice));
-            CREATE_TRY(hipMemcpy(h->d_kcode_hi, kcode_hi.data(), kcode_hi.size() * sizeof(unsigned), hipMemcpyHostToDevice));
         }
         CREATE_TRY(hipMalloc((void **)&h->d_rowcode, rowcode.size() * sizeof(unsigned)));
-        CREATE_TRY(hipMalloc((void **)&h->d_kcode, kcode.size() * sizeof(unsigned)));
         CREATE_TRY(hipMemcpy(h->d_rowcode, rowcode.data(), rowcode.size() * sizeof(unsigned), hipMemcpyHostToDevice));
-        CREATE_TRY(hipMemcpy(h->d_kcode, kcode.data(), kcode.size() * sizeof(unsigned), hipMemcpyHostToDevice));
         long M1 = 1;
         for (int k = 1; k < p.split; ++k) M1 *= h->dims.n[k];
         if (!h->wide && p.split >= 2 && p.split <= PCX_CODE_FIELDS && h->nt == 2 && p.KS <= 32 && M1 >= 16 &&
@@ -290,6 +278,9 @@
         }
     }
 
+    BaryMfmaPlan uplan = h->plan;
+    uplan.R = 0;
+    if (h->mfma_ok) uplan.KS = pick_ks(uplan.K);
     if (h->mfma_ok && !(h->plan.split > PCX_CODE_FIELDS || d - h->plan.split > PCX_CODE_FIELDS)) {
         long kfold_est = 0;
         {
@@ -299,11 +290,11 @@
             BaryGridPlan gtry;
             gtry.MT = 0;
             if (keff > 0 && !h->g0_ok) {
-                (void)bary_plan_grid(h->dims, h->plan, gtry);
+                (void)bary_plan_grid(h->dims, uplan, gtry);
                 if (gtry.MT > 0)
-                    geff = (long)((double)h->plan.M * h->plan.K * 10000.0 / ((double)gtry.MT * 16.0 * h->plan.KS * 4.0));
+                    geff = (long)((double)uplan.M * uplan.K * 10000.0 / ((double)gtry.MT * 16.0 * uplan.KS * 4.0));
             }
-            h->kfold_ok = bary_kfold_take(h->kf, keff, geff, h->plan.KS);
+            h->kfold_ok = bary_kfold_take(h->kf, keff, geff, uplan.KS);
         }
         if (h->kfold_ok) {
             const int nt_rc = h->nt;
@@ -317,9 +308,9 @@
             (void)hipFree(h->d_rowcode_g0);
             h->d_rowcode_g0 = nullptr;
         }
-        if (!h->kfold_ok && !h->g0_ok) h->grid_ok = bary_plan_grid(h->dims, h->plan, h->gp);
+        if (!h->kfold_ok && !h->g0_ok) h->grid_ok = bary_plan_grid(h->dims, uplan, h->gp);
         if (h->grid_ok) {
-            h->nt = h->plan.KS > 32 ? 1 : 2;
+            h->nt = uplan.KS > 32 ? 1 : 2;
             const size_t cap = (size_t)(h->gp.wpb == 4 ? 150 : 64) * 1024;
             if (bary_grid_lds_bytes(h, h->nt) > cap) h->nt = 1;
             if (bary_grid_lds_bytes(h, h->nt) > cap) h->grid_ok = false;
@@ -343,6 +334,32 @@
         CREATE_TRY(hipMemcpy(h->d_gsnodes, sn.data(), sn.size() * sizeof(double), hipMemcpyHostToDevice));
     }
     if (h->grid_ok || h->kfold_ok) h->mfma4_ok = false;
+    if (h->grid_ok || h->kfold_ok) h->plan = uplan;
+    if (h->mfma_ok) {
+        const BaryMfmaPlan &p = h->plan;
+        const unsigned ones_t = (unsigned)(p.rows - 1 - p.tail_base);
+        std::vector<unsigned> kcode((size_t)p.KS * 4 + p.R), kcode_hi((size_t)p.KS * 4 + p.R);
+        for (long kk = 0; kk < (long)kcode.size(); ++kk) {
+            unsigned f[2 * PCX_CODE_FIELDS] = {ones_t, ones_t, ones_t, ones_t, ones_t, ones_t, ones_t, ones_t};
+            const long col = kk < (long)p.KS * 4 ? p.R + kk : kk - (long)p.KS * 4;
+            if (col < p.K) {
+                long rem = col;
+                for (int k = d - 1; k >= p.split; --k) {
+                    int i = (int)(rem % h->dims.n[k]);
+                    rem /= h->dims.n[k];
+                    f[k - p.split] = (unsigned)(h->dims.off[k] - h->dims.off[p.split] + i);
+                }
+            }
+            kcode[kk] = f[0] | (f[1] << 8) | (f[2] << 16) | (f[3] << 24);
+            kcode_hi[kk] = f[4] | (f[5] << 8) | (f[6] << 16) | (f[7] << 24);
+        }
+        if (h->wide) {
+            CREATE_TRY(hipMalloc((void **)&h->d_kcode_hi, kcode_hi.size() * sizeof(unsigned)));
+            CREATE_TRY(hipMemcpy(h->d_kcode_hi, kcode_hi.data(), kcode_hi.size() * sizeof(unsigned), hipMemcpyHostToDevice));
+        }
+        CREATE_TRY(hipMalloc((void **)&h->d_kcode, kcode.size() * sizeof(unsigned)));
+        CREATE_TRY(hipMemcpy(h->d_kcode, kcode.data(), kcode.size() * sizeof(unsigned), hipMemcpyHostToDevice));
+    }
 
     DerivedTensor dt;
     {
@@ -540,115 +557,6 @@
     return PCX_OK;
 }
 
-template <int KS, int NT, bool WIDE, int NF = 4>
-static int launch_mfma_t(pcx_bary *h, const double *const *frag_tab, int m, const double *d_pts, long N,
-                         double *d_out, long ostride, long ooff, hipStream_t st, Scratch *split_scratch,
-                         const int *perm) {
-    const bool allow_split = split_scratch != nullptr;
-    size_t lds = mfma_lds_bytes(h->dims, NT);
-    auto kern = k_bary_mfma<KS, NT, WIDE, NF>;
-    if (lds > 64 * 1024)
-        HIP_TRY(hipFuncSetAttribute((const void *)kern, hipFuncAttributeMaxDynamicSharedMemorySize, (int)lds));
-    long per_wg = 4L * 16 * NT;
-    long blocks = (N + per_wg - 1) / per_wg;
-    if (blocks > 0x7fffffffL) return fail(PCX_ERR_UNSUPPORTED, "batch too large for one launch");
-    int nchunks = (h->plan.MT + PCX_CHUNK_TILES - 1) / PCX_CHUNK_TILES;
-    int nsplit = 1, cps = nchunks;
-    const long want = 512;
-    if (allow_split && blocks * m < want && nchunks > 1) {
-        nsplit = (int)std::min<long>(nchunks, (want + blocks * m - 1) / (blocks * m));
-        cps = (nchunks + nsplit - 1) / nsplit;
-        nsplit = (nchunks + cps - 1) / cps;
-    }
-    double *partial = nullptr;
-    if (nsplit > 1) {
-        int rc = split_scratch->reserve((size_t)m * nchunks * 4 * (size_t)N * sizeof(double));
-        if (rc) return rc;
-        partial = (double *)split_scratch->ptr;
-    }
-    hipLaunchKernelGGL(kern, dim3((unsigned)blocks, (unsigned)nsplit, (unsigned)m), dim3(256), lds, st,
-                       h->dims, h->plan, h->d_nodes, h->d_wts, frag_tab, h->d_rowcode, h->d_kcode,
-                       h->d_rowcode_hi, h->d_kcode_hi, d_pts, d_out, N, ostride, ooff, cps, partial, perm, BaryG0{}, nullptr);
-    HIP_TRY(hipGetLastError());
-    if (nsplit > 1) {
-        long cnt = N * m;
-        hipLaunchKernelGGL(k_bary_reduce, dim3((unsigned)((cnt + 255) / 256)), dim3(256), 0, st, partial, d_out,
-                           N, nchunks, m, ostride, ooff, perm);
-        HIP_TRY(hipGetLastError());
-    }
-    return PCX_OK;
-}
-
-template <int KS>
-static int launch_mfma4_t(pcx_bary *h, const double *const *frag_tab, int m, const double *d_pts, long N,
-                          double *d_out, long ostride, long ooff, hipStream_t st, const int *perm) {
-    size_t lds = mfma4_lds_bytes(h->dims, KS);
-    auto kern = k_bary_mfma4<KS>;
-    if (lds > 64 * 1024)
-        HIP_TRY(hipFuncSetAttribute((const void *)kern, hipFuncAttributeMaxDynamicSharedMemorySize, (int)lds));
-    long blocks = (N + 255) / 256;
-    if (blocks > 0x7fffffffL) return fail(PCX_ERR_UNSUPPORTED, "batch too large for one launch");
-    hipLaunchKernelGGL(kern, dim3((unsigned)blocks, 1, (unsigned)m), dim3(512), lds, st, h->dims, h->plan,
-                       h->d_nodes, h->d_wts, frag_tab, h->d_rowcode, h->d_kcode, d_pts, d_out, N, ostride, ooff, perm);
-    HIP_TRY(hipGetLastError());
-    return PCX_OK;
-}
-
-static int launch_mfma4(pcx_bary *h, const double *const *frag_tab, int m, const double *d_pts, long N,
-                        double *d_out, long ostride, long ooff, hipStream_t st, const int *perm) {
-    switch (h->plan.KS) {
-#define CASE_KS(v) case v: return launch_mfma4_t<v>(h, frag_tab, m, d_pts, N, d_out, ostride, ooff, st, perm);
-        CASE_KS(1) CASE_KS(2) CASE_KS(3) CASE_KS(4) CASE_KS(5) CASE_KS(6) CASE_KS(7) CASE_KS(8)
-        CASE_KS(9) CASE_KS(10) CASE_KS(11) CASE_KS(12) CASE_KS(13) CASE_KS(14) CASE_KS(15) CASE_KS(16)
-        CASE_KS(17) CASE_KS(18) CASE_KS(19) CASE_KS(20) CASE_KS(21) CASE_KS(22) CASE_KS(23) CASE_KS(24)
-        CASE_KS(25) CASE_KS(26) CASE_KS(27) CASE_KS(28) CASE_KS(29) CASE_KS(30) CASE_KS(31) CASE_KS(32)
-#undef CASE_KS
-    }
-    return fail(PCX_ERR_UNSUPPORTED, "no MFMA instantiation for KS=%d", h->plan.KS);
-}
-
-template <int NT, bool WIDE, int NF>
-static int launch_mfma_nf(pcx_bary *h, const double *const *frag_tab, int m, const double *d_pts, long N,
-                          double *d_out, long ostride, long ooff, hipStream_t st, Scratch *split_scratch,
-                          const int *perm) {
-    switch (h->plan.KS) {
-#define CASE_KS(v) case v: return launch_mfma_t<v, NT, WIDE, NF>(h, frag_tab, m, d_pts, N, d_out, ostride, ooff, st, split_scratch, perm);
-        CASE_KS(1) CASE_KS(2) CASE_KS(3) CASE_KS(4) CASE_KS(5) CASE_KS(6) CASE_KS(7) CASE_KS(8)
-        CASE_KS(9) CASE_KS(10) CASE_KS(11) CASE_KS(12) CASE_KS(13) CASE_KS(14) CASE_KS(15) CASE_KS(16)
-        CASE_KS(17) CASE_KS(18) CASE_KS(19) CASE_KS(20) CASE_KS(21) CASE_KS(22) CASE_KS(23) CASE_KS(24)
-        CASE_KS(25) CASE_KS(26) CASE_KS(27) CASE_KS(28) CASE_KS(29) CASE_KS(30) CASE_KS(31) CASE_KS(32)
-#undef CASE_KS
-    }
-    if constexpr (NT == 1) {
-        switch (h->plan.KS) {
-#define CASE_KS(v) case v: return launch_mfma_t<v, 1, WIDE, NF>(h, frag_tab, m, d_pts, N, d_out, ostride, ooff, st, split_scratch, perm);
-            CASE_KS(36) CASE_KS(40) CASE_KS(44) CASE_KS(48) CASE_KS(52) CASE_KS(56) CASE_KS(60) CASE_KS(64)
-#undef CASE_KS
-        }
-    }
-    if constexpr (NT == 2 && !WIDE) {
-        switch (h->plan.KS) {
-#define CASE_KS(v) case v: return launch_mfma_t<v, 2, WIDE, NF>(h, frag_tab, m, d_pts, N, d_out, ostride, ooff, st, split_scratch, perm);
-            CASE_KS(36) CASE_KS(40)
-#undef CASE_KS
-        }
-    }
-    return fail(PCX_ERR_UNSUPPORTED, "no MFMA instantiation for KS=%d, NT=%d", h->plan.KS, NT);
-}
-
-template <int NT, bool WIDE>
-static int launch_mfma_nt(pcx_bary *h, const double *const *frag_tab, int m, const double *d_pts, long N,
-                          double *d_out, long ostride, long ooff, hipStream_t st, Scratch *split_scratch,
-                          const int *perm) {
-    if constexpr (!WIDE) {
-        if (h->plan.split <= 2)
-            return launch_mfma_nf<NT, false, 2>(h, frag_tab, m, d_pts, N, d_out, ostride, ooff, st, split_scratch, perm);
-        if (h->plan.split == 3)
-            return launch_mfma_nf<NT, false, 3>(h, frag_tab, m, d_pts, N, d_out, ostride, ooff, st, split_scratch, perm);
-    }
-    return launch_mfma_nf<NT, WIDE, 4>(h, frag_tab, m, d_pts, N, d_out, ostride, ooff, st, split_scratch, perm);
-}
-
 static int launch_rows(pcx_bary *h, const DerivedTensor &dt, const double *d_pts, long N,
                        double *d_out, long ostride, long ooff, hipStream_t st, const int *perm) {
     int ppw = 256 / h->lpp;
@@ -739,12 +647,18 @@
     const BaryMfmaPlan &p = h->plan;
     const int n0 = h->dims.n[0];
     const size_t cnt = (size_t)n0 * h->g0_tps * p.KS * 64;
+    const size_t nseed = (size_t)n0 * h->g0_tps * 16 * p.R;
     DevBuf frag, slot;
-    int rc = frag.alloc(cnt * sizeof(double));
+    int rc = frag.alloc((cnt + nseed) * sizeof(double));
     if (rc) return rc;
     hipLaunchKernelGGL(k_pack_fragments_slabs, dim3((unsigned)((cnt + 255) / 256)), dim3(256), 0, h->stream, dt.plain,
-                       frag.as<double>(), n0, p.M / n0, p.K, h->g0_tps, p.KS);
+                       frag.as<double>(), n0, p.M / n0, p.K, h->g0_tps, p.KS, p.R);
     HIP_TRY(hipGetLastError());
+    if (nseed) {
+        hipLaunchKernelGGL(k_pack_seed, dim3((unsigned)((nseed + 255) / 256)), dim3(256), 0, h->stream, dt.plain,
+                           frag.as<double>() + cnt, p.M / n0, p.K, n0 * h->g0_tps, p.R, h->g0_tps);
+        HIP_TRY(hipGetLastError());
+    }
     if ((rc = slot.alloc(sizeof(double *)))) return rc;
     double *fp = frag.as<double>();
     HIP_TRY(hipMemcpy(slot.p, &fp, sizeof(double *), hipMemcpyHostToDevice));
@@ -752,39 +666,6 @@
     dt.frag_g0 = frag.release<double>();
     dt.slot_g0 = slot.release<double *>();
     return PCX_OK;
-}
-
-template <int KS, int NF>
-static int launch_g0_t(pcx_bary *h, const DerivedTensor &base, const BaryG0 &gs, const double *d_pts, long N, double *d_out,
-                       long ostride, long ooff, hipStream_t st) {
-    auto kern = k_bary_mfma<KS, 2, false, NF, true>;
-    const size_t lds = mfma_lds_bytes(h->dims, 2);
-    if (lds > 64 * 1024)
-        HIP_TRY(hipFuncSetAttribute((const void *)kern, hipFuncAttributeMaxDynamicSharedMemorySize, (int)lds));
-    const long blocks = (N + 127) / 128;
-    if (blocks > 0x7fffffffL) return fail(PCX_ERR_UNSUPPORTED, "batch too large for one launch");
-    BaryMfmaPlan plan = h->plan;
-    plan.MT = gs.tps * gs.n0;
-    const int nchunks = (plan.MT + PCX_CHUNK_TILES - 1) / PCX_CHUNK_TILES;
-    hipLaunchKernelGGL(kern, dim3((unsigned)blocks, 1, 1), dim3(256), lds, st, h->dims, plan, h->d_nodes, h->d_wts,
-                       (const double *const *)base.slot_g0, h->d_rowcode_g0, h->d_kcode, nullptr, nullptr, d_pts, d_out, N,
-                       ostride, ooff, nchunks, nullptr, nullptr, gs, h->d_diff + h->doff[0]);
-    HIP_TRY(hipGetLastError());
-    return PCX_OK;
-}
-
-template <int NF>
-static int launch_g0_nf(pcx_bary *h, const DerivedTensor &base, const BaryG0 &gs, const double *d_pts, long N, double *d_out,
-                        long ostride, long ooff, hipStream_t st) {
-    switch (h->plan.KS) {
-#define CASE_KS(v) case v: return launch_g0_t<v, NF>(h, base, gs, d_pts, N, d_out, ostride, ooff, st);
-        CASE_KS(1) CASE_KS(2) CASE_KS(3) CASE_KS(4) CASE_KS(5) CASE_KS(6) CASE_KS(7) CASE_KS(8)
-        CASE_KS(9) CASE_KS(10) CASE_KS(11) CASE_KS(12) CASE_KS(13) CASE_KS(14) CASE_KS(15) CASE_KS(16)
-        CASE_KS(17) CASE_KS(18) CASE_KS(19) CASE_KS(20) CASE_KS(21) CASE_KS(22) CASE_KS(23) CASE_KS(24)
-        CASE_KS(25) CASE_KS(26) CASE_KS(27) CASE_KS(28) CASE_KS(29) CASE_KS(30) CASE_KS(31) CASE_KS(32)
-#undef CASE_KS
-    }
-    return fail(PCX_ERR_UNSUPPORTED, "no dim-0 group instantiation for KS=%d", h->plan.KS);
 }
 
 static const long kG0MinPoints = 65536;
@@ -810,18 +691,21 @@
     }
     if (variant == 3) {
         if (!h->mfma4_ok) return fail(PCX_ERR_UNSUPPORTED, "4x4x4 MFMA kernel does not cover this shape");
-        return launch_mfma4(h, frag_tab, m, d_pts, N, d_out, ostride, ooff, st, perm);
+        switch (h->plan.R) {
+        case 1: return bary_launch_mfma4_seed1(h, frag_tab, m, d_pts, N, d_out, ostride, ooff, st, perm);
+        case 2: return bary_launch_mfma4_seed2(h, frag_tab, m, d_pts, N, d_out, ostride, ooff, st, perm);
+        }
+        return launch_mfma4<0>(h, frag_tab, m, d_pts, N, d_out, ostride, ooff, st, perm);
     }
     if (variant == 2) {
         if (!h->mfma_ok) return fail(PCX_ERR_UNSUPPORTED, "MFMA kernel does not cover this shape");
         if (h->kfold_ok) return bary_launch_kfold(h, frag_tab, m, d_pts, N, d_out, ostride, ooff, st, perm);
         if (h->grid_ok) return bary_launch_grid(h, frag_tab, m, d_pts, N, d_out, ostride, ooff, st, split_scratch, perm);
-        int nt = (N >= 65536) ? h->nt : 1;
-        if (h->wide)
-            return nt == 2 ? launch_mfma_nt<2, true>(h, frag_tab, m, d_pts, N, d_out, ostride, ooff, st, split_scratch, perm)
-                           : launch_mfma_nt<1, true>(h, frag_tab, m, d_pts, N, d_out, ostride, ooff, st, split_scratch, perm);
-        return nt == 2 ? launch_mfma_nt<2, false>(h, frag_tab, m, d_pts, N, d_out, ostride, ooff, st, split_scratch, perm)
-                       : launch_mfma_nt<1, false>(h, frag_tab, m, d_pts, N, d_out, ostride, ooff, st, split_scratch, perm);
+        switch (h->plan.R) {
+        case 1: return bary_launch_rowcode_seed1(h, frag_tab, m, d_pts, N, d_out, ostride, ooff, st, split_scratch, perm);
+        case 2: return bary_launch_rowcode_seed2(h, frag_tab, m, d_pts, N, d_out, ostride, ooff, st, split_scratch, perm);
+        }
+        return launch_rowcode<0>(h, frag_tab, m, d_pts, N, d_out, ostride, ooff, st, split_scratch, perm);
     }
     for (int s = 0; s < m; ++s) {
         int rc = launch_rows(h, *dts[s], d_pts, N, d_out, ostride, ooff + s, st, perm);
@@ -905,8 +789,11 @@
         gs.col[i] = col[i];
         gs.maxorder = std::max(gs.maxorder, rel[i]);
     }
-    return (g->g0_nf == 2) ? launch_g0_nf<2>(g, *base, gs, pp, N, d_out, ostride, ooff, st)
-                           : launch_g0_nf<3>(g, *base, gs, pp, N, d_out, ostride, ooff, st);
+    switch (g->plan.R) {
+    case 1: return bary_launch_g0_seed1(g, *base, gs, pp, N, d_out, ostride, ooff, st);
+    case 2: return bary_launch_g0_seed2(g, *base, gs, pp, N, d_out, ostride, ooff, st);
+    }
+    return launch_g0<0>(g, *base, gs, pp, N, d_out, ostride, ooff, st);
 }
 
 static const int kProbePoints = 2048;
diff --git a/pychebyshev_amd/csrc/pcx_bary_internal.h b/pychebyshev_amd/csrc/pcx_bary_internal.h
--- a/pychebyshev_amd/csrc/pcx_bary_internal.h
+++ b/pychebyshev_amd/csrc/pcx_bary_internal.h
@@ -38,6 +38,7 @@
     Scratch s_cheb[2];
     Scratch s_sobol;
     bool mfma_ok = false;
+    bool seed = true;
     BaryMfmaPlan plan;
     int nt = 2;
     unsigned *d_rowcode = nullptr, *d_kcode = nullptr;
@@ -110,6 +111,17 @@
 PCX_HIDDEN int bary_launch_grid(pcx_bary *h, const double *const *frag_tab, int m, const double *d_pts, long N, double *d_out,
                                 long ostride, long ooff, hipStream_t st, Scratch *split_scratch, const int *perm);
 
+#define PCX_DECLARE_SEED_LAUNCHERS(R)                                                                                            \
+    PCX_HIDDEN int bary_launch_rowcode_seed##R(pcx_bary *h, const double *const *frag_tab, int m, const double *d_pts, long N,   \
+                                               double *d_out, long ostride, long ooff, hipStream_t st, Scratch *split_scratch,   \
+                                               const int *perm);                                                                 \
+    PCX_HIDDEN int bary_launch_mfma4_seed##R(pcx_bary *h, const double *const *frag_tab, int m, const double *d_pts, long N,     \
+                                             double *d_out, long ostride, long ooff, hipStream_t st, const int *perm);           \
+    PCX_HIDDEN int bary_launch_g0_seed##R(pcx_bary *h, const DerivedTensor &base, const BaryG0 &gs, const double *d_pts, long N, \
+                                          double *d_out, long ostride, long ooff, hipStream_t st);
+PCX_DECLARE_SEED_LAUNCHERS(1)
+PCX_DECLARE_SEED_LAUNCHERS(2)
+
 PCX_HIDDEN int bary_get_tensor(pcx_bary *h, const int32_t *deriv, DerivedTensor **out);
 PCX_HIDDEN int bary_spec_tensors(pcx_bary *h, const int32_t *derivs, int m, std::vector<DerivedTensor *> &dts,
                                  const double *const **frag_tab);
diff --git a/pychebyshev_amd/csrc/pcx_bary_seed1.hip b/pychebyshev_amd/csrc/pcx_bary_seed1.hip
--- /dev/null
+++ b/pychebyshev_amd/csrc/pcx_bary_seed1.hip
@@ -0,0 +1,4 @@
+
+#include "bary_mfma_launch.h"
+
+PCX_DEFINE_SEED_LAUNCHERS(1)
diff --git a/pychebyshev_amd/csrc/pcx_bary_seed2.hip b/pychebyshev_amd/csrc/pcx_bary_seed2.hip
--- /dev/null
+++ b/pychebyshev_amd/csrc/pcx_bary_seed2.hip
@@ -0,0 +1,4 @@
+
+#include "bary_mfma_launch.h"
+
+PCX_DEFINE_SEED_LAUNCHERS(2)
diff --git a/pychebyshev_amd/csrc/pcx_common.h b/pychebyshev_amd/csrc/pcx_common.h
--- a/pychebyshev_amd/csrc/pcx_common.h
+++ b/pychebyshev_amd/csrc/pcx_common.h
@@ -25,6 +25,7 @@
     int K;
     int MT;
     int KS;
+    int R;
     int tail_base;
     int rows;
 };
```
